# daniabib/ComfyUI_ProPainter_Nodes

Measured on NVIDIA H100. Metric: inpainted frames/sec at 640x360, 80-frame subvideo, higher is better.
Workload: dtype f16

## Files before the change

comfyui_propainter_nodes_b200/csrc/capi.cu:

```cuda
#include <math.h>
#include <string.h>

#include <thread>
#include <vector>

#include "../../include/propainter_b200.h"
#include "engine.cuh"

struct DeviceGuard {
  int prev = -1;
  bool changed = false, ok = true;
  explicit DeviceGuard(int dev) {
    if (cudaGetDevice(&prev) != cudaSuccess) prev = -1;
    if (prev != dev) {
      ok = cudaSetDevice(dev) == cudaSuccess;
      changed = ok;
    }
  }
  ~DeviceGuard() {
    if (changed && prev >= 0) cudaSetDevice(prev);
  }
};

#define PP_HANDLE(h)                                     \
  if ((h) == nullptr) {                                  \
    pp_set_error("null engine handle");                  \
    return PP_ERR_ARG;                                   \
  }                                                      \
  PPEngine& e = *reinterpret_cast<PPEngine*>(h);         \
  DeviceGuard _dev_guard(e.device);                      \
  if (!_dev_guard.ok) {                                  \
    pp_set_error("cudaSetDevice(%d) failed", e.device);  \
    return PP_ERR_CUDA;                                  \
  }

static inline cudaStream_t as_stream(void* s) { return reinterpret_cast<cudaStream_t>(s); }

struct ArenaGuard {
  PPArena& a;
  size_t m;
  bool keep = false;
  explicit ArenaGuard(PPArena& arena) : a(arena), m(arena.mark()) {}
  ~ArenaGuard() { if (!keep) a.release(m); }
};

template <class E>
static int op_instnorm(PPEngine& e, const void* x, const void* residual, void* out, int N, int HW, int C, int relu,
                       cudaStream_t st) {
  ArenaGuard guard(e.arena);
  float* sums;
  PP_TRY(pp_alloc(e, &sums, pp_k_instnorm_scratch_floats(N, HW, C), "instnorm sums"));
  PP_TRY(pp_k_instnorm_stats(static_cast<const E*>(x), N, HW, C, sums, st));
  PP_TRY(pp_k_instnorm_apply(static_cast<const E*>(x), sums, static_cast<const E*>(residual), static_cast<E*>(out), N,
                             HW, C, relu, st));
  PP_CUDA_CHECK(cudaStreamSynchronize(st));
  return PP_OK;
}

template <class E>
static int op_corr_pyramid(PPEngine& e, const void* fmap1, const void* fmap2, int pairs, int h8, int w8, void* l0,
                           void* l1, void* l2, void* l3, cudaStream_t st) {
  ArenaGuard guard(e.arena);
  const int P = h8 * w8, P_pad = pp_raft_corr_pad(P);
  E* fpack;
  PP_TRY(pp_alloc(e, &fpack, (size_t)pairs * P_pad * 256 * (sizeof(E) == 4 ? 3 : 1), "fmap packed"));
  PP_TRY(pp_k_pack_b_operand(static_cast<const E*>(fmap2), fpack, pairs, P, P_pad, 256, st));
  e.launches++;
  E* const corr[4] = {static_cast<E*>(l0), static_cast<E*>(l1), static_cast<E*>(l2), static_cast<E*>(l3)};
  PP_TRY(pp_raft_corr_volume<E>(e, static_cast<const E*>(fmap1), fpack, pairs, P, P_pad, corr[0], st));
  PP_TRY(pp_raft_corr_pool(e, corr, (long long)pairs * P, h8, w8, st));
  PP_CUDA_CHECK(cudaStreamSynchronize(st));
  return PP_OK;
}

template <class E>
static int flow_complete_dist(pp_handle h, const char* what, const float* flows_f, const float* flows_b,
                              const float* flow_masks, int T, int H, int W, float* out_f, float* out_b, int team_first,
                              int team_size, void* stream) {
  PP_HANDLE(h);
  PP_REQUIRE(flows_f && flows_b && flow_masks && out_f && out_b, "%s: null pointer", what);
  PP_REQUIRE(e.comm != nullptr || team_size <= 1, "%s: pp_comm_init was not called", what);
  PP_REQUIRE(team_first >= 0 && team_size >= 1 && team_first + team_size <= e.world,
             "%s: team [%d, %d) of %d ranks", what, team_first, team_first + team_size, e.world);
  ArenaGuard guard(e.arena);
  return pp_stage_flow_complete<E>(e, flows_f, flows_b, flow_masks, T, H, W, out_f, out_b, team_first, team_size,
                                   as_stream(stream));
}

extern "C" {

const char* pp_version(void) { return "propainter_b200 1 sm_90a"; }

int pp_create(int device, void* workspace, size_t workspace_bytes, pp_handle* out) {
  PP_REQUIRE(out != nullptr, "pp_create: out is null");
  PP_REQUIRE(workspace != nullptr && workspace_bytes >= (64u << 20), "pp_create: workspace must be >= 64 MiB");
  PP_REQUIRE((reinterpret_cast<uintptr_t>(workspace) & 255) == 0, "pp_create: workspace must be 256-byte aligned");
  PP_CUDA_CHECK(cudaSetDevice(device));
  cudaDeviceProp prop;
  PP_CUDA_CHECK(cudaGetDeviceProperties(&prop, device));
  PP_REQUIRE(prop.major == 9 && prop.minor == 0, "pp_create: this library is built for sm_90a (Hopper H100); device %d is sm_%d%d",
             device, prop.major, prop.minor);
  PPEngine* e = new PPEngine();
  e->device = device;
  e->arena.base = static_cast<uint8_t*>(workspace);
  e->arena.cap = workspace_bytes;
  if (cudaMalloc(&e->prog_counter, 256) != cudaSuccess || cudaMemset(e->prog_counter, 0, 256) != cudaSuccess) {
    delete e;
    pp_set_error("pp_create: cudaMalloc of the program barrier word failed");
    return PP_ERR_CUDA;
  }
  *out = reinterpret_cast<pp_handle>(e);
  return PP_OK;
}

int pp_set_workspace(pp_handle h, void* workspace, size_t workspace_bytes) {
  PP_HANDLE(h);
  PP_REQUIRE(!e.gen.active, "pp_set_workspace: a generator session is active (call pp_gen_end first)");
  PP_REQUIRE(e.arena.off == 0, "pp_set_workspace: the arena is in use");
  PP_REQUIRE(workspace != nullptr && workspace_bytes >= (64u << 20), "pp_set_workspace: workspace must be >= 64 MiB");
  PP_REQUIRE((reinterpret_cast<uintptr_t>(workspace) & 255) == 0, "pp_set_workspace: workspace must be 256-byte aligned");
  e.arena.base = static_cast<uint8_t*>(workspace);
  e.arena.cap = workspace_bytes;
  e.arena.peak = 0;
  return PP_OK;
}

int pp_destroy(pp_handle h) {
  if (h != nullptr) {
    PPEngine* e = reinterpret_cast<PPEngine*>(h);
    pp_comm_destroy_impl(*e);
    if (e->prog_counter != nullptr) cudaFree(e->prog_counter);
    delete e;
  }
  return PP_OK;
}

int pp_comm_unique_id(void* out128) {
  PP_REQUIRE(out128 != nullptr, "pp_comm_unique_id: null pointer");
  return pp_comm_unique_id_impl(out128);
}

int pp_comm_init(pp_handle h, const void* unique_id128, int rank, int world) {
  PP_HANDLE(h);
  PP_REQUIRE(unique_id128 != nullptr, "pp_comm_init: null id");
  return pp_comm_init_impl(e, unique_id128, rank, world);
}

int pp_comm_destroy(pp_handle h) {
  PP_HANDLE(h);
  return pp_comm_destroy_impl(e);
}

int pp_comm_all_gather_rows(pp_handle h, void* buf, const long long* rows_per_member, size_t row_bytes, int first_rank,
                            int n_members, void* stream) {
  PP_HANDLE(h);
  PP_REQUIRE(buf != nullptr && rows_per_member != nullptr && row_bytes > 0 && n_members >= 1,
             "pp_comm_all_gather_rows: bad argument");
  std::vector<long long> off(n_members, 0);
  for (int m = 1; m < n_members; ++m) off[m] = off[m - 1] + rows_per_member[m - 1];
  return pp_comm_all_gather_blocks_impl(e, buf, off.data(), rows_per_member, row_bytes, first_rank, n_members,
                                        as_stream(stream));
}

int pp_register_conv(pp_handle h, const char* name, const void* w, const float* bias, int cout_g, int cout_g_pad,
                     int bn, int cin_g, int kh, int kw, int groups) {
  PP_HANDLE(h);
  PP_REQUIRE(name != nullptr && w != nullptr, "pp_register_conv: null argument");
  PP_REQUIRE(bn % 16 == 0 && bn >= 16 && bn <= 256 && cout_g_pad % bn == 0 && cout_g <= cout_g_pad && cin_g % 8 == 0,
             "pp_register_conv(%s): invalid packing (cout_g=%d pad=%d bn=%d cin_g=%d)", name, cout_g, cout_g_pad, bn,
             cin_g);
  PPPackedConv c;
  c.w = static_cast<const __half*>(w); c.b = bias;
  c.cout_g = cout_g; c.cout_g_pad = cout_g_pad; c.bn = bn; c.cin_g = cin_g; c.kh = kh; c.kw = kw; c.groups = groups;
  e.convs[name] = c;
  return PP_OK;
}

int pp_set_conv_macs(pp_handle h, const char* name, double macs_per_pixel) {
  PP_HANDLE(h);
  PP_REQUIRE(name != nullptr, "pp_set_conv_macs: null name");
  auto it = e.convs.find(name);
  PP_REQUIRE(it != e.convs.end(), "pp_set_conv_macs: conv '%s' is not registered", name);
  it->second.macs_per_pixel = macs_per_pixel;
  return PP_OK;
}

int pp_register_tensor(pp_handle h, const char* name, const void* ptr, size_t bytes) {
  PP_HANDLE(h);
  PP_REQUIRE(name != nullptr && ptr != nullptr, "pp_register_tensor: null argument");
  PPTensor t;
  t.ptr = ptr; t.bytes = bytes;
  e.tensors[name] = t;
  return PP_OK;
}

int pp_raft_bidir(pp_handle h, const float* frames, int T, int H, int W, int iters, float* flows_f, float* flows_b,
                  void* stream) {
  PP_HANDLE(h);
  PP_REQUIRE(frames && flows_f && flows_b, "pp_raft_bidir: null pointer");
  ArenaGuard guard(e.arena);
  return pp_stage_raft<__half>(e, frames, T, H, W, iters, flows_f, flows_b, as_stream(stream));
}

int pp_raft_bidir_fp32(pp_handle h, const float* frames, int T, int H, int W, int iters, float* flows_f, float* flows_b,
                       void* stream) {
  PP_HANDLE(h);
  PP_REQUIRE(frames && flows_f && flows_b, "pp_raft_bidir_fp32: null pointer");
  ArenaGuard guard(e.arena);
  return pp_stage_raft<float>(e, frames, T, H, W, iters, flows_f, flows_b, as_stream(stream));
}

int pp_flow_complete(pp_handle h, const float* flows_f, const float* flows_b, const float* flow_masks, int T, int H,
                     int W, float* out_f, float* out_b, void* stream) {
  PP_HANDLE(h);
  PP_REQUIRE(flows_f && flows_b && flow_masks && out_f && out_b, "pp_flow_complete: null pointer");
  ArenaGuard guard(e.arena);
  return pp_stage_flow_complete<__half>(e, flows_f, flows_b, flow_masks, T, H, W, out_f, out_b, 0, 1,
                                        as_stream(stream));
}

int pp_flow_complete_fp32(pp_handle h, const float* flows_f, const float* flows_b, const float* flow_masks, int T, int H,
                          int W, float* out_f, float* out_b, void* stream) {
  PP_HANDLE(h);
  PP_REQUIRE(flows_f && flows_b && flow_masks && out_f && out_b, "pp_flow_complete_fp32: null pointer");
  ArenaGuard guard(e.arena);
  return pp_stage_flow_complete<float>(e, flows_f, flows_b, flow_masks, T, H, W, out_f, out_b, 0, 1, as_stream(stream));
}

int pp_flow_complete_dist(pp_handle h, const float* flows_f, const float* flows_b, const float* flow_masks, int T, int H,
                          int W, float* out_f, float* out_b, int team_first, int team_size, void* stream) {
  return flow_complete_dist<__half>(h, "pp_flow_complete_dist", flows_f, flows_b, flow_masks, T, H, W, out_f, out_b,
                                    team_first, team_size, stream);
}

int pp_flow_complete_dist_fp32(pp_handle h, const float* flows_f, const float* flows_b, const float* flow_masks, int T,
                               int H, int W, float* out_f, float* out_b, int team_first, int team_size, void* stream) {
  return flow_complete_dist<float>(h, "pp_flow_complete_dist_fp32", flows_f, flows_b, flow_masks, T, H, W, out_f,
                                   out_b, team_first, team_size, stream);
}

int pp_image_propagate(pp_handle h, const float* frames, const float* masks, const float* flows_f,
                       const float* flows_b, int T, int H, int W, float* updated_frames, float* updated_masks,
                       void* stream) {
  PP_HANDLE(h);
  PP_REQUIRE(frames && masks && flows_f && flows_b && updated_frames && updated_masks,
             "pp_image_propagate: null pointer");
  ArenaGuard guard(e.arena);
  return pp_stage_image_propagate<__half>(e, frames, masks, flows_f, flows_b, T, H, W, updated_frames, updated_masks,
                                          as_stream(stream));
}

int pp_image_propagate_fp32(pp_handle h, const float* frames, const float* masks, const float* flows_f,
                            const float* flows_b, int T, int H, int W, float* updated_frames, float* updated_masks,
                            void* stream) {
  PP_HANDLE(h);
  PP_REQUIRE(frames && masks && flows_f && flows_b && updated_frames && updated_masks,
             "pp_image_propagate_fp32: null pointer");
  ArenaGuard guard(e.arena);
  return pp_stage_image_propagate<float>(e, frames, masks, flows_f, flows_b, T, H, W, updated_frames, updated_masks,
                                         as_stream(stream));
}

int pp_gen_begin_subset(pp_handle h, const float* updated_frames, const float* masks_dilated,
                        const float* updated_masks, const float* flows_f, const float* flows_b, int T, int H, int W,
                        const unsigned char* frames_needed, void* stream) {
  PP_HANDLE(h);
  PP_REQUIRE(updated_frames && masks_dilated && updated_masks && flows_f && flows_b, "pp_gen_begin: null pointer");
  const int r = pp_stage_gen_begin(e, updated_frames, masks_dilated, updated_masks, flows_f, flows_b, T, H, W,
                                   frames_needed, as_stream(stream));
  if (r != PP_OK) pp_stage_gen_end(e);
  return r;
}

int pp_gen_begin(pp_handle h, const float* updated_frames, const float* masks_dilated, const float* updated_masks,
                 const float* flows_f, const float* flows_b, int T, int H, int W, void* stream) {
  return pp_gen_begin_subset(h, updated_frames, masks_dilated, updated_masks, flows_f, flows_b, T, H, W, nullptr, stream);
}

int pp_gen_window(pp_handle h, const int* frame_ids, int t, int l_t, void* pred_f16, void* stream) {
  PP_HANDLE(h);
  PP_REQUIRE(frame_ids && pred_f16, "pp_gen_window: null pointer");
  ArenaGuard guard(e.arena);
  return pp_stage_gen_window(e, frame_ids, t, l_t, static_cast<__half*>(pred_f16), as_stream(stream));
}

int pp_gen_run(pp_handle h, const int* frame_ids, const int* win_t, const int* win_lt, int n_windows, void* pred_f16,
               void* stream) {
  PP_HANDLE(h);
  PP_REQUIRE(frame_ids && win_t && win_lt && pred_f16, "pp_gen_run: null pointer");
  ArenaGuard guard(e.arena);
  return pp_stage_gen_run(e, frame_ids, win_t, win_lt, n_windows, static_cast<__half*>(pred_f16), as_stream(stream));
}

int pp_gen_end(pp_handle h) {
  PP_HANDLE(h);
  return pp_stage_gen_end(e);
}

int pp_composite(pp_handle h, const void* pred_f16, const float* masks_dilated, const uint8_t* orig, uint8_t* comp,
                 const int* frame_ids_dev, const int* first_visit_dev, int l_t, int H, int W, int half_math,
                 void* stream) {
  PP_HANDLE(h);
  PP_REQUIRE(pred_f16 && masks_dilated && orig && comp && frame_ids_dev && first_visit_dev, "pp_composite: null pointer");
  e.launches++;
  return pp_k_composite(static_cast<const __half*>(pred_f16), 4, masks_dilated, orig, comp, frame_ids_dev,
                        first_visit_dev, l_t, H, W, half_math, as_stream(stream));
}

int pp_preprocess(pp_handle h, const float* image, const float* mask, int mask_frames, int T, int H, int W,
                  int flow_mask_dilates, int mask_dilates, uint8_t* orig_u8, float* frames, float* flow_masks,
                  float* masks_dilated, void* stream) {
  PP_HANDLE(h);
  PP_REQUIRE(image && mask && orig_u8 && frames && flow_masks && masks_dilated, "pp_preprocess: null pointer");
  ArenaGuard guard(e.arena);
  uint8_t* scratch;
  PP_TRY(pp_alloc(e, &scratch, (size_t)mask_frames * H * W, "mask scratch"));
  PP_TRY(pp_k_quantize_frames(image, orig_u8, frames, T, H, W, as_stream(stream)));
  PP_TRY(pp_k_prepare_masks(mask, mask_frames, T, H, W, flow_mask_dilates, mask_dilates, scratch, flow_masks,
                            masks_dilated, as_stream(stream)));
  e.launches += 4;
  return PP_OK;
}

static int preprocess_from_u8(PPEngine& e, const uint8_t* u8_in, const uint8_t* m_in, int mask_frames, int T, int H, int W,
                              int out_h, int out_w, int flow_mask_dilates, int mask_dilates, uint8_t* orig_u8, float* frames,
                              float* flow_masks, float* masks_dilated, cudaStream_t st) {
  const bool resize = out_h != H || out_w != W;
  const uint8_t* m_use = m_in;
  if (resize) {
    const size_t mid_px = (size_t)T * H * out_w;
    uint8_t *tmp, *m_out;
    int* coef;
    const int mx = out_h > out_w ? out_h : out_w;
    const double sc = fmax(fmax((double)H / out_h, (double)W / out_w), 1.0);
    const size_t coef_ints = 2 * (size_t)mx * ((size_t)ceil(2.0 * sc) * 2 + 1 + 2) + 64;
    PP_TRY(pp_alloc(e, &tmp, mid_px * 3, "resize pass 1"));
    PP_TRY(pp_alloc(e, &m_out, (size_t)mask_frames * out_h * out_w, "mask resized"));
    PP_TRY(pp_alloc(e, &coef, coef_ints, "resize coefficients"));
    PP_TRY(pp_k_resize_bicubic_u8(u8_in, orig_u8, tmp, coef, coef_ints, T, H, W, 3, out_h, out_w, st));
    PP_TRY(pp_k_resize_bicubic_u8(m_in, m_out, tmp, coef, coef_ints, mask_frames, H, W, 1, out_h, out_w, st));
    m_use = m_out;
    e.launches += 4;
  } else {
    PP_CUDA_CHECK(cudaMemcpyAsync(orig_u8, u8_in, (size_t)T * H * W * 3, cudaMemcpyDeviceToDevice, st));
  }
  PP_TRY(pp_k_u8_to_frames(orig_u8, frames, T, out_h, out_w, st));
  PP_TRY(pp_k_dilate_masks_u8(m_use, mask_frames, T, out_h, out_w, flow_mask_dilates, mask_dilates, flow_masks,
                              masks_dilated, st));
  e.launches += 3;
  return PP_OK;
}

int pp_preprocess_resize(pp_handle h, const float* image, const float* mask, int mask_frames, int T, int H, int W,
                         int out_h, int out_w, int flow_mask_dilates, int mask_dilates, uint8_t* orig_u8, float* frames,
                         float* flow_masks, float* masks_dilated, void* stream) {
  PP_HANDLE(h);
  PP_REQUIRE(image && mask && orig_u8 && frames && flow_masks && masks_dilated, "pp_preprocess_resize: null pointer");
  PP_REQUIRE(out_h > 0 && out_w > 0 && H > 0 && W > 0, "pp_preprocess_resize: bad size");
  ArenaGuard guard(e.arena);
  cudaStream_t st = as_stream(stream);
  const size_t in_px = (size_t)T * H * W;
  uint8_t *u8_in, *m_in;
  PP_TRY(pp_alloc(e, &u8_in, in_px * 3, "resize input"));
  PP_TRY(pp_alloc(e, &m_in, (size_t)mask_frames * H * W, "mask input"));
  PP_TRY(pp_k_quantize_u8(image, u8_in, (long long)in_px * 3, st));
  PP_TRY(pp_k_quantize_u8(mask, m_in, (long long)mask_frames * H * W, st));
  e.launches += 2;
  return preprocess_from_u8(e, u8_in, m_in, mask_frames, T, H, W, out_h, out_w, flow_mask_dilates, mask_dilates, orig_u8,
                            frames, flow_masks, masks_dilated, st);
}

int pp_preprocess_u8(pp_handle h, const uint8_t* image_u8, const uint8_t* mask_u8, int mask_frames, int T, int H, int W,
                     int out_h, int out_w, int flow_mask_dilates, int mask_dilates, uint8_t* orig_u8, float* frames,
                     float* flow_masks, float* masks_dilated, void* stream) {
  PP_HANDLE(h);
  PP_REQUIRE(image_u8 && mask_u8 && orig_u8 && frames && flow_masks && masks_dilated, "pp_preprocess_u8: null pointer");
  PP_REQUIRE(out_h > 0 && out_w > 0 && H > 0 && W > 0, "pp_preprocess_u8: bad size");
  ArenaGuard guard(e.arena);
  return preprocess_from_u8(e, image_u8, mask_u8, mask_frames, T, H, W, out_h, out_w, flow_mask_dilates, mask_dilates,
                            orig_u8, frames, flow_masks, masks_dilated, as_stream(stream));
}

int pp_host_quantize_u8(const float* src, uint8_t* dst, long long n, int threads) {
  PP_REQUIRE(src != nullptr && dst != nullptr && n >= 0, "pp_host_quantize_u8: bad argument");
  if (threads < 1) threads = 1;
  if (threads > 64) threads = 64;
  auto work = [=](long long lo, long long hi) {
    for (long long i = lo; i < hi; ++i) {
      float v = src[i] * 255.0f;
      v = v < 0.0f ? 0.0f : (v > 255.0f ? 255.0f : v);
      dst[i] = (uint8_t)(int)v;
    }
  };
  if (threads == 1 || n < (1 << 16)) { work(0, n); return PP_OK; }
  std::vector<std::thread> pool;
  const long long per = (n + threads - 1) / threads;
  for (int t = 0; t < threads; ++t) {
    const long long lo = t * per, hi = lo + per < n ? lo + per : n;
    if (lo < hi) pool.emplace_back(work, lo, hi);
  }
  for (auto& th : pool) th.join();
  return PP_OK;
}

int pp_postprocess(pp_handle h, const uint8_t* comp_u8, float* image_out, long long n, void* stream) {
  PP_HANDLE(h);
  PP_REQUIRE(comp_u8 && image_out, "pp_postprocess: null pointer");
  e.launches++;
  return pp_k_u8_to_unit_float(comp_u8, image_out, n, as_stream(stream));
}

long long pp_launch_count(pp_handle h) { return h ? reinterpret_cast<PPEngine*>(h)->launches : 0; }
size_t pp_workspace_peak(pp_handle h) { return h ? reinterpret_cast<PPEngine*>(h)->arena.peak : 0; }

int pp_profile_enable(pp_handle h, int on) {
  PP_HANDLE(h);
  PP_CUDA_CHECK(cudaDeviceSynchronize());
  for (auto& r : e.prof) { cudaEventDestroy(r.a); cudaEventDestroy(r.b); }
  e.prof.clear();
  e.profile = on != 0;
  return PP_OK;
}

int pp_profile_dump(pp_handle h, char* buf, size_t cap) {
  PP_HANDLE(h);
  PP_REQUIRE(buf != nullptr && cap > 0, "pp_profile_dump: no buffer");
  PP_CUDA_CHECK(cudaDeviceSynchronize());
  struct Agg { long long n = 0; double ms = 0, rows = 0, flops = 0, bytes = 0; };
  std::map<std::string, Agg> agg;
  for (auto& r : e.prof) {
    float ms = 0.f;
    if (cudaEventElapsedTime(&ms, r.a, r.b) != cudaSuccess) ms = 0.f;
    Agg& a = agg[r.name];
    a.n++; a.ms += ms; a.rows += r.rows; a.flops += r.flops; a.bytes += r.bytes;
  }
  size_t off = 0;
  buf[0] = 0;
  for (auto& kv : agg) {
    char line[512];
    int n = snprintf(line, sizeof(line), "%s\t%lld\t%.6f\t%.0f\t%.0f\t%.0f\n", kv.first.c_str(), kv.second.n,
                     kv.second.ms, kv.second.rows, kv.second.flops, kv.second.bytes);
    if (off + n + 1 > cap) { pp_set_error("pp_profile_dump: buffer too small"); return PP_ERR_ARG; }
    memcpy(buf + off, line, n + 1);
    off += n;
  }
  return PP_OK;
}

int pp_op_conv(pp_handle h, const char* name, const void* x_f16, int N, int H, int W, int stride, int pad, int dil,
               int replicate, int act, float slope, const void* residual_f16, void* out_f16, void* stream) {
  PP_HANDLE(h);
  const PPPackedConv* w = nullptr;
  PP_TRY(pp_get_conv(e, name, &w));
  PPConvCall c(e, name, N, H, W);
  c.in(static_cast<const __half*>(x_f16), w->cin_g * w->groups, 0, w->cin_g, w->groups > 1 ? w->cin_g : 0)
      .geom(stride, stride, pad, pad, dil, dil, replicate)
      .out(static_cast<__half*>(out_f16), w->cout_g * w->groups, 0, w->groups > 1 ? w->cout_g : 0)
      .act(act, slope);
  if (residual_f16 != nullptr) c.residual(static_cast<const __half*>(residual_f16), w->cout_g * w->groups, 0);
  return c.run(as_stream(stream));
}

int pp_op_corr_lookup(pp_handle h, const void* l0, const void* l1, const void* l2, const void* l3,
                      const float* coords, void* out_f16, long long nq, int h8, int w8, void* stream) {
  PP_HANDLE(h);
  e.launches++;
  return pp_k_corr_lookup(static_cast<const __half*>(l0), static_cast<const __half*>(l1),
                          static_cast<const __half*>(l2), static_cast<const __half*>(l3), coords,
                          static_cast<__half*>(out_f16), 328, nq, h8, w8, as_stream(stream));
}

int pp_op_conv_tf32(pp_handle h, const char* name, const float* x0, int x0_C, int x0_co, int x0_ch, const float* x1,
                    int x1_C, int x1_co, int x1_ch, int N, int H, int W, int sh, int sw, int ph, int pw, int dh, int dw,
                    int replicate, int epi, int act, float slope, float scale, int act2, const float* aux0, int aux0_C, int aux0_co, float* aux1,
                    int aux1_C, int aux1_co, float* out, int out_C, int out_co, int out_fp32, void* stream) {
  PP_HANDLE(h);
  PP_REQUIRE(name && x0 && out, "pp_op_conv_tf32: null pointer");
  PP_REQUIRE(epi == PP_EPI_STD || (aux0 && aux1), "pp_op_conv_tf32: the GRU epilogues need aux0 and aux1");
  PPConvCall c(e, name, N, H, W);
  c.in(x0, x0_C, x0_co, x0_ch);
  if (x1 != nullptr) c.in(x1, x1_C, x1_co, x1_ch);
  c.geom(sh, sw, ph, pw, dh, dw, replicate);
  if (out_fp32) c.out_f32(out, out_C, out_co);
  else c.out(out, out_C, out_co);
  if (epi == PP_EPI_GRU_ZR) {
    c.gru_zr(aux0, aux0_C, aux0_co, aux1, aux1_C, aux1_co);
  } else if (epi == PP_EPI_GRU_H) {
    c.gru_h(aux0, aux0_C, aux0_co, aux1, aux1_C, aux1_co);
  } else {
    c.act(act, slope, scale, act2);
    if (aux0 != nullptr) c.residual(aux0, aux0_C, aux0_co);
  }
  return c.run(as_stream(stream));
}

int pp_op_dcn_sample_f32(pp_handle h, const float* x0, int C0, const float* x1, int C1, const float* offs, int N,
                         int H, int W, float max_mag, float* cols, void* stream) {
  PP_HANDLE(h);
  const auto al16 = [](const void* p) { return (reinterpret_cast<uintptr_t>(p) & 15) == 0; };
  PP_REQUIRE(al16(x0) && al16(x1) && al16(cols), "pp_op_dcn_sample_f32: x0, x1 and cols must be 16-byte aligned");
  e.launches++;
  return pp_k_dcn_sample(x0, C0, x1, C1, offs, 432, max_mag, cols, N, H, W, as_stream(stream));
}

int pp_op_upsample2x_f32(pp_handle h, const float* src, float* dst, int N, int H, int W, int C, void* stream) {
  PP_HANDLE(h);
  PP_REQUIRE(src && dst, "pp_op_upsample2x_f32: null pointer");
  PP_REQUIRE(((reinterpret_cast<uintptr_t>(src) | reinterpret_cast<uintptr_t>(dst)) & 15) == 0,
             "pp_op_upsample2x_f32: src and dst must be 16-byte aligned");
  e.launches++;
  return pp_k_upsample2x(src, dst, N, H, W, C, as_stream(stream));
}

int pp_op_instnorm(pp_handle h, const void* x, const void* residual, void* out, int N, int HW, int C, int relu, int fp32,
                   void* stream) {
  PP_HANDLE(h);
  PP_REQUIRE(x && out, "pp_op_instnorm: null pointer");
  return fp32 ? op_instnorm<float>(e, x, residual, out, N, HW, C, relu, as_stream(stream))
              : op_instnorm<__half>(e, x, residual, out, N, HW, C, relu, as_stream(stream));
}

int pp_op_corr_pyramid(pp_handle h, const void* fmap1, const void* fmap2, int pairs, int h8, int w8, int fp32, void* l0,
                       void* l1, void* l2, void* l3, void* stream) {
  PP_HANDLE(h);
  PP_REQUIRE(fmap1 && fmap2 && l0 && l1 && l2 && l3 && pairs >= 1, "pp_op_corr_pyramid: bad argument");
  return fp32 ? op_corr_pyramid<float>(e, fmap1, fmap2, pairs, h8, w8, l0, l1, l2, l3, as_stream(stream))
              : op_corr_pyramid<__half>(e, fmap1, fmap2, pairs, h8, w8, l0, l1, l2, l3, as_stream(stream));
}

int pp_op_corr_lookup_f32(pp_handle h, const float* l0, const float* l1, const float* l2, const float* l3,
                          const float* coords, float* out, long long nq, int h8, int w8, void* stream) {
  PP_HANDLE(h);
  e.launches++;
  return pp_k_corr_lookup(l0, l1, l2, l3, coords, out, 352, nq, h8, w8, as_stream(stream));
}

int pp_op_convex_upsample(pp_handle h, const float* coords1, const void* mask, float* out, int B, int h8, int w8, int fp32,
                          void* stream) {
  PP_HANDLE(h);
  e.launches++;
  if (fp32) return pp_k_convex_upsample(coords1, static_cast<const float*>(mask), out, B, h8, w8, as_stream(stream));
  return pp_k_convex_upsample(coords1, static_cast<const __half*>(mask), out, B, h8, w8, as_stream(stream));
}

int pp_op_imgprop_step(pp_handle h, const void* cur4_f16, const void* prop_in4_f16, void* prop_out4_f16,
                       const void* flow_prop_f16, const void* flow_check_f16, int H, int W, void* stream) {
  PP_HANDLE(h);
  e.launches++;
  return pp_k_imgprop_step(static_cast<const __half*>(cur4_f16), static_cast<const __half*>(prop_in4_f16),
                           static_cast<__half*>(prop_out4_f16), static_cast<const __half*>(flow_prop_f16),
                           static_cast<const __half*>(flow_check_f16), H, W, as_stream(stream));
}

int pp_op_imgprop_step_f32(pp_handle h, const float* cur4, const float* prop_in4, float* prop_out4,
                           const float* flow_prop, const float* flow_check, int H, int W, void* stream) {
  PP_HANDLE(h);
  PP_REQUIRE(cur4 && prop_in4 && prop_out4 && flow_prop && flow_check, "pp_op_imgprop_step_f32: null pointer");
  e.launches++;
  return pp_k_imgprop_step(cur4, prop_in4, prop_out4, flow_prop, flow_check, H, W, as_stream(stream));
}

int pp_op_attention(pp_handle h, const void* qkv_f16, const void* pkv_f16, void* out_f16, const int* win_flags_dev,
                    int t, int gh, int gw, int n_pool, int parity, void* stream) {
  PP_HANDLE(h);
  const int nh = pp_ceil_div(gh, 5) * 5, nw = pp_ceil_div(gw, 9) * 9;
  std::vector<int> ring;
  pp_build_ring_indices(nh, nw, ring);
  ArenaGuard guard(e.arena);
  int* ring_dev;
  PP_TRY(pp_alloc(e, &ring_dev, ring.size(), "ring indices"));
  PP_CUDA_CHECK(cudaMemcpyAsync(ring_dev, ring.data(), ring.size() * sizeof(int), cudaMemcpyHostToDevice,
                                as_stream(stream)));
  const __half* qkv = static_cast<const __half*>(qkv_f16);
  const __half* pkv = static_cast<const __half*>(pkv_f16);
  int meta_host[2] = {0, t};
  int* meta_dev;
  PP_TRY(pp_alloc(e, &meta_dev, 2, "attention meta"));
  PP_CUDA_CHECK(cudaMemcpyAsync(meta_dev, meta_host, sizeof(meta_host), cudaMemcpyHostToDevice, as_stream(stream)));
  const int key_stride = ((t + 1) / 2) * (193 + n_pool);
  int* key_tab;
  PP_TRY(pp_alloc(e, &key_tab, (size_t)(nh / 5) * (nw / 9) * key_stride, "attention key table"));
  int r = pp_k_attention(qkv, qkv + 512, qkv + 1024, 1536, pkv, pkv + 512, 1024, static_cast<__half*>(out_f16), 512,
                         win_flags_dev, ring_dev, meta_dev, meta_dev + 1, 1, t, gh, gw, nh, nw, n_pool, parity,
                         key_tab, key_stride, as_stream(stream));
  PP_CUDA_CHECK(cudaStreamSynchronize(as_stream(stream)));
  e.launches++;
  return r;
}

}
```

comfyui_propainter_nodes_b200/csrc/conv_epilogue.cuh:

```cuda
#pragma once
#include "conv_igemm.cuh"
#include "wgmma_ops.cuh"

namespace ppconv {

template <int ACT, bool ACC = false, int N>
__device__ __forceinline__ void act16_t(float (&v)[N], float slope) {
#pragma unroll
  for (int i = 0; i < N; ++i) {
    if (ACT == PP_ACT_RELU) v[i] = fmaxf(v[i], 0.f);
    else if (ACT == PP_ACT_LRELU) v[i] = v[i] > 0.f ? v[i] : v[i] * slope;
    else if (ACT == PP_ACT_SIGMOID) v[i] = ppx::sigmoidf_(v[i]);
    else if (ACT == PP_ACT_TANH) v[i] = ACC ? ppx::tanh_acc(v[i]) : tanhf(v[i]);
    else if (ACT == PP_ACT_GELU) v[i] = ppx::gelu_erf(v[i]);
  }
}
template <bool ACC = false, int N>
__device__ __forceinline__ void act16(float (&v)[N], int act, float slope) {
  switch (act) {
    case PP_ACT_RELU: act16_t<PP_ACT_RELU, ACC>(v, slope); break;
    case PP_ACT_LRELU: act16_t<PP_ACT_LRELU, ACC>(v, slope); break;
    case PP_ACT_SIGMOID: act16_t<PP_ACT_SIGMOID, ACC>(v, slope); break;
    case PP_ACT_TANH: act16_t<PP_ACT_TANH, ACC>(v, slope); break;
    case PP_ACT_GELU: act16_t<PP_ACT_GELU, ACC>(v, slope); break;
    default: break;
  }
}

__device__ __forceinline__ void load16(const __half* src, int nvalid, bool vec, float (&r)[16]) {
  if (vec && nvalid == 16) {
    const uint4 a = reinterpret_cast<const uint4*>(src)[0], b = reinterpret_cast<const uint4*>(src)[1];
    const __half2* ha = reinterpret_cast<const __half2*>(&a);
    const __half2* hb = reinterpret_cast<const __half2*>(&b);
#pragma unroll
    for (int i = 0; i < 4; ++i) {
      const float2 fa = __half22float2(ha[i]), fb = __half22float2(hb[i]);
      r[2 * i] = fa.x; r[2 * i + 1] = fa.y; r[8 + 2 * i] = fb.x; r[8 + 2 * i + 1] = fb.y;
    }
  } else {
#pragma unroll
    for (int i = 0; i < 16; ++i) r[i] = i < nvalid ? __half2float(src[i]) : 0.f;
  }
}
__device__ __forceinline__ void store16(__half* dst, int nvalid, bool vec, const float (&v)[16]) {
  if (vec && nvalid == 16) {
    __align__(16) __half2 h[8];
#pragma unroll
    for (int i = 0; i < 8; ++i) h[i] = __floats2half2_rn(v[2 * i], v[2 * i + 1]);
    reinterpret_cast<uint4*>(dst)[0] = reinterpret_cast<uint4*>(h)[0];
    reinterpret_cast<uint4*>(dst)[1] = reinterpret_cast<uint4*>(h)[1];
  } else {
#pragma unroll
    for (int i = 0; i < 16; ++i)
      if (i < nvalid) dst[i] = __float2half_rn(v[i]);
  }
}

__device__ __forceinline__ void conv_epilogue16(const PPConvParams& p, const uint32_t (&raw)[16], long long mrow, int g,
                                                int ng0, int epi, bool vec) {
    const int nvalid = min(16, p.Cout_g - ng0);
    float v[16];
#pragma unroll
    for (int i = 0; i < 16; ++i) v[i] = __uint_as_float(raw[i]);
    if (p.bias != nullptr) {
      const float* bp = p.bias + g * p.Cout_g + ng0;
      if (vec && nvalid == 16) {
#pragma unroll
        for (int i = 0; i < 4; ++i) {
          const float4 b4 = __ldg(reinterpret_cast<const float4*>(bp) + i);
          v[4 * i] += b4.x; v[4 * i + 1] += b4.y; v[4 * i + 2] += b4.z; v[4 * i + 3] += b4.w;
        }
      } else {
#pragma unroll
        for (int i = 0; i < 16; ++i)
          if (i < nvalid) v[i] += __ldg(bp + i);
      }
    }
    if (epi == PP_EPI_STD) {
      act16(v, p.act1, p.slope);
      if (p.scale != 1.f) {
#pragma unroll
        for (int i = 0; i < 16; ++i) v[i] *= p.scale;
      }
      if (p.aux0 != nullptr) {
        float r[16];
        load16(p.aux0 + mrow * p.aux0_cstride + p.aux0_coff + ng0, nvalid, vec, r);
#pragma unroll
        for (int i = 0; i < 16; ++i) v[i] += r[i];
      }
      act16(v, p.act2, p.slope);
      const long long o = mrow * p.out_cstride + p.out_coff + (long long)g * p.out_gstep + ng0;
      if (p.out_fp32) {
        float* dst = reinterpret_cast<float*>(p.out) + o;
        if (vec && nvalid == 16) {
#pragma unroll
          for (int i = 0; i < 4; ++i)
            reinterpret_cast<float4*>(dst)[i] = make_float4(v[4 * i], v[4 * i + 1], v[4 * i + 2], v[4 * i + 3]);
        } else {
#pragma unroll
          for (int i = 0; i < 16; ++i)
            if (i < nvalid) dst[i] = v[i];
        }
      } else {
        store16(reinterpret_cast<__half*>(p.out) + o, nvalid, vec, v);
      }
    } else if (epi == PP_EPI_GRU_ZR) {
      const int half_c = p.Cout_g >> 1;
      act16_t<PP_ACT_SIGMOID>(v, 0.f);
      if (ng0 < half_c) {
        store16(reinterpret_cast<__half*>(p.out) + mrow * p.out_cstride + p.out_coff + ng0, nvalid, vec, v);
      } else {
        const int c = ng0 - half_c;
        float h[16];
        load16(p.aux0 + mrow * p.aux0_cstride + p.aux0_coff + c, nvalid, vec, h);
#pragma unroll
        for (int i = 0; i < 16; ++i) v[i] *= h[i];
        store16(p.out2 + mrow * p.out2_cstride + p.out2_coff + c, nvalid, vec, v);
      }
    } else {
      float h[16], z[16];
      load16(p.aux0 + mrow * p.aux0_cstride + p.aux0_coff + ng0, nvalid, vec, h);
      load16(p.aux1 + mrow * p.aux1_cstride + p.aux1_coff + ng0, nvalid, vec, z);
      act16_t<PP_ACT_TANH>(v, 0.f);
#pragma unroll
      for (int i = 0; i < 16; ++i) v[i] = (1.f - z[i]) * h[i] + z[i] * v[i];
      store16(reinterpret_cast<__half*>(p.out) + mrow * p.out_cstride + p.out_coff + ng0, nvalid, vec, v);
    }
}

__device__ __forceinline__ void load16_split(const float* src, int lo, int nvalid, bool vec, float (&r)[16]) {
  if (vec && nvalid == 16) {
#pragma unroll
    for (int i = 0; i < 4; ++i) {
      const float4 h = reinterpret_cast<const float4*>(src)[i], l = reinterpret_cast<const float4*>(src + lo)[i];
      r[4 * i] = h.x + l.x; r[4 * i + 1] = h.y + l.y; r[4 * i + 2] = h.z + l.z; r[4 * i + 3] = h.w + l.w;
    }
  } else {
#pragma unroll
    for (int i = 0; i < 16; ++i) r[i] = i < nvalid ? src[i] + src[lo + i] : 0.f;
  }
}
__device__ __forceinline__ void store16_split(float* dst, int lo, int nvalid, bool vec, const float (&v)[16]) {
  float h[16], l[16];
#pragma unroll
  for (int i = 0; i < 16; ++i) { h[i] = ppx::tf32_rna(v[i]); l[i] = v[i] - h[i]; }
  if (vec && nvalid == 16) {
#pragma unroll
    for (int i = 0; i < 4; ++i) {
      reinterpret_cast<float4*>(dst)[i] = make_float4(h[4 * i], h[4 * i + 1], h[4 * i + 2], h[4 * i + 3]);
      reinterpret_cast<float4*>(dst + lo)[i] = make_float4(l[4 * i], l[4 * i + 1], l[4 * i + 2], l[4 * i + 3]);
    }
  } else {
#pragma unroll
    for (int i = 0; i < 16; ++i)
      if (i < nvalid) { dst[i] = h[i]; dst[lo + i] = l[i]; }
  }
}

__device__ __forceinline__ void conv_epilogue16_split(const PPConvParams& p, const float (&acc)[16], long long mrow, int g,
                                                      int ng0, bool vec) {
  const int nvalid = min(16, p.Cout_g - ng0);
  float v[16];
#pragma unroll
  for (int i = 0; i < 16; ++i) v[i] = acc[i];
  if (p.bias != nullptr) {
    const float* bp = p.bias + g * p.Cout_g + ng0;
#pragma unroll
    for (int i = 0; i < 16; ++i)
      if (i < nvalid) v[i] += __ldg(bp + i);
  }
  const float* aux0 = reinterpret_cast<const float*>(p.aux0);
  const float* aux1 = reinterpret_cast<const float*>(p.aux1);
  float* out = reinterpret_cast<float*>(p.out);
  if (p.epi == PP_EPI_STD) {
    act16<true>(v, p.act1, p.slope);
    if (p.scale != 1.f) {
#pragma unroll
      for (int i = 0; i < 16; ++i) v[i] *= p.scale;
    }
    if (aux0 != nullptr) {
      float r[16];
      load16_split(aux0 + mrow * p.aux0_cstride + p.aux0_coff + ng0, p.aux0_lo, nvalid, vec, r);
#pragma unroll
      for (int i = 0; i < 16; ++i) v[i] += r[i];
    }
    act16<true>(v, p.act2, p.slope);
    float* dst = out + mrow * p.out_cstride + p.out_coff + (long long)g * p.out_gstep + ng0;
    if (p.out_fp32) {
      if (vec && nvalid == 16) {
#pragma unroll
        for (int i = 0; i < 4; ++i)
          reinterpret_cast<float4*>(dst)[i] = make_float4(v[4 * i], v[4 * i + 1], v[4 * i + 2], v[4 * i + 3]);
      } else {
#pragma unroll
        for (int i = 0; i < 16; ++i)
          if (i < nvalid) dst[i] = v[i];
      }
    } else {
      store16_split(dst, p.out_lo, nvalid, vec, v);
    }
  } else if (p.epi == PP_EPI_GRU_ZR) {
    const int half_c = p.Cout_g >> 1;
    act16_t<PP_ACT_SIGMOID, true>(v, 0.f);
    if (ng0 < half_c) {
      store16_split(out + mrow * p.out_cstride + p.out_coff + ng0, p.out_lo, nvalid, vec, v);
    } else {
      const int c = ng0 - half_c;
      float h[16];
      load16_split(aux0 + mrow * p.aux0_cstride + p.aux0_coff + c, p.aux0_lo, nvalid, vec, h);
#pragma unroll
      for (int i = 0; i < 16; ++i) v[i] *= h[i];
      store16_split(reinterpret_cast<float*>(p.out2) + mrow * p.out2_cstride + p.out2_coff + c, p.out2_lo, nvalid, vec, v);
    }
  } else {
    float h[16], z[16];
    load16_split(aux0 + mrow * p.aux0_cstride + p.aux0_coff + ng0, p.aux0_lo, nvalid, vec, h);
    load16_split(aux1 + mrow * p.aux1_cstride + p.aux1_coff + ng0, p.aux1_lo, nvalid, vec, z);
    act16_t<PP_ACT_TANH, true>(v, 0.f);
#pragma unroll
    for (int i = 0; i < 16; ++i) v[i] = (1.f - z[i]) * h[i] + z[i] * v[i];
    store16_split(out + mrow * p.out_cstride + p.out_coff + ng0, p.out_lo, nvalid, vec, v);
  }
}

constexpr int STG_LD = 40;
constexpr int STG_BYTES = 64 * STG_LD * 4;

template <int N, class Emit>
__device__ __forceinline__ void drain_acc(const float (&acc)[N / 2], float* stg, int t128, int bar_id, Emit&& emit) {
  const int wrow = 16 * (t128 >> 5) + ((t128 & 31) >> 2), wcol = 2 * (t128 & 3);
#pragma unroll 1
  for (int c0 = 0; c0 < N; c0 += 32) {
#pragma unroll
    for (int cc = 0; cc < N; cc += 32) {
      if (cc == c0) {
#pragma unroll
        for (int j = 0; j < 4; ++j) {
          if (cc + 8 * j < N) {
            const int i = (cc / 8 + j) * 4;
            *reinterpret_cast<float2*>(stg + wrow * STG_LD + 8 * j + wcol) = make_float2(acc[i], acc[i + 1]);
            *reinterpret_cast<float2*>(stg + (wrow + 8) * STG_LD + 8 * j + wcol) = make_float2(acc[i + 2], acc[i + 3]);
          }
        }
      }
    }
    ppx::named_bar(bar_id, 128);
    const int c = c0 + 16 * (t128 & 1);
    if (c < N) emit(stg + (t128 >> 1) * STG_LD + 16 * (t128 & 1), t128 >> 1, c);
    ppx::named_bar(bar_id, 128);
  }
}

template <bool SPLIT = false, int EPI = -1>
__device__ __forceinline__ void epilogue_from_stage(const PPConvParams& p, const float* src, long long mrow, int g, int ng0) {
  if constexpr (SPLIT) {
    float acc[16];
#pragma unroll
    for (int i = 0; i < 16; i += 4) {
      const float4 v = *reinterpret_cast<const float4*>(src + i);
      acc[i] = v.x; acc[i + 1] = v.y; acc[i + 2] = v.z; acc[i + 3] = v.w;
    }
    conv_epilogue16_split(p, acc, mrow, g, ng0, p.vec_ok != 0);
  } else {
    uint32_t raw[16];
#pragma unroll
    for (int i = 0; i < 16; i += 4) {
      const float4 v = *reinterpret_cast<const float4*>(src + i);
      raw[i] = __float_as_uint(v.x); raw[i + 1] = __float_as_uint(v.y);
      raw[i + 2] = __float_as_uint(v.z); raw[i + 3] = __float_as_uint(v.w);
    }
    conv_epilogue16(p, raw, mrow, g, ng0, EPI >= 0 ? EPI : p.epi, p.vec_ok != 0);
  }
}

template <int V>
struct IntC { static constexpr int value = V; };
template <int MAX_N, class F>
__device__ __forceinline__ void with_tile_width(int bn, F&& f) {
  switch (bn) {
    case 16: f(IntC<16>{}); break;
    case 32: f(IntC<32>{}); break;
    case 48: f(IntC<48>{}); break;
    case 64: f(IntC<64>{}); break;
    case 80: f(IntC<80>{}); break;
    case 96: f(IntC<96>{}); break;
    case 112: f(IntC<112>{}); break;
    case 128: f(IntC<128>{}); break;
    default:
      if constexpr (MAX_N > 128) {
        switch (bn) {
          case 144: f(IntC<144>{}); break;
          case 160: f(IntC<160>{}); break;
          case 176: f(IntC<176>{}); break;
          case 192: f(IntC<192>{}); break;
          case 208: f(IntC<208>{}); break;
          case 224: f(IntC<224>{}); break;
          case 240: f(IntC<240>{}); break;
          case 256: f(IntC<256>{}); break;
          default: __trap();
        }
      } else {
        __trap();
      }
  }
}

}
```

comfyui_propainter_nodes_b200/csrc/conv_gemm.cu:

```cuda
#include <string.h>

#include "conv_epilogue.cuh"
#include "conv_igemm.cuh"

namespace {

constexpr int NUM_THREADS = 384;
constexpr int NUM_CONSUMERS = 256;
constexpr int WARP_PRODUCER = 8;
constexpr int STAGE_BYTES = 48 * 1024;
constexpr int STAGES = 3;
constexpr int OUT_BYTES = 64 * 1024;
constexpr int BIAS_BYTES = 2 * 256 * 4;
constexpr int SMEM_BYTES = 1024 + STAGES * STAGE_BYTES + OUT_BYTES + 1024 + BIAS_BYTES;

struct GemmParams {
  PPConvParams c;
  CUtensorMap tmap_a[PP_MAX_SEGS];
  CUtensorMap tmap_out;
  CUtensorMap tmap_res;
  int m_tiles, n_tiles, chunks;
  int debug;
};

struct Smem {
  uint8_t* stages;
  uint8_t* out;
  uint64_t *full, *empty, *res;
  float* bias;
};
__device__ __forceinline__ Smem gemm_smem() {
  uint8_t* base = ppx::dyn_smem_1024();
  Smem m;
  m.stages = base;
  m.out = base + STAGES * STAGE_BYTES;
  m.full = reinterpret_cast<uint64_t*>(m.out + OUT_BYTES);
  m.empty = m.full + STAGES;
  m.res = m.empty + STAGES;
  m.bias = reinterpret_cast<float*>(m.out + OUT_BYTES + 1024);
  return m;
}

template <int ACT1>
__device__ __forceinline__ void gemm_epi4(float (&v)[4], bool has_bias, const float2& bias, float scale, bool has_res,
                                          const float (&res)[4], int act2, float slope) {
  if (has_bias) {
    v[0] += bias.x; v[1] += bias.y; v[2] += bias.x; v[3] += bias.y;
  }
  ppconv::act16_t<ACT1>(v, slope);
  if (scale != 1.f) {
#pragma unroll
    for (int i = 0; i < 4; ++i) v[i] *= scale;
  }
  if (has_res) {
#pragma unroll
    for (int i = 0; i < 4; ++i) v[i] += res[i];
  }
  if (act2 != PP_ACT_NONE) ppconv::act16(v, act2, slope);
}

template <int MB, int BN, int ACT1>
__device__ __forceinline__ void gemm_epilogue(const PPConvParams& p, const float (&acc)[MB][BN / 2], uint8_t* so,
                                              const float* bs, bool has_res, int t128) {
  constexpr int PANEL = 128 * MB * 128;
  const bool has_bias = p.bias != nullptr;
  const float scale = p.scale, slope = p.slope;
  const int act2 = p.act2;
  const int fr = 16 * (t128 >> 5) + ((t128 & 31) >> 2), fc = 2 * (t128 & 3);
#pragma unroll
  for (int b = 0; b < MB; ++b) {
    const int r = 64 * b + fr;
#pragma unroll
    for (int j = 0; j < BN / 8; ++j) {
      const int col = 8 * j + fc;
      const int off = (col >> 6) * PANEL + r * 128 + (((((col & 63) >> 3) ^ (r & 7))) << 4) + (col & 7) * 2;
      __half2* lo = reinterpret_cast<__half2*>(so + off);
      __half2* hi = reinterpret_cast<__half2*>(so + off + 8 * 128);
      const float2 bias = *reinterpret_cast<const float2*>(bs + col);
      float v[4] = {acc[b][4 * j], acc[b][4 * j + 1], acc[b][4 * j + 2], acc[b][4 * j + 3]};
      float res[4] = {0.f, 0.f, 0.f, 0.f};
      if (has_res) {
        const float2 r0 = __half22float2(*lo), r1 = __half22float2(*hi);
        res[0] = r0.x; res[1] = r0.y; res[2] = r1.x; res[3] = r1.y;
      }
      gemm_epi4<ACT1>(v, has_bias, bias, scale, has_res, res, act2, slope);
      *lo = __floats2half2_rn(v[0], v[1]);
      *hi = __floats2half2_rn(v[2], v[3]);
    }
  }
}

template <int MB, int BN>
__device__ __forceinline__ void gemm_tile(const GemmParams& h, const Smem& m, int tile, int& s, uint32_t& ph, uint32_t& rph,
                                          int wg, int t128) {
  using namespace ppx;
  const PPConvParams& p = h.c;
  constexpr int A_BYTES = 128 * MB * 128;
  constexpr int WG_ROWS = 64 * MB;
  constexpr int PANEL = 128 * MB * 128;
  const int n0 = (tile % h.n_tiles) * BN;
  const int m0 = (tile / h.n_tiles) * (128 * MB);
  float acc[MB][BN / 2];
  int prev = -1;
  for (int c = 0; c < h.chunks; ++c) {
    mbar_wait(&m.full[s], ph);
    const uint32_t a = smem_u32(m.stages + s * STAGE_BYTES);
    uint64_t adesc[MB];
#pragma unroll
    for (int b = 0; b < MB; ++b) adesc[b] = gmma_desc_sw128_kmajor(a + (wg * MB + b) * 64 * 128);
    const uint64_t bdesc = gmma_desc_sw128_kmajor(a + A_BYTES);
    wgmma_fence();
#pragma unroll
    for (int k = 0; k < 4; ++k)
#pragma unroll
      for (int b = 0; b < MB; ++b) wgmma_f16<BN>(acc[b], adesc[b] + 2 * k, bdesc + 2 * k, (c | k) != 0 ? 1u : 0u);
    wgmma_commit();
    wgmma_wait<1>();
    if (prev >= 0) mbar_arrive(&m.empty[prev]);
    prev = s;
    if (++s == STAGES) { s = 0; ph ^= 1; }
  }
  wgmma_wait<0>();
#pragma unroll
  for (int b = 0; b < MB; ++b) wgmma_fence_acc(acc[b]);
  mbar_arrive(&m.empty[prev]);
  if (h.debug & 1) return;

  const int bar_id = 2 + wg, row0 = m0 + wg * WG_ROWS;
  const int npanel = (min(BN, p.Cout_g - n0) + 63) / 64;
  uint8_t* so = m.out + wg * WG_ROWS * 128;
  const bool issuer = t128 == 0;
  float* bs = m.bias + wg * 256;
  {
    const int c0 = 2 * t128, n = n0 + c0;
    float2 bv = make_float2(0.f, 0.f);
    if (p.bias != nullptr && c0 < BN) {
      if (n < p.Cout_g) bv.x = __ldg(p.bias + n);
      if (n + 1 < p.Cout_g) bv.y = __ldg(p.bias + n + 1);
    }
    if (c0 < BN) *reinterpret_cast<float2*>(bs + c0) = bv;
  }
  if (issuer) tma_store_wait_read<0>();
  named_bar(bar_id, 128);
  const bool has_res = p.aux0 != nullptr;
  if (has_res) {
    if (issuer) {
      mbar_arrive_expect_tx(&m.res[wg], (uint32_t)(npanel * WG_ROWS * 128));
      for (int pnl = 0; pnl < npanel; ++pnl) tma_load_2d(smem_u32(so + pnl * PANEL), &h.tmap_res, n0 + pnl * 64, row0, &m.res[wg]);
    }
    mbar_wait(&m.res[wg], rph);
    rph ^= 1;
  }
  switch (p.act1) {
    case PP_ACT_RELU: gemm_epilogue<MB, BN, PP_ACT_RELU>(p, acc, so, bs, has_res, t128); break;
    case PP_ACT_LRELU: gemm_epilogue<MB, BN, PP_ACT_LRELU>(p, acc, so, bs, has_res, t128); break;
    case PP_ACT_SIGMOID: gemm_epilogue<MB, BN, PP_ACT_SIGMOID>(p, acc, so, bs, has_res, t128); break;
    case PP_ACT_TANH: gemm_epilogue<MB, BN, PP_ACT_TANH>(p, acc, so, bs, has_res, t128); break;
    case PP_ACT_GELU: gemm_epilogue<MB, BN, PP_ACT_GELU>(p, acc, so, bs, has_res, t128); break;
    default: gemm_epilogue<MB, BN, PP_ACT_NONE>(p, acc, so, bs, has_res, t128); break;
  }
  fence_proxy_async();
  named_bar(bar_id, 128);
  if (issuer) {
    for (int pnl = 0; pnl < npanel; ++pnl) tma_store_2d(&h.tmap_out, smem_u32(so + pnl * PANEL), n0 + pnl * 64, row0);
    tma_store_commit();
  }
}

template <int MB>
__global__ void __launch_bounds__(NUM_THREADS, 1) conv_gemm_kernel(const __grid_constant__ GemmParams h) {
  using namespace ppx;
  constexpr int BN = 256 / MB;
  constexpr int A_BYTES = 128 * MB * 128;
  const Smem m = gemm_smem();
  const PPConvParams& p = h.c;
  const int tid = threadIdx.x, warp = tid >> 5;
  const int total_tiles = h.m_tiles * h.n_tiles;
  if (tid == 0) {
    for (int s = 0; s < STAGES; ++s) { mbar_init(&m.full[s], 1); mbar_init(&m.empty[s], NUM_CONSUMERS); }
    mbar_init(&m.res[0], 1);
    mbar_init(&m.res[1], 1);
    mbar_fence_init();
  }
  __syncthreads();
  asm volatile("griddepcontrol.wait;" ::: "memory");
  asm volatile("griddepcontrol.launch_dependents;" ::: "memory");

  if (warp < 8) setmaxnreg_inc<232>();
  else setmaxnreg_dec<40>();
  if (warp < 8) {
    const int wg = tid >> 7, t128 = tid & 127;
    int s = 0;
    uint32_t ph = 0, rph = 0;
    for (int tile = blockIdx.x; tile < total_tiles; tile += gridDim.x) gemm_tile<MB, BN>(h, m, tile, s, ph, rph, wg, t128);
    if (t128 == 0) tma_store_wait<0>();
  } else if (warp == WARP_PRODUCER) {
    if (elect_one()) {
      int s = 0;
      uint32_t ph = 0;
      for (int tile = blockIdx.x; tile < total_tiles; tile += gridDim.x) {
        const int n0 = (tile % h.n_tiles) * BN;
        const int m0 = (tile / h.n_tiles) * (128 * MB);
        const uint32_t b_bytes = (uint32_t)(min(BN, p.Cout_g_pad - n0) * 128);
        for (int c = 0; c < h.chunks; ++c) {
          const int ci = c * 64;
          const int q = pp_seg_of(p, ci);
          mbar_wait(&m.empty[s], ph ^ 1);
          mbar_arrive_expect_tx(&m.full[s], (uint32_t)A_BYTES + b_bytes);
          const uint32_t dst = smem_u32(m.stages + s * STAGE_BYTES);
          tma_load_4d(dst, &h.tmap_a[q], ci - p.seg[q].cbegin, m0, 0, 0, &m.full[s]);
          bulk_g2s(dst + A_BYTES, p.wpacked + ((long long)c * p.Cout_g_pad + n0) * 64, b_bytes, &m.full[s]);
          if (++s == STAGES) { s = 0; ph ^= 1; }
        }
      }
    }
  }
}

int gemm_mb(const PPConvParams& p) { return p.Cout_g_pad <= 128 && p.M_total >= 256 ? 2 : 1; }

long long gemm_tiles(const PPConvParams& p, int mb) {
  return pp_ceil_div64(p.M_total, 128 * mb) * pp_ceil_div(p.Cout_g_pad, 256 / mb);
}

bool aligned16(const void* ptr, int cstride, int coff) {
  return (reinterpret_cast<uintptr_t>(ptr) & 15) == 0 && cstride % 8 == 0 && coff % 8 == 0;
}

}

int pp_conv_gemm_eligible(const PPConvParams& p) {
  if (p.kh != 1 || p.kw != 1 || p.sh != 1 || p.sw != 1 || p.ph != 0 || p.pw != 0 || p.pad_replicate) return 0;
  if (p.groups != 1 || p.split || p.epi != PP_EPI_STD || p.out_fp32 || p.M_total < 128) return 0;
  if (!pp_conv_segs_chunked(p, true)) return 0;
  if (!aligned16(p.out, p.out_cstride, p.out_coff)) return 0;
  if (p.aux0 != nullptr && !aligned16(p.aux0, p.aux0_cstride, p.aux0_coff)) return 0;
  if (p.bias != nullptr && (reinterpret_cast<uintptr_t>(p.bias) & 7) != 0) return 0;
  int num_sms = 0;
  if (pp_num_sms(&num_sms) != PP_OK || gemm_tiles(p, gemm_mb(p)) < num_sms) return 0;
  return pp_tmap_supported() ? 1 : 0;
}

int pp_launch_conv_gemm(const PPConvParams& pin, cudaStream_t stream) {
  static bool attr_set = false;
  if (!attr_set) {
    PP_CUDA_CHECK(cudaFuncSetAttribute(conv_gemm_kernel<1>, cudaFuncAttributeMaxDynamicSharedMemorySize, SMEM_BYTES));
    PP_CUDA_CHECK(cudaFuncSetAttribute(conv_gemm_kernel<2>, cudaFuncAttributeMaxDynamicSharedMemorySize, SMEM_BYTES));
    attr_set = true;
  }
  GemmParams h;
  memset(&h, 0, sizeof(h));
  h.c = pin;
  const PPConvParams& p = h.c;
  const int mb = gemm_mb(p);
  h.m_tiles = (int)pp_ceil_div64(p.M_total, 128 * mb);
  h.n_tiles = pp_ceil_div(p.Cout_g_pad, 256 / mb);
  h.chunks = pp_ceil_div(p.Cin, 64);
  PP_REQUIRE((long long)h.m_tiles * h.n_tiles < (1LL << 31), "conv_gemm: too many tiles");
  h.debug = pp_conv_noepi();
  PP_TRY(pp_conv_input_tmaps(p, 128 * mb, 1, true, h.tmap_a));
  PP_TRY(pp_tmap_2d_f16(&h.tmap_out, static_cast<const __half*>(p.out) + p.out_coff, p.Cout_g, p.M_total, p.out_cstride, 64 * mb));
  if (p.aux0 != nullptr)
    PP_TRY(pp_tmap_2d_f16(&h.tmap_res, p.aux0 + p.aux0_coff, p.Cout_g, p.M_total, p.aux0_cstride, 64 * mb));
  int num_sms = 0;
  PP_TRY(pp_num_sms(&num_sms));
  return pp_conv_launch(mb == 2 ? conv_gemm_kernel<2> : conv_gemm_kernel<1>, h, min(h.m_tiles * h.n_tiles, num_sms),
                        NUM_THREADS, SMEM_BYTES, stream);
}
```

comfyui_propainter_nodes_b200/csrc/conv_halo.cu:

```cuda
#include <cuda.h>
#include <stdlib.h>
#include <string.h>

#include <memory>

#include "conv_epilogue.cuh"
#include "conv_igemm.cuh"
#include "dcn_sample.cuh"

namespace {

constexpr int NUM_THREADS = 384;
constexpr int NUM_EPI_THREADS = 256;
constexpr int WARP_A = 8, WARP_B = 9;
constexpr int MAX_SA = 4, MAX_SB = 8;
constexpr int SMEM_BUDGET = 186 * 1024;

struct HaloParams {
  PPConvParams c;
  CUtensorMap tmap[PP_MAX_SEGS];
  int MT;
  int BW, BH;
  int tiles_x, tiles_y, n_tiles;
  int a_stage_bytes, b_stage_bytes, SA, SB;
  int tps;
  int chunks;
  int flat;
  int n_img;
  int sub_bytes;
  int debug;
};

struct TileCoord {
  int n_idx, tx, ty, img, g;
};
__device__ __forceinline__ TileCoord decode_tile(const HaloParams& h, int tile) {
  TileCoord t;
  t.n_idx = tile % h.n_tiles;
  int r = tile / h.n_tiles;
  t.tx = r % h.tiles_x; r /= h.tiles_x;
  t.ty = r % h.tiles_y; r /= h.tiles_y;
  t.img = r % h.n_img;
  t.g = r / h.n_img;
  return t;
}

__host__ __device__ inline int halo_total_tiles(const HaloParams& h) {
  return h.n_tiles * h.tiles_x * h.tiles_y * h.n_img * h.c.groups;
}

struct Ring {
  int s;
  uint32_t ph;
};

struct HaloSmem {
  uint8_t* a;
  uint8_t* b;
  int SA, SB, a_stage_bytes, b_stage_bytes;
  uint64_t *a_full, *a_empty, *b_full, *b_empty;
  uint64_t* spare;
  float* acc_stg;
  int bytes;
};

__host__ __device__ inline HaloSmem halo_smem(uint8_t* base, int SA, int a_stage_bytes, int SB, int b_stage_bytes) {
  const int b_off = SA * a_stage_bytes, bar_off = b_off + SB * b_stage_bytes, acc_off = bar_off + 1024;
  HaloSmem m;
  m.SA = SA; m.SB = SB; m.a_stage_bytes = a_stage_bytes; m.b_stage_bytes = b_stage_bytes;
  m.a = base;
  m.b = base + b_off;
  m.a_full = reinterpret_cast<uint64_t*>(base + bar_off);
  m.a_empty = m.a_full + MAX_SA;
  m.b_full = m.a_empty + MAX_SA;
  m.b_empty = m.b_full + MAX_SB;
  m.spare = m.b_empty + MAX_SB;
  m.acc_stg = reinterpret_cast<float*>(base + acc_off);
  m.bytes = 1024 + acc_off + 2 * ppconv::STG_BYTES;
  return m;
}

__host__ __device__ constexpr int halo_max_tps(int bn) { return 128 / bn > 1 ? 128 / bn : 1; }

template <int BN, int MB, bool TF32>
__device__ __forceinline__ void halo_tap(float (&acc)[MB][BN / 2], uint64_t (&adesc)[MB], uint64_t& bdesc, uint32_t& accum,
                                         int& kx, int kw, uint32_t step_x, uint32_t step_row, uint32_t tap16) {
#pragma unroll
  for (int k = 0; k < 4; ++k)
#pragma unroll
    for (int b = 0; b < MB; ++b) {
      if constexpr (TF32) ppx::wgmma_tf32<BN>(acc[b], adesc[b] + 2 * k, bdesc + 2 * k, (accum | k) != 0 ? 1u : 0u);
      else ppx::wgmma_f16<BN>(acc[b], adesc[b] + 2 * k, bdesc + 2 * k, (accum | k) != 0 ? 1u : 0u);
    }
  accum = 1u;
  bdesc += tap16;
  const uint32_t step = ++kx == kw ? step_row : step_x;
  if (kx == kw) kx = 0;
#pragma unroll
  for (int b = 0; b < MB; ++b) adesc[b] += step;
}

template <int BN, int MB, int NT, bool TF32>
__device__ __forceinline__ void halo_tap_group(int tn, float (&acc)[MB][BN / 2], uint64_t (&adesc)[MB], uint64_t bdesc,
                                               uint32_t& accum, int& kx, int kw, uint32_t step_x, uint32_t step_row,
                                               uint32_t tap16) {
  using namespace ppx;
  if constexpr (NT > 1) {
    if (tn < NT) {
      halo_tap_group<BN, MB, NT - 1, TF32>(tn, acc, adesc, bdesc, accum, kx, kw, step_x, step_row, tap16);
      return;
    }
  }
  wgmma_fence();
#pragma unroll
  for (int tt = 0; tt < NT; ++tt) halo_tap<BN, MB, TF32>(acc, adesc, bdesc, accum, kx, kw, step_x, step_row, tap16);
  wgmma_commit();
}

template <int BN, int MB, int NT, bool TF32 = false, bool PROG = false>
__device__ __forceinline__ void halo_tile(const HaloParams& h, int tile, const HaloSmem& m, Ring& ra, Ring& rb, float* stg,
                                          int wg, int t128) {
  using namespace ppx;
  const PPConvParams& p = h.c;
  const int taps = p.kh * p.kw;
  const TileCoord t = decode_tile(h, tile);
  const int n0 = t.n_idx * p.BN;
  const int bnt = min(p.BN, p.Cout_g_pad - n0);
  const uint32_t sbo = h.flat ? 1024u : (uint32_t)h.BW * 128;
  const uint32_t step_x = (uint32_t)p.dw * 8;
  const uint32_t step_row = (uint32_t)(p.dh * h.BW - (p.kw - 1) * p.dw) * 8;
  const uint32_t tap16 = (uint32_t)p.BN * 8;
  const int kw = p.kw;
  uint32_t aoff[MB];
#pragma unroll
  for (int b = 0; b < MB; ++b) aoff[b] = MB == 2 ? wg * h.sub_bytes + b * 8 * sbo : wg * 8 * sbo;
  float acc[MB][BN / 2];
  uint32_t accum = 0;
  int pend_a = -1, pend_b = -1;
  for (int c = 0; c < h.chunks; ++c) {
    mbar_wait(&m.a_full[ra.s], ra.ph);
    uint64_t adesc[MB];
#pragma unroll
    for (int b = 0; b < MB; ++b) adesc[b] = gmma_desc_sw128_kmajor(smem_u32(m.a + ra.s * m.a_stage_bytes) + aoff[b], sbo);
    int kx = 0;
    for (int tap0 = 0; tap0 < taps; tap0 += h.tps) {
      mbar_wait(&m.b_full[rb.s], rb.ph);
      const uint64_t bdesc = gmma_desc_sw128_kmajor(smem_u32(m.b + rb.s * m.b_stage_bytes));
      halo_tap_group<BN, MB, NT, TF32>(min(h.tps, taps - tap0), acc, adesc, bdesc, accum, kx, kw, step_x, step_row, tap16);
      wgmma_wait<1>();
      if (pend_b >= 0) mbar_arrive(&m.b_empty[pend_b]);
      if (pend_a >= 0) mbar_arrive(&m.a_empty[pend_a]);
      pend_b = rb.s;
      pend_a = tap0 + h.tps >= taps ? ra.s : -1;
      if (++rb.s == m.SB) { rb.s = 0; rb.ph ^= 1; }
    }
    if (++ra.s == m.SA) { ra.s = 0; ra.ph ^= 1; }
  }
  wgmma_wait<0>();
#pragma unroll
  for (int b = 0; b < MB; ++b) wgmma_fence_acc(acc[b]);
  if (pend_b >= 0) mbar_arrive(&m.b_empty[pend_b]);
  if (pend_a >= 0) mbar_arrive(&m.a_empty[pend_a]);

  const bool skip = (h.debug & 1) != 0;
#pragma unroll
  for (int b = 0; b < MB; ++b) {
    const int sub = MB == 2 ? wg : 0, rbase = MB == 2 ? 64 * b : 64 * wg;
    ppconv::drain_acc<BN>(acc[b], stg, t128, 4 + wg, [&](const float* src, int r64, int cc) {
      const int r = rbase + r64;
      bool mvalid;
      long long mrow;
      if (h.flat) {
        mrow = ((long long)t.tx * h.MT + sub) * 128 + r;
        mvalid = mrow < p.M_total;
      } else {
        const int oy = t.ty * 16 + (r >> 3), ox = t.tx * (8 * h.MT) + 8 * sub + (r & 7);
        mvalid = oy < p.OH && ox < p.OW;
        mrow = ((long long)t.img * p.OH + oy) * p.OW + ox;
      }
      if (!mvalid || skip || cc >= bnt || n0 + cc >= p.Cout_g) return;
      ppconv::epilogue_from_stage<TF32, PROG ? PP_EPI_STD : -1>(p, src, mrow, t.g, n0 + cc);
    });
  }
}

template <class F>
__device__ __forceinline__ void with_tile_shape(int mt, int bn, F&& f) {
  if (mt == 2) ppconv::with_tile_width<128>(bn, [&](auto n) { f(n, ppconv::IntC<2>{}); });
  else ppconv::with_tile_width<256>(bn, [&](auto n) { f(n, ppconv::IntC<1>{}); });
}

__device__ __forceinline__ void halo_smem_init_barriers(const HaloSmem& m) {
  using namespace ppx;
  for (int s = 0; s < m.SA; ++s) { mbar_init(&m.a_full[s], 1); mbar_init(&m.a_empty[s], NUM_EPI_THREADS); }
  for (int s = 0; s < m.SB; ++s) { mbar_init(&m.b_full[s], 1); mbar_init(&m.b_empty[s], NUM_EPI_THREADS); }
  mbar_fence_init();
}

__device__ __forceinline__ void halo_produce_patches(const HaloParams& h, const HaloSmem& m, Ring& r) {
  using namespace ppx;
  const PPConvParams& p = h.c;
  const int total_tiles = halo_total_tiles(h);
  const uint32_t bytes = (uint32_t)(h.BW * h.BH * 128);
  for (int tile = blockIdx.x; tile < total_tiles; tile += gridDim.x) {
    const TileCoord t = decode_tile(h, tile);
    const int x0 = h.flat ? t.tx * (128 * h.MT) : t.tx * (8 * h.MT) - p.pw, y0 = h.flat ? 0 : t.ty * 16 - p.ph;
    for (int c = 0; c < h.chunks; ++c) {
      const int ci = c * 64;
      const int q = pp_seg_of(p, ci);
      const int ch0 = t.g * p.seg[q].gstep + (ci - p.seg[q].cbegin);
      mbar_wait(&m.a_empty[r.s], r.ph ^ 1);
      mbar_arrive_expect_tx(&m.a_full[r.s], bytes);
      tma_load_4d(smem_u32(m.a + r.s * m.a_stage_bytes), &h.tmap[q], ch0, x0, y0, t.img, &m.a_full[r.s]);
      if (++r.s == m.SA) { r.s = 0; r.ph ^= 1; }
    }
  }
}

__device__ __forceinline__ void halo_produce_weights(const HaloParams& h, const HaloSmem& m, Ring& r) {
  using namespace ppx;
  const PPConvParams& p = h.c;
  const int total_tiles = halo_total_tiles(h);
  const int taps = p.kh * p.kw;
  for (int tile = blockIdx.x; tile < total_tiles; tile += gridDim.x) {
    const TileCoord t = decode_tile(h, tile);
    const int n0 = t.n_idx * p.BN;
    const uint32_t bytes = (uint32_t)(min(p.BN, p.Cout_g_pad - n0) * 128);
    const __half* wbase = p.wpacked + ((long long)t.g * p.num_kc * p.Cout_g_pad + n0) * 64;
    for (int c = 0; c < h.chunks; ++c) {
      for (int tap0 = 0; tap0 < taps; tap0 += h.tps) {
        const int tn = min(h.tps, taps - tap0);
        mbar_wait(&m.b_empty[r.s], r.ph ^ 1);
        mbar_arrive_expect_tx(&m.b_full[r.s], bytes * (uint32_t)tn);
        for (int t = 0; t < tn; ++t) {
          const int kc = (tap0 + t) * h.chunks + c;
          bulk_g2s(smem_u32(m.b + r.s * m.b_stage_bytes + t * p.BN * 128), wbase + (long long)kc * p.Cout_g_pad * 64, bytes,
                   &m.b_full[r.s]);
        }
        if (++r.s == m.SB) { r.s = 0; r.ph ^= 1; }
      }
    }
  }
}

template <bool TF32>
__device__ __forceinline__ void halo_body(const HaloParams& h) {
  using namespace ppx;
  const HaloSmem m = halo_smem(dyn_smem_1024(), h.SA, h.a_stage_bytes, h.SB, h.b_stage_bytes);
  const int tid = threadIdx.x, warp = tid >> 5;
  if (tid == 0) halo_smem_init_barriers(m);
  __syncthreads();
  asm volatile("griddepcontrol.wait;" ::: "memory");
  asm volatile("griddepcontrol.launch_dependents;" ::: "memory");

  if (warp < 8) setmaxnreg_inc<232>();
  else setmaxnreg_dec<40>();
  if (warp < 8) {
    const int wg = tid >> 7, t128 = tid & 127;
    float* stg = m.acc_stg + wg * (ppconv::STG_BYTES / 4);
    Ring ra = {0, 0}, rb = {0, 0};
    const int total_tiles = halo_total_tiles(h);
    with_tile_shape(h.MT, h.c.BN, [&](auto bn, auto mb) {
      constexpr int BN = decltype(bn)::value;
      for (int tile = blockIdx.x; tile < total_tiles; tile += gridDim.x)
        halo_tile<BN, decltype(mb)::value, halo_max_tps(BN), TF32>(h, tile, m, ra, rb, stg, wg, t128);
    });
  } else if (warp == WARP_A) {
    if (elect_one()) {
      Ring r = {0, 0};
      halo_produce_patches(h, m, r);
    }
  } else if (warp == WARP_B) {
    if (elect_one()) {
      Ring r = {0, 0};
      halo_produce_weights(h, m, r);
    }
  }
}

__global__ void __launch_bounds__(NUM_THREADS, 1) conv_halo_kernel(const __grid_constant__ HaloParams h) {
  halo_body<false>(h);
}

__global__ void __launch_bounds__(NUM_THREADS, 1) conv_halo_tf32_kernel(const __grid_constant__ HaloParams h) {
  halo_body<true>(h);
}

constexpr int PROG_MAX_LAYERS = 10;
enum { PROG_CONV = 0, PROG_DCN = 1 };

constexpr int PROG_WIDTHS[] = {32, 64, 224};

template <class F>
__device__ __forceinline__ void with_prog_width(int bn, F&& f) {
  static_assert(sizeof(PROG_WIDTHS) == 3 * sizeof(int), "with_prog_width: one case per PROG_WIDTHS entry");
  switch (bn) {
    case PROG_WIDTHS[0]: f(ppconv::IntC<PROG_WIDTHS[0]>{}); break;
    case PROG_WIDTHS[1]: f(ppconv::IntC<PROG_WIDTHS[1]>{}); break;
    case PROG_WIDTHS[2]: f(ppconv::IntC<PROG_WIDTHS[2]>{}); break;
    default: __trap();
  }
}

struct ProgParams {
  int n_layers;
  int SA, SB, a_stage_bytes, b_stage_bytes;
  unsigned int* counter;
  unsigned int base;
  unsigned long long* ts;
  int kind[PROG_MAX_LAYERS];
  PPDcnArgs dcn[PROG_MAX_LAYERS];
  HaloParams layer[PROG_MAX_LAYERS];
};

__device__ __forceinline__ void prog_wait(const unsigned int* counter, unsigned int target) {
  unsigned int v, spins = 0;
  uint64_t t0 = 0;
  for (;;) {
    asm volatile("ld.acquire.gpu.global.u32 %0, [%1];" : "=r"(v) : "l"(counter) : "memory");
    if ((int)(v - target) >= 0) return;
    __nanosleep(64);
    if ((++spins & 0xFFFu) == 0) {
      uint64_t now;
      asm volatile("mov.u64 %0, %%globaltimer;" : "=l"(now));
      if (t0 == 0) t0 = now;
      else if (now - t0 > 2000000000ull) __trap();
    }
  }
}

__global__ void __launch_bounds__(NUM_THREADS, 1) conv_prog_kernel(const __grid_constant__ ProgParams P) {
  using namespace ppx;
  const HaloSmem m = halo_smem(dyn_smem_1024(), P.SA, P.a_stage_bytes, P.SB, P.b_stage_bytes);
  uint64_t* layer_go = m.spare;

  const int tid = threadIdx.x, warp = tid >> 5;
  const unsigned int G = gridDim.x;
  if (tid == 0) {
    mbar_init(layer_go, 1);
    halo_smem_init_barriers(m);
  }
  __syncthreads();
  asm volatile("griddepcontrol.wait;" ::: "memory");
  asm volatile("griddepcontrol.launch_dependents;" ::: "memory");

  if (warp < 8) setmaxnreg_inc<232>();
  else setmaxnreg_dec<40>();
  if (warp < 8) {
    const int wg = tid >> 7, t128 = tid & 127;
    float* stg = m.acc_stg + wg * (ppconv::STG_BYTES / 4);
    Ring ra = {0, 0}, rb = {0, 0};
    for (int li = 0; li < P.n_layers; ++li) {
      mbar_wait(layer_go, (uint32_t)li & 1u);
      if (P.ts != nullptr && blockIdx.x == 0 && tid == 0) {
        unsigned long long now;
        asm volatile("mov.u64 %0, %%globaltimer;" : "=l"(now));
        P.ts[2 * li] = now;
      }
      if (P.kind[li] == PROG_DCN) {
        const PPDcnArgs& a = P.dcn[li];
        const unsigned per_img = (unsigned)(a.H * a.W * 144);
        const unsigned total = per_img * (unsigned)a.N;
        const unsigned stride = G * NUM_EPI_THREADS;
        for (unsigned idx = blockIdx.x * NUM_EPI_THREADS + tid; idx < total; idx += 4 * stride) {
#pragma unroll
          for (int u = 0; u < 4; ++u) {
            const unsigned i2 = idx + u * stride;
            if (i2 < total) {
              const unsigned n = i2 / per_img;
              if (a.C == 128) dcn_sample_item<8, true>(a, i2 - n * per_img, (int)n);
              else dcn_sample_item<16, true>(a, i2 - n * per_img, (int)n);
            }
          }
        }
      } else {
        const HaloParams& h = P.layer[li];
        const int total_tiles = halo_total_tiles(h);
        with_prog_width(h.c.BN, [&](auto bn) {
          constexpr int BN = decltype(bn)::value;
          for (int tile = blockIdx.x; tile < total_tiles; tile += G)
            halo_tile<BN, 1, halo_max_tps(BN), false, true>(h, tile, m, ra, rb, stg, wg, t128);
        });
      }
      fence_proxy_async_global();
      asm volatile("bar.sync 1, %0;" ::"n"(NUM_EPI_THREADS) : "memory");
      if (tid == 0) {
        __threadfence();
        atomicAdd(P.counter, 1u);
        if (P.ts != nullptr && blockIdx.x == 0) {
          unsigned long long now;
          asm volatile("mov.u64 %0, %%globaltimer;" : "=l"(now));
          P.ts[2 * li + 1] = now;
        }
      }
    }
  } else if (warp == WARP_A) {
    if (elect_one()) {
      Ring r = {0, 0};
      for (int li = 0; li < P.n_layers; ++li) {
        if (li > 0) {
          prog_wait(P.counter, P.base + (unsigned int)li * G);
          fence_proxy_async_global();
        }
        mbar_arrive(layer_go);
        if (P.kind[li] == PROG_CONV) halo_produce_patches(P.layer[li], m, r);
      }
    }
  } else if (warp == WARP_B) {
    if (elect_one()) {
      Ring r = {0, 0};
      for (int li = 0; li < P.n_layers; ++li)
        if (P.kind[li] == PROG_CONV) halo_produce_weights(P.layer[li], m, r);
    }
  }
}

}

int pp_conv_halo_eligible(const PPConvParams& p) {
  if (p.sh != 1 || p.sw != 1 || p.pad_replicate) return 0;
  const bool flat = p.kh * p.kw == 1;
  if (flat) {
    if (p.ph != 0 || p.pw != 0 || p.groups != 1) return 0;
  } else if (p.Cin % 64 != 0) {
    return 0;
  }
  if (!pp_conv_segs_chunked(p, flat)) return 0;
  if ((p.kw - 1) * p.dw + 16 > 256 || (p.kh - 1) * p.dh + 16 > 256) return 0;
  if ((long long)p.N * p.OH * p.OW < 128) return 0;
  return pp_tmap_supported() ? 1 : 0;
}

namespace {

int halo_set_smem_limit() {
  static bool done = false;
  if (!done) {
    PP_CUDA_CHECK(cudaFuncSetAttribute(conv_halo_kernel, cudaFuncAttributeMaxDynamicSharedMemorySize, 224 * 1024));
    PP_CUDA_CHECK(cudaFuncSetAttribute(conv_halo_tf32_kernel, cudaFuncAttributeMaxDynamicSharedMemorySize, 224 * 1024));
    PP_CUDA_CHECK(cudaFuncSetAttribute(conv_prog_kernel, cudaFuncAttributeMaxDynamicSharedMemorySize, 224 * 1024));
    done = true;
  }
  return PP_OK;
}

bool halo_stages(int budget, int a_bytes, int b_bytes, int& sa, int& sb) {
  for (sa = 3; sa >= 2; --sa) {
    sb = (budget - sa * a_bytes) / b_bytes;
    if (sb >= 3) {
      if (sb > MAX_SB) sb = MAX_SB;
      return true;
    }
  }
  return false;
}

int halo_configure(const PPConvParams& pin, HaloParams& h, bool one_wave) {
  h.c = pin;
  PPConvParams& p = h.c;
  int num_sms = 0;
  PP_TRY(pp_num_sms(&num_sms));
  const bool flat = p.kh * p.kw == 1;
  const int n_tiles0 = pp_ceil_div(p.Cout_g_pad, 128);
  int bn = pp_ceil_div(pp_ceil_div(p.Cout_g_pad, n_tiles0), 16) * 16;
  const int tiles_y = flat ? 1 : pp_ceil_div(p.OH, 16);
  auto tiles_x = [&](int mt) { return flat ? (int)pp_ceil_div64(p.M_total, 128 * mt) : pp_ceil_div(p.OW, 8 * mt); };
  const int n_img = flat ? 1 : p.N;
  auto count = [&](int mt, int bn_) {
    return (long long)pp_ceil_div(p.Cout_g_pad, bn_) * tiles_x(mt) * tiles_y * n_img * p.groups;
  };
  int mt = count(2, bn) < num_sms ? 1 : 2;
  while (count(mt, bn) < num_sms && bn >= 64 && bn % 32 == 0) bn /= 2;
  if (one_wave) {
    mt = 1;
    long long best_cols = -1, best_waves = 0;
    for (const int b : PROG_WIDTHS) {
      const long long waves = (count(1, b) + num_sms - 1) / num_sms;
      if (best_cols < 0 || waves * b < best_cols || (waves * b == best_cols && waves < best_waves)) {
        best_cols = waves * b;
        best_waves = waves;
        bn = b;
      }
    }
  }
  p.BN = bn;
  h.MT = mt;
  h.flat = flat ? 1 : 0;
  h.n_img = n_img;
  h.BW = flat ? 128 * mt : 8 * mt + (p.kw - 1) * p.dw;
  h.BH = flat ? 1 : 16 + (p.kh - 1) * p.dh;
  h.sub_bytes = flat ? 128 * 128 : 8 * 128;
  h.tiles_x = tiles_x(mt);
  h.tiles_y = tiles_y;
  h.n_tiles = pp_ceil_div(p.Cout_g_pad, bn);
  h.chunks = pp_ceil_div(p.Cin, 64);
  h.a_stage_bytes = pp_ceil_div(h.BW * h.BH * 128, 1024) * 1024;
  h.tps = min(halo_max_tps(bn), p.kh * p.kw);
  h.b_stage_bytes = h.tps * bn * 128;
  int sa = 0, sb = 0;
  PP_REQUIRE(halo_stages(SMEM_BUDGET, h.a_stage_bytes, h.b_stage_bytes, sa, sb),
             "conv_halo: patch %dx%d does not fit shared memory", h.BW, h.BH);
  if (sa == 3 && sb == MAX_SB && (SMEM_BUDGET - 4 * h.a_stage_bytes) / h.b_stage_bytes >= MAX_SB) sa = 4;
  h.SA = sa; h.SB = sb;
  h.debug = pp_conv_noepi();
  const long long total_tiles = count(mt, bn);
  PP_REQUIRE(total_tiles < (1LL << 31), "conv_halo: too many tiles");
  return pp_conv_input_tmaps(p, h.BW, h.BH, flat, h.tmap);
}

}

int pp_launch_conv_halo(const PPConvParams& pin, cudaStream_t stream) {
  HaloParams h;
  PP_TRY(halo_configure(pin, h, false));
  PP_TRY(halo_set_smem_limit());
  int num_sms = 0;
  PP_TRY(pp_num_sms(&num_sms));
  const int smem = halo_smem(nullptr, h.SA, h.a_stage_bytes, h.SB, h.b_stage_bytes).bytes;
  return pp_conv_launch(h.c.split ? conv_halo_tf32_kernel : conv_halo_kernel, h, min(halo_total_tiles(h), num_sms),
                        NUM_THREADS, smem, stream);
}

namespace {
thread_local PPProgRecorder* g_recorder = nullptr;
}

struct PPProgRecorder {
  ProgParams prog;
  double flops = 0.0;
  int n_conv = 0;
};

bool pp_prog_recording() { return g_recorder != nullptr; }

int pp_prog_begin() {
  PP_REQUIRE(g_recorder == nullptr, "conv program: already recording");
  g_recorder = new PPProgRecorder();
  memset(&g_recorder->prog, 0, sizeof(ProgParams));
  return PP_OK;
}

void pp_prog_abort() {
  delete g_recorder;
  g_recorder = nullptr;
}

int pp_prog_record_conv(const PPConvParams& p) {
  PPProgRecorder* r = g_recorder;
  PP_REQUIRE(r != nullptr, "conv program: not recording");
  PP_REQUIRE(r->prog.n_layers < PROG_MAX_LAYERS, "conv program: more than %d layers", PROG_MAX_LAYERS);
  PP_REQUIRE(pp_conv_halo_eligible(p), "conv program: layer is not a stride-1 TMA halo-kernel convolution");
  PP_REQUIRE(!p.split, "conv program: split-tf32 layers are not supported");
  PP_REQUIRE(p.epi == PP_EPI_STD, "conv program: only the plain epilogue (bias, activations, residual) is compiled in");
  const int li = r->prog.n_layers;
  PP_TRY(halo_configure(p, r->prog.layer[li], true));
  const HaloParams& h = r->prog.layer[li];
  PP_REQUIRE(h.MT == 1 && (h.c.BN == PROG_WIDTHS[0] || h.c.BN == PROG_WIDTHS[1] || h.c.BN == PROG_WIDTHS[2]),
             "conv program: layer tile %d x %d columns is not instantiated", h.MT, h.c.BN);
  r->prog.kind[li] = PROG_CONV;
  r->prog.n_layers++;
  r->n_conv++;
  return PP_OK;
}

int pp_prog_record_dcn(const PPDcnArgs& a) {
  PPProgRecorder* r = g_recorder;
  PP_REQUIRE(r != nullptr, "conv program: not recording");
  PP_REQUIRE(r->prog.n_layers < PROG_MAX_LAYERS, "conv program: more than %d layers", PROG_MAX_LAYERS);
  const int li = r->prog.n_layers;
  r->prog.kind[li] = PROG_DCN;
  r->prog.dcn[li] = a;
  r->prog.n_layers++;
  return PP_OK;
}

int pp_prog_end(unsigned int* counter, unsigned int* arrivals, cudaStream_t stream) {
  PPProgRecorder* r = g_recorder;
  PP_REQUIRE(r != nullptr, "conv program: not recording");
  g_recorder = nullptr;
  std::unique_ptr<PPProgRecorder> guard(r);
  ProgParams& P = r->prog;
  if (P.n_layers == 0) return PP_OK;
  PP_TRY(halo_set_smem_limit());
  int num_sms = 0;
  PP_TRY(pp_num_sms(&num_sms));
  int a_max = 1024, b_max = 2048;
  for (int i = 0; i < P.n_layers; ++i)
    if (P.kind[i] == PROG_CONV) {
      if (P.layer[i].a_stage_bytes > a_max) a_max = P.layer[i].a_stage_bytes;
      if (P.layer[i].b_stage_bytes > b_max) b_max = P.layer[i].b_stage_bytes;
    }
  int sa = 0, sb = 0;
  PP_REQUIRE(halo_stages(SMEM_BUDGET, a_max, b_max, sa, sb), "conv program: stages do not fit shared memory (A %d B, B %d B)",
             a_max, b_max);
  P.SA = sa; P.SB = sb; P.a_stage_bytes = a_max; P.b_stage_bytes = b_max;
  P.counter = counter;
  P.base = *arrivals;
  static int ts_mode = -1, ts_printed = 0;
  static unsigned long long* ts_dev = nullptr;
  if (ts_mode < 0) {
    const char* e = getenv("PP_PROG_TS");
    ts_mode = (e != nullptr && atoi(e) != 0) ? atoi(e) : 0;
    if (ts_mode) PP_CUDA_CHECK(cudaMalloc(&ts_dev, 2 * PROG_MAX_LAYERS * sizeof(unsigned long long)));
  }
  P.ts = (ts_mode && ts_printed < ts_mode) ? ts_dev : nullptr;
  const int grid = num_sms;
  *arrivals += (unsigned int)(P.n_layers * grid);
  PP_TRY(pp_conv_launch(conv_prog_kernel, P, grid, NUM_THREADS, halo_smem(nullptr, sa, a_max, sb, b_max).bytes, stream));
  if (P.ts != nullptr) {
    unsigned long long h[2 * PROG_MAX_LAYERS];
    PP_CUDA_CHECK(cudaStreamSynchronize(stream));
    PP_CUDA_CHECK(cudaMemcpy(h, ts_dev, sizeof(h), cudaMemcpyDeviceToHost));
    ++ts_printed;
    fprintf(stderr, "[prog %d] %d layers:", ts_printed, P.n_layers);
    for (int i = 0; i < P.n_layers; ++i) {
      const HaloParams& L = P.layer[i];
      if (P.kind[i] == PROG_CONV)
        fprintf(stderr, " | conv K=%d N=%d bn=%d mt=%d tiles=%d: %.1f us (gap %.1f)", L.c.K_total, L.c.Cout_g, L.c.BN, L.MT,
                halo_total_tiles(L), (h[2 * i + 1] - h[2 * i]) / 1e3, i ? (h[2 * i] - h[2 * i - 1]) / 1e3 : 0.0);
      else
        fprintf(stderr, " | dcn: %.1f us (gap %.1f)", (h[2 * i + 1] - h[2 * i]) / 1e3, i ? (h[2 * i] - h[2 * i - 1]) / 1e3 : 0.0);
    }
    fprintf(stderr, " | total %.1f us\n", (h[2 * P.n_layers - 1] - h[0]) / 1e3);
  }
  return PP_OK;
}
```

comfyui_propainter_nodes_b200/csrc/conv_igemm.cu:

```cuda
#include <stdlib.h>

#include "conv_igemm.cuh"
#include "conv_epilogue.cuh"

namespace {

constexpr int BM = 128;
constexpr int BK = 64;
constexpr int A_STAGE_BYTES = BM * BK * 2;
constexpr int NUM_CONSUMERS = 256;
constexpr int NUM_PRODUCERS = 128;
constexpr int NUM_THREADS = 384;
constexpr int MAX_STAGES = 8;
constexpr int SMEM_BUDGET = 192 * 1024;

template <int BN, bool TF32>
__device__ __forceinline__ void igemm_consume(const PPConvParams& p, uint8_t* smem, int stage_bytes, uint64_t* full_bar,
                                              uint64_t* empty_bar, float* stg, int wg, int t128) {
  using namespace ppx;
  const int S = p.stages;
  const int num_kc = p.num_kc;
  const int m_tiles = (p.M_total + BM - 1) / BM;
  const int n_tiles = p.Cout_g_pad / p.BN;
  const int total_tiles = m_tiles * n_tiles * p.groups;
  float acc[BN / 2];
  int s = 0;
  uint32_t phase = 0;
  for (int tile = blockIdx.x; tile < total_tiles; tile += gridDim.x) {
    const int n_idx = tile % n_tiles;
    const int rest = tile / n_tiles;
    const int m0 = (rest % m_tiles) * BM;
    const int g = rest / m_tiles;
    const int n0 = n_idx * p.BN;
    int prev = -1;
    for (int kc = 0; kc < num_kc; ++kc) {
      mbar_wait(&full_bar[s], phase);
      fence_proxy_async();
      wgmma_fence();
      const uint32_t a_addr = smem_u32(smem + s * stage_bytes);
      const uint64_t adesc = gmma_desc_sw128_kmajor(a_addr + wg * (A_STAGE_BYTES / 2));
      const uint64_t bdesc = gmma_desc_sw128_kmajor(a_addr + A_STAGE_BYTES);
#pragma unroll
      for (int k = 0; k < BK / 16; ++k) {
        if constexpr (TF32) wgmma_tf32<BN>(acc, adesc + 2 * k, bdesc + 2 * k, (kc | k) != 0 ? 1u : 0u);
        else wgmma_f16<BN>(acc, adesc + 2 * k, bdesc + 2 * k, (kc | k) != 0 ? 1u : 0u);
      }
      wgmma_commit();
      wgmma_wait<1>();
      if (prev >= 0) mbar_arrive(&empty_bar[prev]);
      prev = s;
      if (++s == S) { s = 0; phase ^= 1; }
    }
    wgmma_wait<0>();
    wgmma_fence_acc(acc);
    mbar_arrive(&empty_bar[prev]);
    ppconv::drain_acc<BN>(acc, stg, t128, 4 + wg, [&](const float* src, int r, int c) {
      const int m = m0 + wg * 64 + r;
      if (m < p.M_total && n0 + c < p.Cout_g)
        ppconv::epilogue_from_stage<TF32>(p, src, m, g, n0 + c);
    });
  }
}

template <bool TF32>
__device__ __forceinline__ void igemm_body(const PPConvParams& p) {
  using namespace ppx;
  uint8_t* smem = dyn_smem_1024();

  const int S = p.stages;
  const int b_stage_bytes = p.BN * 128;
  const int stage_bytes = A_STAGE_BYTES + b_stage_bytes;
  float* stg = reinterpret_cast<float*>(smem + S * stage_bytes);
  uint64_t* full_bar = reinterpret_cast<uint64_t*>(smem + S * stage_bytes + 2 * ppconv::STG_BYTES);
  uint64_t* empty_bar = full_bar + MAX_STAGES;

  const int tid = threadIdx.x;
  const int num_kc = p.num_kc;
  const int m_tiles = (p.M_total + BM - 1) / BM;
  const int n_tiles = p.Cout_g_pad / p.BN;
  const int total_tiles = m_tiles * n_tiles * p.groups;

  if (tid == 0) {
    for (int s = 0; s < S; ++s) {
      mbar_init(&full_bar[s], NUM_PRODUCERS + 1);
      mbar_init(&empty_bar[s], NUM_CONSUMERS);
    }
    mbar_fence_init();
  }
  __syncthreads();
  asm volatile("griddepcontrol.wait;" ::: "memory");
  asm volatile("griddepcontrol.launch_dependents;" ::: "memory");

  if (tid < NUM_CONSUMERS) {
    setmaxnreg_inc<216>();
    const int wg = tid >> 7;
    ppconv::with_tile_width<256>(p.BN, [&](auto bn) {
      igemm_consume<decltype(bn)::value, TF32>(p, smem, stage_bytes, full_bar, empty_bar, stg + wg * (ppconv::STG_BYTES / 4), wg,
                                         tid & 127);
    });
  } else {
    setmaxnreg_dec<64>();
    const int ptid = tid - NUM_CONSUMERS;
    const int j = ptid & 7;
    const int rb = ptid >> 3;
    const uint32_t a_off = rb * 128 + ((j ^ (rb & 7)) << 4);
    int s = 0;
    uint32_t phase = 0;
    for (int tile = blockIdx.x; tile < total_tiles; tile += gridDim.x) {
      const int n0 = (tile % n_tiles) * p.BN;
      const int rest = tile / n_tiles;
      const int m0 = (rest % m_tiles) * BM;
      const int g = rest / m_tiles;
      const __half* wsrc = p.wpacked + ((long long)g * num_kc * p.Cout_g_pad + n0) * BK;
      int rpix[8], riy[8], rix[8];
      uint32_t rvalid = 0;
#pragma unroll
      for (int i = 0; i < 8; ++i) {
        const int m = m0 + rb + 16 * i;
        if (m < p.M_total) {
          const int ox = m % p.OW;
          const int t = m / p.OW;
          const int oy = t % p.OH;
          const int img = t / p.OH;
          rpix[i] = img * p.H * p.W;
          riy[i] = oy * p.sh - p.ph;
          rix[i] = ox * p.sw - p.pw;
          rvalid |= 1u << i;
        } else {
          rpix[i] = 0; riy[i] = 0; rix[i] = 0;
        }
      }
      int k = j * 8;
      int tap0 = k / p.Cin;
      int ci = k - tap0 * p.Cin;
      int ky = tap0 / p.kw;
      int kx = tap0 - ky * p.kw;
      for (int kc = 0; kc < num_kc; ++kc) {
        mbar_wait(&empty_bar[s], phase ^ 1);
        if (ptid == 0) {
          mbar_arrive_expect_tx(&full_bar[s], (uint32_t)b_stage_bytes);
          bulk_g2s(smem_u32(smem + s * stage_bytes + A_STAGE_BYTES), wsrc + (long long)kc * p.Cout_g_pad * BK,
                   (uint32_t)b_stage_bytes, &full_bar[s]);
        }
        const bool kvalid = k < p.K_total;
        const int q = pp_seg_of(p, ci);
        const __half* sbase = p.seg[q].ptr + p.seg[q].coff + g * p.seg[q].gstep + (ci - p.seg[q].cbegin);
        const long long cs = p.seg[q].cstride;
        const int dy = ky * p.dh, dx = kx * p.dw;
        const uint32_t a_dst = smem_u32(smem + s * stage_bytes) + a_off;
#pragma unroll
        for (int i = 0; i < 8; ++i) {
          int iy = riy[i] + dy, ix = rix[i] + dx;
          bool v = kvalid && ((rvalid >> i) & 1u);
          if (p.pad_replicate) {
            iy = min(max(iy, 0), p.H - 1);
            ix = min(max(ix, 0), p.W - 1);
          } else {
            v = v && ((unsigned)iy < (unsigned)p.H) && ((unsigned)ix < (unsigned)p.W);
          }
          const __half* src = v ? sbase + (long long)(rpix[i] + iy * p.W + ix) * cs : p.seg[0].ptr;
          cp_async16(a_dst + i * (16 * 128), src, v ? 16u : 0u);
        }
        k += BK;
        ci += BK;
        while (ci >= p.Cin) {
          ci -= p.Cin;
          if (++kx == p.kw) { kx = 0; ++ky; }
        }
        cp_async_arrive_noinc(&full_bar[s]);
        if (++s == S) { s = 0; phase ^= 1; }
      }
    }
  }
}

__global__ void __launch_bounds__(NUM_THREADS, 1) conv_igemm_kernel(const __grid_constant__ PPConvParams p) {
  igemm_body<false>(p);
}

__global__ void __launch_bounds__(NUM_THREADS, 1) conv_igemm_tf32_kernel(const __grid_constant__ PPConvParams p) {
  igemm_body<true>(p);
}

}

namespace {
thread_local char g_last_kind = '?';
}
char pp_last_conv_kind() { return g_last_kind; }

int pp_launch_conv(const PPConvParams& pin, cudaStream_t stream) {
  PPConvParams p = pin;
  PP_REQUIRE(p.BN >= 16 && p.BN <= 256 && p.BN % 16 == 0, "conv: BN=%d must be a multiple of 16 in [16,256]", p.BN);
  PP_REQUIRE(p.Cout_g_pad % p.BN == 0, "conv: Cout_g_pad=%d not a multiple of BN=%d", p.Cout_g_pad, p.BN);
  PP_REQUIRE(p.Cin % 8 == 0, "conv: Cin=%d must be a multiple of 8", p.Cin);
  PP_REQUIRE(p.nseg >= 1 && p.nseg <= PP_MAX_SEGS, "conv: nseg=%d", p.nseg);
  PP_REQUIRE(p.seg[p.nseg - 1].cend == p.Cin && p.seg[0].cbegin == 0, "conv: segments do not cover Cin=%d", p.Cin);
  for (int i = 0; i < p.nseg; ++i) {
    PP_REQUIRE(p.seg[i].cstride % 8 == 0 && p.seg[i].coff % 8 == 0 && p.seg[i].gstep % 8 == 0 &&
                   p.seg[i].cbegin % 8 == 0 && p.seg[i].cend % 8 == 0,
               "conv: segment %d is not 16-byte aligned (cstride=%d coff=%d)", i, p.seg[i].cstride, p.seg[i].coff);
    PP_REQUIRE((reinterpret_cast<uintptr_t>(p.seg[i].ptr) & 15) == 0, "conv: segment %d pointer misaligned", i);
  }
  PP_REQUIRE((reinterpret_cast<uintptr_t>(p.wpacked) & 15) == 0, "conv: weight pointer misaligned");
  p.K_total = p.kh * p.kw * p.Cin;
  p.num_kc = pp_ceil_div(p.K_total, BK);
  p.M_total = p.N * p.OH * p.OW;
  if (p.M_total <= 0) return PP_OK;
  if (p.split) {
    auto al = [](const void* ptr, long long cs, long long co, long long gs, long long lo) {
      return ptr == nullptr || ((reinterpret_cast<uintptr_t>(ptr) & 15) == 0 && cs % 4 == 0 && co % 4 == 0 && gs % 4 == 0 &&
                                lo % 4 == 0);
    };
    bool ok = al(p.out, p.out_cstride, p.out_coff, p.out_gstep, p.out_fp32 ? 0 : p.out_lo) &&
              al(p.aux0, p.aux0_cstride, p.aux0_coff, 0, p.aux0_lo) && al(p.aux1, p.aux1_cstride, p.aux1_coff, 0, p.aux1_lo) &&
              al(p.out2, p.out2_cstride, p.out2_coff, 0, p.out2_lo);
    if (p.epi == PP_EPI_GRU_ZR) ok = ok && ((p.Cout_g >> 1) % 16 == 0);
    p.vec_ok = ok ? 1 : 0;
  } else {
    const int esz = p.out_fp32 ? 4 : 2, per16 = 16 / esz;
    auto al = [](const void* ptr, long long cs, long long co, long long gs, int per) {
      return ptr == nullptr || ((reinterpret_cast<uintptr_t>(ptr) & 15) == 0 && cs % per == 0 && co % per == 0 && gs % per == 0);
    };
    bool ok = al(p.out, p.out_cstride, p.out_coff, p.out_gstep, per16) && al(p.aux0, p.aux0_cstride, p.aux0_coff, 0, 8) &&
              al(p.aux1, p.aux1_cstride, p.aux1_coff, 0, 8) && al(p.out2, p.out2_cstride, p.out2_coff, 0, 8);
    if (p.bias != nullptr) ok = ok && (reinterpret_cast<uintptr_t>(p.bias) & 15) == 0 && (p.groups == 1 || p.Cout_g % 4 == 0);
    if (p.epi == PP_EPI_GRU_ZR) ok = ok && ((p.Cout_g >> 1) % 16 == 0);
    p.vec_ok = ok ? 1 : 0;
  }
  if (pp_prog_recording()) {
    PP_REQUIRE(!p.split, "conv program: split-tf32 layers are not supported");
    g_last_kind = 'p';
    return pp_prog_record_conv(p);
  }
  if (pp_conv_gemm_eligible(p)) { g_last_kind = 'g'; return pp_launch_conv_gemm(p, stream); }
  if (pp_conv_halo_eligible(p)) { g_last_kind = 'h'; return pp_launch_conv_halo(p, stream); }
  g_last_kind = 'i';
  for (int i = 0; i < p.nseg; ++i)
    PP_REQUIRE(p.seg[i].cvalid == 0, "conv: zero-extended input channels (cvalid=%d of %d) need the TMA halo kernel "
               "(stride 1, zero padding, Cin %% 64 == 0)", p.seg[i].cvalid, p.seg[i].cend - p.seg[i].cbegin);
  const int stage_bytes = A_STAGE_BYTES + p.BN * 128;
  int stages = SMEM_BUDGET / stage_bytes;
  if (stages > MAX_STAGES) stages = MAX_STAGES;
  p.stages = stages;
  const size_t smem = (size_t)stages * stage_bytes + 2 * ppconv::STG_BYTES + 1024 + 256;
  static bool smem_limit_set = false;
  if (!smem_limit_set) {
    PP_CUDA_CHECK(cudaFuncSetAttribute(conv_igemm_kernel, cudaFuncAttributeMaxDynamicSharedMemorySize, 220 * 1024));
    PP_CUDA_CHECK(cudaFuncSetAttribute(conv_igemm_tf32_kernel, cudaFuncAttributeMaxDynamicSharedMemorySize, 220 * 1024));
    smem_limit_set = true;
  }
  int num_sms = 0;
  PP_TRY(pp_num_sms(&num_sms));
  const long long total_tiles = (long long)pp_ceil_div(p.M_total, BM) * (p.Cout_g_pad / p.BN) * p.groups;
  PP_REQUIRE(total_tiles < (1LL << 31), "conv: too many tiles");
  const int grid = (int)(total_tiles < num_sms ? total_tiles : num_sms);
  return pp_conv_launch(p.split ? conv_igemm_tf32_kernel : conv_igemm_kernel, p, grid, NUM_THREADS, smem, stream);
}

int pp_num_sms(int* n) {
  static int num_sms = 0;
  if (num_sms == 0) {
    int dev = 0, v = 0;
    PP_CUDA_CHECK(cudaGetDevice(&dev));
    PP_CUDA_CHECK(cudaDeviceGetAttribute(&v, cudaDevAttrMultiProcessorCount, dev));
    num_sms = v;
  }
  *n = num_sms;
  return PP_OK;
}

int pp_conv_noepi() {
  const char* e = getenv("PP_CONV_NOEPI");
  return (e != nullptr && atoi(e) != 0) ? 1 : 0;
}

namespace {

typedef CUresult (*EncodeTiledFn)(CUtensorMap*, CUtensorMapDataType, cuuint32_t, void*, const cuuint64_t*, const cuuint64_t*,
                                  const cuuint32_t*, const cuuint32_t*, CUtensorMapInterleave, CUtensorMapSwizzle,
                                  CUtensorMapL2promotion, CUtensorMapFloatOOBfill);

EncodeTiledFn encode_fn() {
  static EncodeTiledFn fn = nullptr;
  static bool tried = false;
  if (!tried) {
    tried = true;
    cudaDriverEntryPointQueryResult qr;
    void* ptr = nullptr;
    if (cudaGetDriverEntryPoint("cuTensorMapEncodeTiled", &ptr, cudaEnableDefault, &qr) == cudaSuccess &&
        qr == cudaDriverEntryPointSuccess)
      fn = reinterpret_cast<EncodeTiledFn>(ptr);
  }
  return fn;
}

}

bool pp_tmap_supported() { return encode_fn() != nullptr; }

int pp_conv_input_tmaps(const PPConvParams& p, int bw, int bh, bool flat, CUtensorMap* maps) {
  EncodeTiledFn enc = encode_fn();
  PP_REQUIRE(enc != nullptr, "conv: cuTensorMapEncodeTiled is not available");
  for (int i = 0; i < p.nseg; ++i) {
    const PPConvSeg& s = p.seg[i];
    const cuuint64_t cacc = (cuuint64_t)(p.groups - 1) * s.gstep + (s.cvalid > 0 ? s.cvalid : s.cend - s.cbegin);
    cuuint64_t dims[4] = {cacc, (cuuint64_t)p.W, (cuuint64_t)p.H, (cuuint64_t)p.N};
    cuuint64_t strides[3] = {(cuuint64_t)s.cstride * 2, (cuuint64_t)p.W * s.cstride * 2, (cuuint64_t)p.H * p.W * s.cstride * 2};
    cuuint32_t box[4] = {64, (cuuint32_t)bw, (cuuint32_t)bh, 1};
    if (flat) {
      dims[1] = (cuuint64_t)p.M_total; dims[2] = 1; dims[3] = 1;
      strides[1] = strides[2] = (cuuint64_t)p.M_total * s.cstride * 2;
    }
    cuuint32_t es[4] = {1, 1, 1, 1};
    const CUresult r = enc(&maps[i], CU_TENSOR_MAP_DATA_TYPE_FLOAT16, 4, const_cast<__half*>(s.ptr + s.coff), dims, strides, box,
                           es, CU_TENSOR_MAP_INTERLEAVE_NONE, CU_TENSOR_MAP_SWIZZLE_128B,
                           CU_TENSOR_MAP_L2_PROMOTION_L2_128B, CU_TENSOR_MAP_FLOAT_OOB_FILL_NONE);
    PP_REQUIRE(r == CUDA_SUCCESS, "conv: cuTensorMapEncodeTiled failed (%d) for segment %d (cstride=%d W=%d H=%d N=%d)",
               (int)r, i, s.cstride, p.W, p.H, p.N);
  }
  return PP_OK;
}

int pp_tmap_2d_f16(CUtensorMap* map, const __half* base, int cols, long long rows, int ld, int box_rows) {
  EncodeTiledFn enc = encode_fn();
  PP_REQUIRE(enc != nullptr, "conv: cuTensorMapEncodeTiled is not available");
  cuuint64_t dims[2] = {(cuuint64_t)cols, (cuuint64_t)rows};
  cuuint64_t strides[1] = {(cuuint64_t)ld * 2};
  cuuint32_t box[2] = {64, (cuuint32_t)box_rows};
  cuuint32_t es[2] = {1, 1};
  const CUresult r = enc(map, CU_TENSOR_MAP_DATA_TYPE_FLOAT16, 2, const_cast<__half*>(base), dims, strides, box, es,
                         CU_TENSOR_MAP_INTERLEAVE_NONE, CU_TENSOR_MAP_SWIZZLE_128B, CU_TENSOR_MAP_L2_PROMOTION_L2_128B,
                         CU_TENSOR_MAP_FLOAT_OOB_FILL_NONE);
  PP_REQUIRE(r == CUDA_SUCCESS, "conv: cuTensorMapEncodeTiled (2-D, %d x %lld, ld %d) failed (%d)", cols, rows, ld, (int)r);
  return PP_OK;
}
```

comfyui_propainter_nodes_b200/csrc/conv_igemm.cuh:

```cuda
#pragma once
#include <cuda.h>

#include "pp_common.cuh"

enum PPAct : int { PP_ACT_NONE = 0, PP_ACT_RELU = 1, PP_ACT_LRELU = 2, PP_ACT_SIGMOID = 3, PP_ACT_TANH = 4,
                   PP_ACT_GELU = 5 };

enum PPEpi : int {
  PP_EPI_STD = 0,
  PP_EPI_GRU_ZR = 1,
  PP_EPI_GRU_H = 2,
};

struct PPConvSeg {
  const __half* ptr;
  int cstride;
  int coff;
  int gstep;
  int cbegin;
  int cend;
  int cvalid;
};

constexpr int PP_MAX_SEGS = 6;

struct PPConvParams {
  PPConvSeg seg[PP_MAX_SEGS];
  int nseg;
  int N, H, W, OH, OW;
  int Cin;
  int kh, kw, sh, sw, ph, pw, dh, dw;
  int pad_replicate;
  int K_total;
  int num_kc;
  int M_total;
  const __half* wpacked;
  const float* bias;
  int Cout_g, Cout_g_pad, BN, groups;
  int stages;
  int vec_ok;
  int epi, act1, act2;
  float slope, scale;
  void* out; int out_cstride, out_coff, out_gstep, out_fp32;
  const __half* aux0; int aux0_cstride, aux0_coff;
  const __half* aux1; int aux1_cstride, aux1_coff;
  __half* out2; int out2_cstride, out2_coff;
  int split;
  int out_lo, aux0_lo, aux1_lo, out2_lo;
};

int pp_launch_conv(const PPConvParams& p, cudaStream_t stream);
char pp_last_conv_kind();
int pp_conv_halo_eligible(const PPConvParams& p);
int pp_launch_conv_halo(const PPConvParams& p, cudaStream_t stream);
int pp_conv_gemm_eligible(const PPConvParams& p);
int pp_launch_conv_gemm(const PPConvParams& p, cudaStream_t stream);

int pp_num_sms(int* n);
bool pp_tmap_supported();
int pp_conv_input_tmaps(const PPConvParams& p, int bw, int bh, bool flat, CUtensorMap* maps);
int pp_tmap_2d_f16(CUtensorMap* map, const __half* base, int cols, long long rows, int ld, int box_rows);
int pp_conv_noepi();

inline bool pp_conv_segs_chunked(const PPConvParams& p, bool flat) {
  for (int i = 0; i < p.nseg; ++i) {
    if (p.seg[i].cbegin % 64 != 0) return false;
    if (p.seg[i].cend % 64 != 0 && !(flat && i == p.nseg - 1)) return false;
  }
  return true;
}

__device__ __forceinline__ int pp_seg_of(const PPConvParams& p, int ci) {
  int q = 0;
#pragma unroll
  for (int t = 1; t < PP_MAX_SEGS; ++t)
    if (t < p.nseg && ci >= p.seg[t].cbegin) q = t;
  return q;
}

template <class Params>
int pp_conv_launch(void (*kernel)(Params), const Params& params, int grid, int threads, size_t smem_bytes,
                   cudaStream_t stream) {
  cudaLaunchConfig_t cfg = {};
  cfg.gridDim = dim3(grid);
  cfg.blockDim = dim3(threads);
  cfg.dynamicSmemBytes = smem_bytes;
  cfg.stream = stream;
  cudaLaunchAttribute attr[1];
  attr[0].id = cudaLaunchAttributeProgrammaticStreamSerialization;
  attr[0].val.programmaticStreamSerializationAllowed = 1;
  cfg.attrs = attr;
  cfg.numAttrs = 1;
  PP_CUDA_CHECK(cudaLaunchKernelEx(&cfg, kernel, params));
  PP_CUDA_CHECK(cudaGetLastError());
  return PP_OK;
}

struct PPDcnArgs;
struct PPProgRecorder;
bool pp_prog_recording();
int pp_prog_begin();
void pp_prog_abort();
int pp_prog_record_conv(const PPConvParams& p);
int pp_prog_record_dcn(const PPDcnArgs& a);
int pp_prog_end(unsigned int* counter, unsigned int* arrivals, cudaStream_t stream);
```

comfyui_propainter_nodes_b200/csrc/pp_common.cuh:

```cuda
#pragma once
#include <cuda_runtime.h>
#include <cuda_fp16.h>
#include <stdint.h>
#include <stdio.h>

#define PP_OK 0
#define PP_ERR_CUDA 1
#define PP_ERR_ARG 2
#define PP_ERR_STATE 3

void pp_set_error(const char* fmt, ...);

#define PP_CUDA_CHECK(expr)                                                                   \
  do {                                                                                        \
    cudaError_t _e = (expr);                                                                  \
    if (_e != cudaSuccess) {                                                                  \
      pp_set_error("%s:%d CUDA error %s: %s", __FILE__, __LINE__, #expr, cudaGetErrorString(_e)); \
      return PP_ERR_CUDA;                                                                     \
    }                                                                                         \
  } while (0)

#define PP_REQUIRE(cond, ...)        \
  do {                               \
    if (!(cond)) {                   \
      pp_set_error(__VA_ARGS__);     \
      return PP_ERR_ARG;             \
    }                                \
  } while (0)

#define PP_TRY(expr)                 \
  do {                               \
    int _r = (expr);                 \
    if (_r != PP_OK) return _r;      \
  } while (0)

static inline int pp_ceil_div(int a, int b) { return (a + b - 1) / b; }
static inline long long pp_ceil_div64(long long a, long long b) { return (a + b - 1) / b; }

#ifdef __CUDACC__

namespace ppx {

__device__ __forceinline__ uint32_t smem_u32(const void* p) {
  return static_cast<uint32_t>(__cvta_generic_to_shared(p));
}

__device__ __forceinline__ void mbar_init(uint64_t* bar, uint32_t count) {
  asm volatile("mbarrier.init.shared::cta.b64 [%0], %1;" ::"r"(smem_u32(bar)), "r"(count));
}
__device__ __forceinline__ void mbar_fence_init() {
  asm volatile("fence.mbarrier_init.release.cluster;" ::: "memory");
}
__device__ __forceinline__ void mbar_arrive(uint64_t* bar) {
  asm volatile("mbarrier.arrive.shared::cta.b64 _, [%0];" ::"r"(smem_u32(bar)) : "memory");
}
__device__ __forceinline__ void mbar_arrive_expect_tx(uint64_t* bar, uint32_t bytes) {
  asm volatile("mbarrier.arrive.expect_tx.shared::cta.b64 _, [%0], %1;" ::"r"(smem_u32(bar)), "r"(bytes)
               : "memory");
}
__device__ __forceinline__ void mbar_wait(uint64_t* bar, uint32_t parity) {
  const uint32_t addr = smem_u32(bar);
  asm volatile(
      "{\n"
      ".reg .pred p;\n"
      ".reg .u32 n;\n"
      "mov.u32 n, 0;\n"
      "WAIT_LOOP:\n"
      "mbarrier.try_wait.parity.shared::cta.b64 p, [%0], %1;\n"
      "@p bra WAIT_DONE;\n"
      "add.u32 n, n, 1;\n"
      "setp.lt.u32 p, n, 0x4000000;\n"
      "@p bra WAIT_LOOP;\n"
      "trap;\n"
      "WAIT_DONE:\n"
      "}\n" ::"r"(addr),
      "r"(parity)
      : "memory");
}

__device__ __forceinline__ void grid_barrier(unsigned int* counter, unsigned int target) {
  __syncthreads();
  if (threadIdx.x == 0) {
    __threadfence();
    atomicAdd(counter, 1u);
    unsigned int v, spins = 0;
    uint64_t t0 = 0;
    for (;;) {
      asm volatile("ld.acquire.gpu.global.u32 %0, [%1];" : "=r"(v) : "l"(counter) : "memory");
      if (v >= target) break;
      if ((++spins & 0xFFFu) == 0) {
        uint64_t now;
        asm volatile("mov.u64 %0, %%globaltimer;" : "=l"(now));
        if (t0 == 0) t0 = now;
        else if (now - t0 > 2000000000ull) __trap();
      }
    }
  }
  __syncthreads();
}

__device__ __forceinline__ void cp_async16(uint32_t dst_smem, const void* src, uint32_t src_bytes) {
  asm volatile("cp.async.cg.shared.global [%0], [%1], 16, %2;" ::"r"(dst_smem), "l"(src), "r"(src_bytes)
               : "memory");
}
__device__ __forceinline__ void cp_async_arrive_noinc(uint64_t* bar) {
  asm volatile("cp.async.mbarrier.arrive.noinc.shared::cta.b64 [%0];" ::"r"(smem_u32(bar)) : "memory");
}
__device__ __forceinline__ void cp_async_commit() { asm volatile("cp.async.commit_group;" ::: "memory"); }
template <int N>
__device__ __forceinline__ void cp_async_wait() {
  asm volatile("cp.async.wait_group %0;" ::"n"(N) : "memory");
}
__device__ __forceinline__ void fence_proxy_async() { asm volatile("fence.proxy.async.shared::cta;" ::: "memory"); }
__device__ __forceinline__ void fence_proxy_async_global() { asm volatile("fence.proxy.async.global;" ::: "memory"); }

__device__ __forceinline__ void bulk_g2s(uint32_t dst_smem, const void* src, uint32_t bytes, uint64_t* bar) {
  asm volatile(
      "cp.async.bulk.shared::cluster.global.mbarrier::complete_tx::bytes [%0], [%1], %2, [%3];" ::"r"(dst_smem),
      "l"(src), "r"(bytes), "r"(smem_u32(bar))
      : "memory");
}

__device__ __forceinline__ void tma_load_2d(uint32_t dst, const void* tmap, int c0, int c1, uint64_t* bar) {
  asm volatile(
      "cp.async.bulk.tensor.2d.shared::cluster.global.mbarrier::complete_tx::bytes [%0], [%1, {%3, %4}], [%2];" ::"r"(dst),
      "l"(tmap), "r"(smem_u32(bar)), "r"(c0), "r"(c1)
      : "memory");
}
__device__ __forceinline__ void tma_load_4d(uint32_t dst, const void* tmap, int c0, int c1, int c2, int c3, uint64_t* bar) {
  asm volatile(
      "cp.async.bulk.tensor.4d.shared::cluster.global.mbarrier::complete_tx::bytes [%0], [%1, {%3, %4, %5, %6}], [%2];" ::"r"(dst),
      "l"(tmap), "r"(smem_u32(bar)), "r"(c0), "r"(c1), "r"(c2), "r"(c3)
      : "memory");
}
__device__ __forceinline__ void tma_store_2d(const void* tmap, uint32_t src, int c0, int c1) {
  asm volatile("cp.async.bulk.tensor.2d.global.shared::cta.bulk_group [%0, {%2, %3}], [%1];" ::"l"(tmap), "r"(src), "r"(c0), "r"(c1)
               : "memory");
}
__device__ __forceinline__ void tma_store_commit() { asm volatile("cp.async.bulk.commit_group;" ::: "memory"); }
template <int N>
__device__ __forceinline__ void tma_store_wait_read() {
  asm volatile("cp.async.bulk.wait_group.read %0;" ::"n"(N) : "memory");
}
template <int N>
__device__ __forceinline__ void tma_store_wait() {
  asm volatile("cp.async.bulk.wait_group %0;" ::"n"(N) : "memory");
}

__device__ __forceinline__ uint8_t* dyn_smem_1024() {
  extern __shared__ uint8_t smem_raw[];
  const uint32_t raw_addr = smem_u32(smem_raw);
  return smem_raw + (((raw_addr + 1023u) & ~1023u) - raw_addr);
}

__device__ __forceinline__ void wgmma_fence() { asm volatile("wgmma.fence.sync.aligned;" ::: "memory"); }
__device__ __forceinline__ void wgmma_commit() { asm volatile("wgmma.commit_group.sync.aligned;" ::: "memory"); }
template <int N>
__device__ __forceinline__ void wgmma_wait() {
  asm volatile("wgmma.wait_group.sync.aligned %0;" ::"n"(N) : "memory");
}
template <int N>
__device__ __forceinline__ void wgmma_fence_acc(float (&d)[N]) {
#pragma unroll
  for (int i = 0; i < N; ++i) asm volatile("" : "+f"(d[i])::"memory");
}

__device__ __forceinline__ uint64_t gmma_desc_sw128(uint32_t smem_addr, uint32_t lbo, uint32_t sbo) {
  uint64_t d = 0;
  d |= (uint64_t)((smem_addr & 0x3FFFF) >> 4);
  d |= (uint64_t)((lbo >> 4) & 0x3FFF) << 16;
  d |= (uint64_t)((sbo >> 4) & 0x3FFF) << 32;
  d |= (uint64_t)1 << 62;
  return d;
}
__device__ __forceinline__ uint64_t gmma_desc_sw128_kmajor(uint32_t smem_addr, uint32_t sbo = 1024) {
  return gmma_desc_sw128(smem_addr, 16, sbo);
}
__device__ __forceinline__ uint64_t gmma_desc_sw128_mnmajor(uint32_t smem_addr, uint32_t panel_bytes) {
  return gmma_desc_sw128(smem_addr, panel_bytes, 1024);
}

template <int N>
__device__ __forceinline__ void setmaxnreg_inc() { asm volatile("setmaxnreg.inc.sync.aligned.u32 %0;" ::"n"(N)); }
template <int N>
__device__ __forceinline__ void setmaxnreg_dec() { asm volatile("setmaxnreg.dec.sync.aligned.u32 %0;" ::"n"(N)); }

__device__ __forceinline__ void named_bar(int id, int n) { asm volatile("bar.sync %0, %1;" ::"r"(id), "r"(n) : "memory"); }

__device__ __forceinline__ bool elect_one() {
  uint32_t pred;
  asm volatile(
      "{\n"
      ".reg .pred p;\n"
      "elect.sync _|p, 0xffffffff;\n"
      "selp.u32 %0, 1, 0, p;\n"
      "}\n"
      : "=r"(pred));
  return pred != 0;
}

__device__ __forceinline__ float tf32_rna(float x) {
  uint32_t r;
  asm("cvt.rna.tf32.f32 %0, %1;" : "=r"(r) : "f"(x));
  return __uint_as_float(r);
}

__device__ __forceinline__ float sigmoidf_(float x) { return 1.f / (1.f + __expf(-x)); }
__device__ __forceinline__ float gelu_erf(float x) { return 0.5f * x * (1.f + erff(x * 0.70710678118654752f)); }

__device__ __forceinline__ float rcp_acc(float d) {
  const float r = __fdividef(1.f, d);
  return fmaf(fmaf(-d, r, 1.f), r, r);
}
__device__ __forceinline__ float exp_acc(float x) {
  const float t = x * 1.44269502f;
  const float r = fmaf(x, 1.44269502f, -t) + x * 1.92596303e-8f;
  return exp2f(t) * fmaf(r, 0.693147181f, 1.f);
}
__device__ __forceinline__ float tanh_acc(float x) {
  const float a = fabsf(x);
  const float e = expm1f(2.f * a), d = e + 2.f;
  float q = e * rcp_acc(d);
  q = fmaf(fmaf(-q, d, e), rcp_acc(d), q);
  return copysignf(a > 9.f ? 1.f : q, x);
}

}

#endif
```

comfyui_propainter_nodes_b200/engine.py:

```python
from __future__ import annotations

import ctypes
import math
import os
from typing import Dict, Tuple

import torch

from . import weights as Wspec

_LIB = None
_PKG_DIR = os.path.dirname(os.path.abspath(__file__))
LIB_PATH = os.environ.get("PP_LIB_PATH") or os.path.join(_PKG_DIR, "libpropainter_b200.so")

MAX_BN = 256
ACT_NONE, ACT_RELU, ACT_LRELU, ACT_SIGMOID, ACT_TANH, ACT_GELU = range(6)

_VP, _I, _F, _LL, _SZ, _CP = (ctypes.c_void_p, ctypes.c_int, ctypes.c_float, ctypes.c_longlong, ctypes.c_size_t,
                              ctypes.c_char_p)
_SIGNATURES = {
    "pp_last_error": (_CP, []),
    "pp_version": (_CP, []),
    "pp_create": (_I, [_I, _VP, _SZ, ctypes.POINTER(_VP)]),
    "pp_destroy": (_I, [_VP]),
    "pp_set_workspace": (_I, [_VP, _VP, _SZ]),
    "pp_comm_unique_id": (_I, [_VP]),
    "pp_comm_init": (_I, [_VP, _VP, _I, _I]),
    "pp_comm_destroy": (_I, [_VP]),
    "pp_comm_all_gather_rows": (_I, [_VP, _VP, ctypes.POINTER(_LL), _SZ, _I, _I, _VP]),
    "pp_register_conv": (_I, [_VP, _CP, _VP, _VP, _I, _I, _I, _I, _I, _I, _I]),
    "pp_register_tensor": (_I, [_VP, _CP, _VP, _SZ]),
    "pp_set_conv_macs": (_I, [_VP, _CP, ctypes.c_double]),
    "pp_raft_bidir": (_I, [_VP, _VP, _I, _I, _I, _I, _VP, _VP, _VP]),
    "pp_raft_bidir_fp32": (_I, [_VP, _VP, _I, _I, _I, _I, _VP, _VP, _VP]),
    "pp_flow_complete": (_I, [_VP, _VP, _VP, _VP, _I, _I, _I, _VP, _VP, _VP]),
    "pp_flow_complete_dist": (_I, [_VP, _VP, _VP, _VP, _I, _I, _I, _VP, _VP, _I, _I, _VP]),
    "pp_flow_complete_fp32": (_I, [_VP, _VP, _VP, _VP, _I, _I, _I, _VP, _VP, _VP]),
    "pp_flow_complete_dist_fp32": (_I, [_VP, _VP, _VP, _VP, _I, _I, _I, _VP, _VP, _I, _I, _VP]),
    "pp_image_propagate": (_I, [_VP, _VP, _VP, _VP, _VP, _I, _I, _I, _VP, _VP, _VP]),
    "pp_image_propagate_fp32": (_I, [_VP, _VP, _VP, _VP, _VP, _I, _I, _I, _VP, _VP, _VP]),
    "pp_gen_begin": (_I, [_VP, _VP, _VP, _VP, _VP, _VP, _I, _I, _I, _VP]),
    "pp_gen_begin_subset": (_I, [_VP, _VP, _VP, _VP, _VP, _VP, _I, _I, _I, ctypes.c_char_p, _VP]),
    "pp_gen_window": (_I, [_VP, ctypes.POINTER(_I), _I, _I, _VP, _VP]),
    "pp_gen_run": (_I, [_VP, ctypes.POINTER(_I), ctypes.POINTER(_I), ctypes.POINTER(_I), _I, _VP, _VP]),
    "pp_gen_end": (_I, [_VP]),
    "pp_composite": (_I, [_VP, _VP, _VP, _VP, _VP, _VP, _VP, _I, _I, _I, _I, _VP]),
    "pp_preprocess": (_I, [_VP, _VP, _VP, _I, _I, _I, _I, _I, _I, _VP, _VP, _VP, _VP, _VP]),
    "pp_preprocess_resize": (_I, [_VP, _VP, _VP, _I, _I, _I, _I, _I, _I, _I, _I, _VP, _VP, _VP, _VP, _VP]),
    "pp_preprocess_u8": (_I, [_VP, _VP, _VP, _I, _I, _I, _I, _I, _I, _I, _I, _VP, _VP, _VP, _VP, _VP]),
    "pp_host_quantize_u8": (_I, [_VP, _VP, _LL, _I]),
    "pp_postprocess": (_I, [_VP, _VP, _VP, _LL, _VP]),
    "pp_launch_count": (_LL, [_VP]),
    "pp_workspace_peak": (_SZ, [_VP]),
    "pp_profile_enable": (_I, [_VP, _I]),
    "pp_profile_dump": (_I, [_VP, ctypes.c_char_p, _SZ]),
    "pp_op_conv": (_I, [_VP, _CP, _VP, _I, _I, _I, _I, _I, _I, _I, _I, _F, _VP, _VP, _VP]),
    "pp_op_corr_lookup": (_I, [_VP, _VP, _VP, _VP, _VP, _VP, _VP, _LL, _I, _I, _VP]),
    "pp_op_conv_tf32": (_I, [_VP, _CP, _VP, _I, _I, _I, _VP, _I, _I, _I, _I, _I, _I, _I, _I, _I, _I, _I, _I, _I, _I, _I,
                             _F, _F, _I, _VP, _I, _I, _VP, _I, _I, _VP, _I, _I, _I, _VP]),
    "pp_op_dcn_sample_f32": (_I, [_VP, _VP, _I, _VP, _I, _VP, _I, _I, _I, _F, _VP, _VP]),
    "pp_op_upsample2x_f32": (_I, [_VP, _VP, _VP, _I, _I, _I, _I, _VP]),
    "pp_op_instnorm": (_I, [_VP, _VP, _VP, _VP, _I, _I, _I, _I, _I, _VP]),
    "pp_op_corr_pyramid": (_I, [_VP, _VP, _VP, _I, _I, _I, _I, _VP, _VP, _VP, _VP, _VP]),
    "pp_op_corr_lookup_f32": (_I, [_VP, _VP, _VP, _VP, _VP, _VP, _VP, _LL, _I, _I, _VP]),
    "pp_op_convex_upsample": (_I, [_VP, _VP, _VP, _VP, _I, _I, _I, _I, _VP]),
    "pp_op_imgprop_step": (_I, [_VP, _VP, _VP, _VP, _VP, _VP, _I, _I, _VP]),
    "pp_op_imgprop_step_f32": (_I, [_VP, _VP, _VP, _VP, _VP, _VP, _I, _I, _VP]),
    "pp_op_attention": (_I, [_VP, _VP, _VP, _VP, _VP, _I, _I, _I, _I, _I, _VP]),
}


def load_library() -> ctypes.CDLL:
    global _LIB
    if _LIB is None:
        if not os.path.exists(LIB_PATH):
            raise RuntimeError(
                f"{LIB_PATH} is missing: build it with `make -C {os.path.join(_PKG_DIR, 'csrc')}` "
                "(there is no CPU or PyTorch fallback for the ProPainter hot path)")
        lib = ctypes.CDLL(LIB_PATH)
        for name, (res, args) in _SIGNATURES.items():
            fn = getattr(lib, name)
            fn.restype = res
            fn.argtypes = args
        _LIB = lib
    return _LIB


def exported_symbols():
    return sorted(_SIGNATURES)




def choose_bn(cout: int) -> Tuple[int, int]:
    best = None
    t0 = (cout + MAX_BN - 1) // MAX_BN
    for n_tiles in (t0, t0 + 1):
        bn = ((cout + n_tiles - 1) // n_tiles + 15) // 16 * 16
        if bn > MAX_BN:
            continue
        cand = (bn * n_tiles, n_tiles, bn)
        if best is None or cand < best:
            best = cand
    return best[2], best[0]


def pack_conv_weight(w: torch.Tensor, groups: int = 1, cin_map=None):
    w = w.detach().float().cpu()
    cout, cin_ref, kh, kw = w.shape
    if cin_map is None:
        cin_map = list(range(cin_ref)) + [-1] * ((-cin_ref) % 8)
    assert len(cin_map) % 8 == 0
    cin_k = len(cin_map)
    idx = torch.tensor([max(i, 0) for i in cin_map], dtype=torch.long)
    keep = torch.tensor([1.0 if i >= 0 else 0.0 for i in cin_map])
    wk = w[:, idx] * keep.view(1, -1, 1, 1)
    wk = wk.permute(0, 2, 3, 1).reshape(cout, kh * kw * cin_k)
    cout_g = cout // groups
    bn, cout_g_pad = choose_bn(cout_g)
    K = wk.shape[1]
    K_pad = (K + 63) // 64 * 64
    buf = torch.zeros(groups, cout_g_pad, K_pad)
    buf[:, :cout_g, :K] = wk.view(groups, cout_g, K)
    num_kc = K_pad // 64
    buf = buf.view(groups, cout_g_pad, num_kc, 8, 8).permute(0, 2, 1, 3, 4).contiguous()
    rows = torch.arange(cout_g_pad)
    pos = torch.arange(8).view(1, 8) ^ (rows.view(-1, 1) & 7)
    buf = torch.gather(buf, 3, pos.view(1, 1, cout_g_pad, 8, 1).expand(groups, num_kc, cout_g_pad, 8, 8))
    meta = dict(cout_g=cout_g, cout_g_pad=cout_g_pad, bn=bn, cin_g=cin_k, kh=kh, kw=kw, groups=groups)
    return buf.to(torch.float16).contiguous(), meta


def split_tf32(x: torch.Tensor):
    x = x.detach().float().contiguous()
    hi = ((x.view(torch.int32) + 0x1000) & ~0x1FFF).view(torch.float32)
    return hi, x - hi


def pack_conv_weight_tf32(w, cin_map=None):
    w = w.detach().float().cpu()
    cout, cin_ref, kh, kw = w.shape
    if cin_map is None:
        cin_map = list(range(cin_ref)) + [-1] * ((-cin_ref) % 4)
    assert len(cin_map) % 4 == 0
    cin_k = len(cin_map)
    idx = torch.tensor([max(i, 0) for i in cin_map], dtype=torch.long)
    keep = torch.tensor([1.0 if i >= 0 else 0.0 for i in cin_map])
    hi, lo = split_tf32(w[:, idx] * keep.view(1, -1, 1, 1))
    wk = torch.cat([hi, hi, lo], 1).permute(0, 2, 3, 1).reshape(cout, kh * kw * 3 * cin_k)
    bn, cout_pad = choose_bn(cout)
    K = wk.shape[1]
    K_pad = (K + 31) // 32 * 32
    buf = torch.zeros(cout_pad, K_pad)
    buf[:cout, :K] = wk
    num_kc = K_pad // 32
    buf = buf.view(cout_pad, num_kc, 8, 4).permute(1, 0, 2, 3).contiguous()
    rows = torch.arange(cout_pad)
    pos = torch.arange(8).view(1, 8) ^ (rows.view(-1, 1) & 7)
    buf = torch.gather(buf, 2, pos.view(1, cout_pad, 8, 1).expand(num_kc, cout_pad, 8, 4))
    meta = dict(cout_g=cout, cout_g_pad=cout_pad, bn=bn, cin_g=2 * 3 * cin_k, kh=kh, kw=kw, groups=1)
    return buf.contiguous(), meta


def _fold_bn(w, b, sd, p, eps=1e-5):
    scale = sd[p + ".weight"] / torch.sqrt(sd[p + ".running_var"] + eps)
    return w * scale.view(-1, 1, 1, 1), (b - sd[p + ".running_mean"]) * scale + sd[p + ".bias"]


def _pad_map(n_real: int, total: int):
    return list(range(n_real)) + [-1] * (total - n_real)


def build_layers(raft_sd, rfc_sd, gen_sd):
    convs: Dict[str, tuple] = {}
    tens: Dict[str, torch.Tensor] = {}

    def add(name, w, b, groups=1, cin_map=None, macs=None):
        convs[name] = (w.float(), None if b is None else b.float(), groups, cin_map,
                       float(w.shape[0] * w.shape[1] * w.shape[2] * w.shape[3]) if macs is None else float(macs))

    r = {(k[7:] if k.startswith("module.") else k): v.float() for k, v in raft_sd.items()}
    Wspec.check_state_dict(r, Wspec.raft_spec())
    for net, bn in (("fnet", False), ("cnet", True)):
        def cv(dst, src, norm=None, cin_map=None):
            w, b = r[f"{net}.{src}.weight"], r[f"{net}.{src}.bias"]
            if bn and norm is not None:
                w, b = _fold_bn(w, b, r, f"{net}.{norm}")
            add(f"raft.{net}.{dst}", w, b, 1, cin_map)
        cv("conv1", "conv1", "norm1", _pad_map(3, 8))
        for li in (1, 2, 3):
            for bi in (0, 1):
                q = f"layer{li}.{bi}."
                cv(q + "conv1", q + "conv1", q + "norm1")
                cv(q + "conv2", q + "conv2", q + "norm2")
                if li > 1 and bi == 0:
                    cv(q + "downsample", q + "downsample.0", q + "norm3")
        cv("conv2", "conv2")
    u = "update_block."
    add("raft.update.convc1", r[u + "encoder.convc1.weight"], r[u + "encoder.convc1.bias"], 1, _pad_map(324, 328))
    add("raft.update.convc2", r[u + "encoder.convc2.weight"], r[u + "encoder.convc2.bias"])
    wf1 = r[u + "encoder.convf1.weight"]
    wf1 = torch.cat([wf1.permute(0, 2, 3, 1).reshape(128, 98), torch.zeros(128, 30)], 1).view(128, 128, 1, 1)
    add("raft.update.convf1", wf1, r[u + "encoder.convf1.bias"], 1, None, macs=128 * 98)
    add("raft.update.convf2", r[u + "encoder.convf2.weight"], r[u + "encoder.convf2.bias"])
    add("raft.update.conv", r[u + "encoder.conv.weight"], r[u + "encoder.conv.bias"])
    for s in ("1", "2"):
        add("raft.update.gru.zr" + s, torch.cat([r[u + f"gru.convz{s}.weight"], r[u + f"gru.convr{s}.weight"]], 0),
            torch.cat([r[u + f"gru.convz{s}.bias"], r[u + f"gru.convr{s}.bias"]], 0))
        add("raft.update.gru.q" + s, r[u + f"gru.convq{s}.weight"], r[u + f"gru.convq{s}.bias"])
    add("raft.update.fh1", r[u + "flow_head.conv1.weight"], r[u + "flow_head.conv1.bias"])
    add("raft.update.fh2", r[u + "flow_head.conv2.weight"], r[u + "flow_head.conv2.bias"])
    add("raft.update.mask0", r[u + "mask.0.weight"], r[u + "mask.0.bias"])
    add("raft.update.mask2", r[u + "mask.2.weight"], r[u + "mask.2.bias"])

    f = {k: v.float() for k, v in rfc_sd.items()}
    Wspec.check_state_dict(f, Wspec.rfc_spec())
    add("rfc.downsample", f["downsample.0.weight"][:, :, 0], f["downsample.0.bias"], 1, _pad_map(3, 8))
    for enc in ("encoder1", "encoder2"):
        for i in (0, 2):
            add(f"rfc.{enc}.{i}.conv1", f[f"{enc}.{i}.conv1.0.weight"][:, :, 0], f[f"{enc}.{i}.conv1.0.bias"])
            add(f"rfc.{enc}.{i}.conv2", f[f"{enc}.{i}.conv2.0.weight"][:, :, :, :, 0], f[f"{enc}.{i}.conv2.0.bias"])
    for j, i in enumerate((0, 2, 4)):
        add(f"rfc.mid.{j}", f[f"mid_dilation.{i}.weight"][:, :, 0], f[f"mid_dilation.{i}.bias"])

    def add_align(dst, sd, src):
        for j, i in enumerate((0, 2, 4, 6)):
            w = sd[f"{src}.conv_offset.{i}.weight"]
            cm = None if w.shape[1] % 8 == 0 else _pad_map(w.shape[1], (w.shape[1] + 7) // 8 * 8)
            add(f"{dst}.offset.{j}", w, sd[f"{src}.conv_offset.{i}.bias"], 1, cm)
        w = sd[src + ".weight"]
        add(f"{dst}.dcn", w.permute(0, 2, 3, 1).reshape(w.shape[0], -1, 1, 1), sd[src + ".bias"])

    fp = "feat_prop_module."
    for d in ("backward_", "forward_"):
        add_align(f"rfc.fp.{d}", f, fp + "deform_align." + d)
        add(f"rfc.fp.{d}.backbone.0", f[fp + f"backbone.{d}.0.weight"], f[fp + f"backbone.{d}.0.bias"])
        add(f"rfc.fp.{d}.backbone.1", f[fp + f"backbone.{d}.2.weight"], f[fp + f"backbone.{d}.2.bias"])
    add("rfc.fp.fusion", f[fp + "fusion.weight"], f[fp + "fusion.bias"])
    for dst, src in (("decoder2.0", "decoder2.0"), ("decoder2.deconv", "decoder2.2.conv"), ("decoder1.0", "decoder1.0"),
                     ("decoder1.deconv", "decoder1.2.conv"), ("upsample.0", "upsample.0"),
                     ("upsample.deconv", "upsample.2.conv")):
        add("rfc." + dst, f[src + ".weight"], f[src + ".bias"])

    g = {k: v.float() if v.is_floating_point() else v for k, v in gen_sd.items()}
    Wspec.check_state_dict(g, Wspec.generator_spec())
    enc_groups = {0: 1, 2: 1, 4: 1, 6: 1, 8: 1, 10: 2, 12: 4, 14: 8, 16: 1}
    for i, gr in enc_groups.items():
        w = g[f"encoder.layers.{i}.weight"]
        if i == 14:
            cout, cg = w.shape[0], w.shape[1]
            nx, npv = 256 // gr, 384 // gr
            assert cg == nx + npv and cout % gr == 0
            dense = torch.zeros(cout, 640, w.shape[2], w.shape[3])
            for k in range(gr):
                rows = slice(k * (cout // gr), (k + 1) * (cout // gr))
                dense[rows, k * nx:(k + 1) * nx] = w[rows, :nx]
                dense[rows, 256 + k * npv:256 + (k + 1) * npv] = w[rows, nx:]
            add("gen.encoder.14", dense, g["encoder.layers.14.bias"], 1, None, macs=w.numel())
            continue
        add(f"gen.encoder.{i}", w, g[f"encoder.layers.{i}.bias"], gr, _pad_map(5, 8) if i == 0 else None)
    for dst, src in (("0", "0.conv"), ("2", "2"), ("4", "4.conv"), ("6", "6")):
        add("gen.decoder." + dst, g[f"decoder.{src}.weight"], g[f"decoder.{src}.bias"])
    add("gen.ss", g["ss.embedding.weight"].view(512, 128, 7, 7), g["ss.embedding.bias"])
    perm = (torch.arange(49).view(49, 1) + 49 * torch.arange(128).view(1, 128)).reshape(-1)
    add("gen.sc.embedding", g["sc.embedding.weight"][perm].view(6272, 512, 1, 1), g["sc.embedding.bias"][perm])
    add("gen.sc.bias_conv", g["sc.bias_conv.weight"], g["sc.bias_conv.bias"])
    for d in ("backward_1", "forward_1"):
        add_align(f"gen.fp.{d}", g, fp + "deform_align." + d)
        add(f"gen.fp.{d}.backbone.0", g[fp + f"backbone.{d}.0.weight"], g[fp + f"backbone.{d}.0.bias"], 1,
            _pad_map(258, 264))
        add(f"gen.fp.{d}.backbone.1", g[fp + f"backbone.{d}.2.weight"], g[fp + f"backbone.{d}.2.bias"])
    add("gen.fp.fuse.0", g[fp + "fuse.0.weight"], g[fp + "fuse.0.bias"], 1, _pad_map(258, 264))
    add("gen.fp.fuse.1", g[fp + "fuse.2.weight"], g[fp + "fuse.2.bias"])
    perm40 = (torch.arange(49).view(49, 1) + 49 * torch.arange(40).view(1, 40)).reshape(-1)
    for b in range(Wspec.N_TRANSFORMER_BLOCKS):
        t = f"transformers.transformer.{b}."
        a = t + "attention."
        o = f"gen.tf.{b}."
        qkv_w = torch.cat([g[a + "query.weight"], g[a + "key.weight"], g[a + "value.weight"]], 0)
        qkv_b = torch.cat([g[a + "query.bias"], g[a + "key.bias"], g[a + "value.bias"]], 0)
        add(o + "qkv", qkv_w.view(1536, 512, 1, 1), qkv_b)
        add(o + "kv", qkv_w[512:].reshape(1024, 512, 1, 1), qkv_b[512:])
        add(o + "proj", g[a + "proj.weight"].view(512, 512, 1, 1), g[a + "proj.bias"])
        add(o + "fc1", g[t + "mlp.fc1.0.weight"][perm40].view(1960, 512, 1, 1), g[t + "mlp.fc1.0.bias"][perm40])
        add(o + "fc2", g[t + "mlp.fc2.1.weight"].view(512, 40, 7, 7), g[t + "mlp.fc2.1.bias"])
        for n in ("norm1", "norm2"):
            tens[o + n + ".weight"] = g[t + n + ".weight"].float()
            tens[o + n + ".bias"] = g[t + n + ".bias"].float()
        tens[o + "pool.weight"] = g[a + "pool_layer.weight"].reshape(512, 16).float().t().contiguous()
        tens[o + "pool.bias"] = g[a + "pool_layer.bias"].float()
        expect = torch.from_numpy(Wspec.rolled_valid_indices())
        if not torch.equal(g[a + "valid_ind_rolled"].cpu().long(), expect):
            raise ValueError("checkpoint's valid_ind_rolled differs from the 5x9 window ring this engine implements")
    return convs, tens




def _ptr(t):
    return None if t is None else ctypes.c_void_p(t.data_ptr())


class Engine:

    MIN_WORKSPACE = 256 << 20

    def __init__(self, device: torch.device | str | int = "cuda:0", workspace_gb: float | None = None):
        self.lib = load_library()
        self.device = torch.device(device)
        if self.device.type != "cuda" or not torch.cuda.is_available():
            raise RuntimeError("the ProPainter CUDA engine needs a CUDA device (no CPU fallback)")
        if self.device.index is None:
            self.device = torch.device("cuda", torch.cuda.current_device())
        self._keep = []
        self._total_mem = torch.cuda.get_device_properties(self.device).total_memory
        self.fixed_workspace = workspace_gb is not None
        nbytes = self.MIN_WORKSPACE if workspace_gb is None else int(min(workspace_gb * (1 << 30), self._total_mem * 0.8))
        self.workspace = torch.empty(nbytes, dtype=torch.uint8, device=self.device)
        h = ctypes.c_void_p()
        self._check(self.lib.pp_create(self.device.index, _ptr(self.workspace), nbytes, ctypes.byref(h)))
        self.h = h
        self.conv_meta: Dict[str, dict] = {}

    @staticmethod
    def clip_workspace_bytes(T: int, H: int, W: int) -> int:
        return int(1400 * min(T, 100) * H * W + (2 << 30))

    def set_workspace_bytes(self, nbytes: int) -> None:
        nbytes = max(int(nbytes), self.MIN_WORKSPACE)
        torch.cuda.current_stream(self.device).synchronize()
        self.workspace = None
        torch.cuda.empty_cache()
        ws = torch.empty(nbytes, dtype=torch.uint8, device=self.device)
        self._check(self.lib.pp_set_workspace(self.h, _ptr(ws), nbytes))
        self.workspace = ws

    def reserve_for_clip(self, T: int, H: int, W: int) -> int:
        if self.fixed_workspace:
            return self.workspace.numel()
        free, _ = torch.cuda.mem_get_info(self.device)
        have = self.workspace.numel()
        want = min(self.clip_workspace_bytes(T, H, W), int(self._total_mem * 0.8), int((free + have) * 0.9))
        if want > have:
            self.set_workspace_bytes(want)
        return self.workspace.numel()

    def release_workspace(self) -> None:
        if not self.fixed_workspace and self.workspace.numel() > self.MIN_WORKSPACE:
            self.set_workspace_bytes(self.MIN_WORKSPACE)

    def _check(self, rc: int):
        if rc != 0:
            raise RuntimeError("propainter_b200: " + self.lib.pp_last_error().decode())

    def _stream(self):
        return ctypes.c_void_p(torch.cuda.current_stream(self.device).cuda_stream)

    def close(self):
        if getattr(self, "h", None):
            self.lib.pp_destroy(self.h)
            self.h = None
        self.workspace = None
        self._keep = []

    def __del__(self):
        try:
            self.close()
        except Exception:
            pass

    def _register_packed(self, name, packed, meta, w, b, macs):
        packed = packed.to(self.device)
        bias = None if b is None else b.detach().float().contiguous().to(self.device)
        self._keep += [packed, bias]
        self.conv_meta[name] = meta
        self._check(self.lib.pp_register_conv(self.h, name.encode(), _ptr(packed), _ptr(bias), meta["cout_g"],
                                              meta["cout_g_pad"], meta["bn"], meta["cin_g"], meta["kh"], meta["kw"],
                                              meta["groups"]))
        self._check(self.lib.pp_set_conv_macs(self.h, name.encode(), float(w.numel() if macs is None else macs)))

    def register_conv(self, name, w, b, groups=1, cin_map=None, macs=None):
        self._register_packed(name, *pack_conv_weight(w, groups, cin_map), w, b, macs)

    def register_conv_tf32(self, name, w, b, cin_map=None, macs=None):
        self._register_packed(name + ".tf32", *pack_conv_weight_tf32(w, cin_map), w, b, macs)

    def register_tensor(self, name, t):
        t = t.detach().float().contiguous().to(self.device)
        self._keep.append(t)
        self._check(self.lib.pp_register_tensor(self.h, name.encode(), _ptr(t), t.numel() * 4))

    PAD64_CONVS = ("rfc.encoder1.0.conv1", "rfc.encoder1.0.conv2", "rfc.upsample.0", "rfc.upsample.deconv") + tuple(
        f"raft.{net}.layer2.{blk}" for net in ("fnet", "cnet") for blk in ("0.conv2", "1.conv1", "1.conv2")) + (
        "gen.fp.backward_1.offset.0", "gen.fp.forward_1.offset.0", "gen.fp.backward_1.backbone.0",
        "gen.fp.forward_1.backbone.0", "gen.fp.fuse.0")

    TF32_CIN_MAPS = {"raft.fnet.conv1": (3, 4), "raft.cnet.conv1": (3, 4), "raft.update.convc1": (324, 352),
                     "rfc.downsample": (3, 4)}

    def load_weights(self, raft_sd, rfc_sd, gen_sd):
        convs, tens = build_layers(raft_sd, rfc_sd, gen_sd)
        for name, (w, b, groups, cin_map, macs) in convs.items():
            if name.startswith(("raft.", "rfc.")):
                tm = self.TF32_CIN_MAPS.get(name)
                self.register_conv_tf32(name, w, b, None if tm is None else _pad_map(*tm), macs)
            if name in self.PAD64_CONVS:
                cin_map = list(cin_map) if cin_map is not None else list(range(w.shape[1]))
                cin_map += [-1] * ((-len(cin_map)) % 64)
            self.register_conv(name, w, b, groups, cin_map, macs)
        for name, t in tens.items():
            self.register_tensor(name, t)
        return self

    def _f32(self, t):
        return t.to(device=self.device, dtype=torch.float32).contiguous()

    def raft_bidir(self, frames: torch.Tensor, iters: int, out=None, fp32: bool = False):
        frames = self._f32(frames)
        T, _, H, W = frames.shape
        if out is not None:
            ff, fb = out
            assert ff.is_contiguous() and fb.is_contiguous() and ff.dtype == torch.float32 and ff.shape == (T - 1, 2, H, W)
        else:
            ff = torch.empty(T - 1, 2, H, W, device=self.device, dtype=torch.float32)
            fb = torch.empty_like(ff)
        fn = self.lib.pp_raft_bidir_fp32 if fp32 else self.lib.pp_raft_bidir
        self._check(fn(self.h, _ptr(frames), T, H, W, int(iters), _ptr(ff), _ptr(fb), self._stream()))
        return ff, fb

    def flow_complete(self, flows_f, flows_b, flow_masks, fp32: bool = False):
        flows_f, flows_b, flow_masks = self._f32(flows_f), self._f32(flows_b), self._f32(flow_masks)
        T, _, H, W = flow_masks.shape
        assert flows_f.shape[0] == T - 1
        of, ob = torch.empty_like(flows_f), torch.empty_like(flows_b)
        fn = self.lib.pp_flow_complete_fp32 if fp32 else self.lib.pp_flow_complete
        self._check(fn(self.h, _ptr(flows_f), _ptr(flows_b), _ptr(flow_masks), T, H, W, _ptr(of), _ptr(ob),
                       self._stream()))
        return of, ob

    def flow_complete_dist(self, flows_f, flows_b, flow_masks, team_first: int, team_size: int, out=None,
                           fp32: bool = False):
        flows_f, flows_b, flow_masks = self._f32(flows_f), self._f32(flows_b), self._f32(flow_masks)
        T, _, H, W = flow_masks.shape
        assert flows_f.shape[0] == T - 1
        of, ob = out if out is not None else (torch.empty_like(flows_f), torch.empty_like(flows_b))
        assert of.is_contiguous() and ob.is_contiguous() and of.dtype == torch.float32
        fn = self.lib.pp_flow_complete_dist_fp32 if fp32 else self.lib.pp_flow_complete_dist
        self._check(fn(self.h, _ptr(flows_f), _ptr(flows_b), _ptr(flow_masks), T, H, W, _ptr(of), _ptr(ob),
                       int(team_first), int(team_size), self._stream()))
        return of, ob

    def image_propagate(self, frames, masks, flows_f, flows_b, fp32: bool = False):
        frames, masks, flows_f, flows_b = map(self._f32, (frames, masks, flows_f, flows_b))
        T, _, H, W = frames.shape
        uf, um = torch.empty_like(frames), torch.empty_like(masks)
        fn = self.lib.pp_image_propagate_fp32 if fp32 else self.lib.pp_image_propagate
        self._check(fn(self.h, _ptr(frames), _ptr(masks), _ptr(flows_f), _ptr(flows_b), T, H, W, _ptr(uf), _ptr(um),
                       self._stream()))
        return uf, um

    def gen_begin(self, updated_frames, masks_dilated, updated_masks, flows_f, flows_b, frames_needed=None):
        a = [self._f32(x) for x in (updated_frames, masks_dilated, updated_masks, flows_f, flows_b)]
        T, _, H, W = a[0].shape
        self._gen_shape = (T, H, W)
        self._gen_inputs = a
        self._gen_needed = None if frames_needed is None else set(int(i) for i in frames_needed)
        if frames_needed is None:
            self._check(self.lib.pp_gen_begin(self.h, *[_ptr(x) for x in a], T, H, W, self._stream()))
        else:
            need = bytes(1 if i in self._gen_needed else 0 for i in range(T))
            self._check(self.lib.pp_gen_begin_subset(self.h, *[_ptr(x) for x in a], T, H, W, need, self._stream()))

    def gen_window(self, frame_ids, l_t: int) -> torch.Tensor:
        T, H, W = self._gen_shape
        ids = (ctypes.c_int * len(frame_ids))(*[int(i) for i in frame_ids])
        pred = torch.empty(l_t, H, W, 4, device=self.device, dtype=torch.float16)
        self._check(self.lib.pp_gen_window(self.h, ids, len(frame_ids), int(l_t), _ptr(pred), self._stream()))
        return pred

    @staticmethod
    def gen_slot_bytes(H: int, W: int) -> int:
        p4 = (H // 4) * (W // 4)
        gh, gw = (H // 4 + 6 - 7) // 3 + 1, (W // 4 + 6 - 7) // 3 + 1
        rows_pad = -(-gh // 5) * 5 * (-(-gw // 9) * 9)
        xfmr = p4 * (256 + 80) + gh * gw * 2 * (512 * 3 + 1960) + rows_pad * 2 * (512 + 1536)
        featprop = p4 * 2 * (128 * 4) + p4 * 2 * (264 + 432 + 1152 + 128 * 3) // 8
        return int(1.25 * (xfmr + featprop))

    def gen_batches(self, windows, budget_bytes: int, shape=None):
        T, H, W = shape if shape is not None else self._gen_shape
        per_slot = self.gen_slot_bytes(H, W)
        out, cur, used = [], [], 0
        for w in windows:
            need = (len(w[0]) + len(w[1])) * per_slot
            if cur and used + need > budget_bytes:
                out.append(cur)
                cur, used = [], 0
            cur.append(w)
            used += need
        if cur:
            out.append(cur)
        return out

    def gen_run(self, windows) -> torch.Tensor:
        T, H, W = self._gen_shape
        enc_bytes = T * (H // 4) * (W // 4) * (256 + 32) + (64 << 20)
        decoder_reserve = 24 * H * W * 2 * 200
        budget = max(self.workspace.numel() - enc_bytes - decoder_reserve, self.gen_slot_bytes(H, W))
        out = [self._gen_run_or_split(b) for b in self.gen_batches(list(windows), budget)]
        return out[0] if len(out) == 1 else torch.cat(out, 0)

    def _gen_run_or_split(self, windows) -> torch.Tensor:
        try:
            return self._gen_run_once(windows)
        except RuntimeError as ex:
            if "workspace" not in str(ex) or len(windows) == 1:
                raise
        half = len(windows) // 2
        return torch.cat([self._gen_run_or_split(windows[:half]), self._gen_run_or_split(windows[half:])], 0)

    gen_run_calls = 0

    def _gen_run_once(self, windows) -> torch.Tensor:
        self.gen_run_calls += 1
        T, H, W = self._gen_shape
        flat, wt, wl = [], [], []
        if getattr(self, "_gen_needed", None) is not None:
            missing = {int(i) for nb, refs in windows for i in list(nb) + list(refs)} - self._gen_needed
            if missing:
                raise ValueError(f"gen_run: frames {sorted(missing)} were not encoded by gen_begin(frames_needed=...)")
        for nb, refs in windows:
            flat += [int(i) for i in nb] + [int(i) for i in refs]
            wt.append(len(nb) + len(refs))
            wl.append(len(nb))
        arr = lambda v: (ctypes.c_int * len(v))(*v)
        pred = torch.empty(sum(wl), H, W, 4, device=self.device, dtype=torch.float16)
        self._check(self.lib.pp_gen_run(self.h, arr(flat), arr(wt), arr(wl), len(windows), _ptr(pred), self._stream()))
        return pred

    def gen_end(self):
        self._check(self.lib.pp_gen_end(self.h))
        self._gen_inputs = None

    def composite(self, pred, masks_dilated, orig_u8, comp_u8, frame_ids_dev, first_visit_dev, half_math=False):
        l_t, H, W, _ = pred.shape
        self._check(self.lib.pp_composite(self.h, _ptr(pred), _ptr(masks_dilated), _ptr(orig_u8), _ptr(comp_u8),
                                          _ptr(frame_ids_dev), _ptr(first_visit_dev), l_t, H, W, int(bool(half_math)),
                                          self._stream()))

    def preprocess(self, image, mask, flow_mask_dilates: int, mask_dilates: int, process_size=None):
        T, H, W, _ = image.shape
        ow, oh = (W, H) if process_size is None else (int(process_size[0]), int(process_size[1]))
        if image.device.type == "cpu" and mask.device.type == "cpu" and image.dtype == torch.float32 and mask.dtype == torch.float32:
            return self._preprocess_host(image.contiguous(), mask.contiguous(), flow_mask_dilates, mask_dilates, ow, oh)
        img = image.to(self.device, torch.float32, non_blocking=True).contiguous()
        msk = mask.to(self.device, torch.float32, non_blocking=True).contiguous()
        orig = torch.empty(T, oh, ow, 3, device=self.device, dtype=torch.uint8)
        frames = torch.empty(T, 3, oh, ow, device=self.device, dtype=torch.float32)
        fm = torch.empty(T, 1, oh, ow, device=self.device, dtype=torch.float32)
        md = torch.empty_like(fm)
        if (ow, oh) == (W, H):
            self._check(self.lib.pp_preprocess(self.h, _ptr(img), _ptr(msk), msk.shape[0], T, H, W, int(flow_mask_dilates),
                                               int(mask_dilates), _ptr(orig), _ptr(frames), _ptr(fm), _ptr(md),
                                               self._stream()))
        else:
            self._check(self.lib.pp_preprocess_resize(self.h, _ptr(img), _ptr(msk), msk.shape[0], T, H, W, oh, ow,
                                                      int(flow_mask_dilates), int(mask_dilates), _ptr(orig), _ptr(frames),
                                                      _ptr(fm), _ptr(md), self._stream()))
        return frames.unsqueeze(0), fm.unsqueeze(0), md.unsqueeze(0), orig

    def _preprocess_host(self, image, mask, flow_mask_dilates, mask_dilates, ow, oh):
        T, H, W, _ = image.shape
        threads = min(os.cpu_count() or 1, int(os.environ.get("PP_HOST_THREADS", 16)))
        try:
            img8 = torch.empty(image.shape, dtype=torch.uint8, pin_memory=True)
            msk8 = torch.empty(mask.shape, dtype=torch.uint8, pin_memory=True)
        except RuntimeError:
            img8 = torch.empty(image.shape, dtype=torch.uint8)
            msk8 = torch.empty(mask.shape, dtype=torch.uint8)
        self._check(self.lib.pp_host_quantize_u8(_ptr(image), _ptr(img8), image.numel(), threads))
        img8d = img8.to(self.device, non_blocking=True)
        self._check(self.lib.pp_host_quantize_u8(_ptr(mask), _ptr(msk8), mask.numel(), threads))
        msk8d = msk8.to(self.device, non_blocking=True)
        orig = torch.empty(T, oh, ow, 3, device=self.device, dtype=torch.uint8)
        frames = torch.empty(T, 3, oh, ow, device=self.device, dtype=torch.float32)
        fm = torch.empty(T, 1, oh, ow, device=self.device, dtype=torch.float32)
        md = torch.empty_like(fm)
        self._check(self.lib.pp_preprocess_u8(self.h, _ptr(img8d), _ptr(msk8d), mask.shape[0], T, H, W, oh, ow,
                                              int(flow_mask_dilates), int(mask_dilates), _ptr(orig), _ptr(frames), _ptr(fm),
                                              _ptr(md), self._stream()))
        self._keep_staging = (img8, msk8)
        return frames.unsqueeze(0), fm.unsqueeze(0), md.unsqueeze(0), orig

    def postprocess(self, comp_u8: torch.Tensor) -> torch.Tensor:
        out = torch.empty(comp_u8.shape, device=self.device, dtype=torch.float32)
        self._check(self.lib.pp_postprocess(self.h, _ptr(comp_u8), _ptr(out), comp_u8.numel(), self._stream()))
        return out

    rank, world = 0, 1

    def comm_unique_id(self) -> bytes:
        buf = ctypes.create_string_buffer(128)
        self._check(self.lib.pp_comm_unique_id(buf))
        return buf.raw

    def comm_init(self, unique_id: bytes, rank: int, world: int):
        assert len(unique_id) == 128
        self._check(self.lib.pp_comm_init(self.h, ctypes.create_string_buffer(unique_id, 128), int(rank), int(world)))
        self.rank, self.world = int(rank), int(world)

    def comm_destroy(self):
        self._check(self.lib.pp_comm_destroy(self.h))
        self.rank, self.world = 0, 1

    def comm_all_gather_rows(self, buf: torch.Tensor, rows, first_rank: int = 0):
        assert buf.is_contiguous() and buf.shape[0] == sum(rows)
        row_bytes = buf[0].numel() * buf.element_size() if buf.shape[0] else 0
        if len(rows) <= 1 or row_bytes == 0:
            return buf
        arr = (ctypes.c_longlong * len(rows))(*[int(r) for r in rows])
        self._check(self.lib.pp_comm_all_gather_rows(self.h, _ptr(buf), arr, row_bytes, int(first_rank), len(rows),
                                                     self._stream()))
        return buf

    @property
    def launch_count(self) -> int:
        return int(self.lib.pp_launch_count(self.h))

    @property
    def workspace_peak(self) -> int:
        return int(self.lib.pp_workspace_peak(self.h))

    def profile_enable(self, on: bool):
        self._check(self.lib.pp_profile_enable(self.h, int(on)))

    def profile_dump(self):
        buf = ctypes.create_string_buffer(1 << 20)
        self._check(self.lib.pp_profile_dump(self.h, buf, len(buf)))
        out = {}
        for line in buf.value.decode().splitlines():
            name, n, ms, rows, flops, nbytes = line.split("\t")
            out[name] = dict(count=int(n), ms=float(ms), rows=float(rows), flops=float(flops), bytes=float(nbytes))
        return out

    def op_conv(self, name, x_nhwc, stride=1, pad=0, dil=1, replicate=False, act=ACT_NONE, slope=0.0, residual=None):
        m = self.conv_meta[name]
        N, H, W, _ = x_nhwc.shape
        kh, kw = m["kh"], m["kw"]
        OH = (H + 2 * pad - dil * (kh - 1) - 1) // stride + 1
        OW = (W + 2 * pad - dil * (kw - 1) - 1) // stride + 1
        out = torch.empty(N, OH, OW, m["cout_g"] * m["groups"], device=self.device, dtype=torch.float16)
        self._check(self.lib.pp_op_conv(self.h, name.encode(), _ptr(x_nhwc), N, H, W, stride, pad, dil, int(replicate),
                                        act, float(slope), _ptr(residual), _ptr(out), self._stream()))
        return out

    def op_corr_lookup(self, levels, coords, h8, w8):
        nq = coords.shape[0]
        out = torch.empty(nq, 328, device=self.device, dtype=torch.float16)
        self._check(self.lib.pp_op_corr_lookup(self.h, *[_ptr(l) for l in levels], _ptr(coords), _ptr(out), nq, h8, w8,
                                               self._stream()))
        return out

    EPI_STD, EPI_GRU_ZR, EPI_GRU_H = range(3)

    def op_conv_tf32(self, name, inputs, out, out_co=0, stride=(1, 1), pad=(0, 0), act=ACT_NONE, slope=0.0, scale=1.0,
                     act2=ACT_NONE, residual=None, gru_zr=None, gru_h=None, out_fp32=False, dilation=(1, 1),
                     replicate=False):
        N, H, W = inputs[0][0].shape[:3]
        (x0, c0, n0), (x1, c1, n1) = inputs[0], (inputs[1] if len(inputs) > 1 else (None, 0, 0))
        C = lambda t: 0 if t is None else t.shape[-1] // 2
        epi, a0, a0_co, a1, a1_co = self.EPI_STD, None, 0, None, 0
        if residual is not None:
            a0, a0_co = residual
        if gru_zr is not None:
            epi, (a0, a0_co, a1, a1_co) = self.EPI_GRU_ZR, gru_zr
        if gru_h is not None:
            epi, (a0, a0_co, a1, a1_co) = self.EPI_GRU_H, gru_h
        self._check(self.lib.pp_op_conv_tf32(
            self.h, (name + ".tf32").encode(), _ptr(x0), C(x0), c0, n0, _ptr(x1), C(x1), c1, n1, N, H, W, stride[0],
            stride[1], pad[0], pad[1], dilation[0], dilation[1], int(replicate), epi, act, float(slope), float(scale), act2, _ptr(a0), C(a0), a0_co, _ptr(a1), C(a1),
            a1_co, _ptr(out), out.shape[-1] if out_fp32 else C(out), out_co, int(out_fp32), self._stream()))
        return out

    def op_dcn_sample_f32(self, x0, x1, offs, max_mag=5.0):
        N, H, W = x0.shape[:3]
        cols = torch.empty(N, H, W, 2 * 2304, device=self.device, dtype=torch.float32)
        C1 = 0 if x1 is None else x1.shape[-1] // 2
        self._check(self.lib.pp_op_dcn_sample_f32(self.h, _ptr(x0), x0.shape[-1] // 2, _ptr(x1), C1, _ptr(offs), N, H,
                                                  W, float(max_mag), _ptr(cols), self._stream()))
        return cols

    def op_upsample2x_f32(self, x):
        N, H, W, C2 = x.shape
        out = torch.empty(N, 2 * H, 2 * W, C2, device=self.device, dtype=torch.float32)
        self._check(self.lib.pp_op_upsample2x_f32(self.h, _ptr(x), _ptr(out), N, H, W, C2 // 2, self._stream()))
        return out

    def op_instnorm(self, x, C, relu=False, residual=None, out=None, fp32=True):
        out = torch.empty_like(x) if out is None else out
        N, HW = x.shape[:2]
        self._check(self.lib.pp_op_instnorm(self.h, _ptr(x), _ptr(residual), _ptr(out), N, HW, C, int(relu), int(fp32),
                                            self._stream()))
        return out

    def op_corr_pyramid(self, fmap1, fmap2, h8, w8, fp32=True):
        pairs = fmap1.shape[0]
        dt = torch.float32 if fp32 else torch.float16
        lv = [torch.empty(pairs * h8 * w8, (h8 >> l) * (w8 >> l), device=self.device, dtype=dt) for l in range(4)]
        self._check(self.lib.pp_op_corr_pyramid(self.h, _ptr(fmap1), _ptr(fmap2), pairs, h8, w8, int(fp32),
                                                *[_ptr(t) for t in lv], self._stream()))
        return lv

    def op_corr_lookup_f32(self, levels, coords, h8, w8):
        nq = coords.shape[0]
        out = torch.empty(nq, 704, device=self.device, dtype=torch.float32)
        self._check(self.lib.pp_op_corr_lookup_f32(self.h, *[_ptr(l) for l in levels], _ptr(coords), _ptr(out), nq, h8,
                                                   w8, self._stream()))
        return out

    def op_convex_upsample(self, coords1, mask, B, h8, w8, fp32=True):
        out = torch.empty(B, 2, 8 * h8, 8 * w8, device=self.device, dtype=torch.float32)
        self._check(self.lib.pp_op_convex_upsample(self.h, _ptr(coords1), _ptr(mask), _ptr(out), B, h8, w8, int(fp32),
                                                   self._stream()))
        return out

    def op_imgprop_step(self, cur4, prop4, flow_prop, flow_check):
        H, W, _ = cur4.shape
        out = torch.empty_like(cur4)
        self._check(self.lib.pp_op_imgprop_step(self.h, _ptr(cur4), _ptr(prop4), _ptr(out), _ptr(flow_prop),
                                                _ptr(flow_check), H, W, self._stream()))
        return out

    def op_imgprop_step_f32(self, cur4, prop4, flow_prop, flow_check):
        H, W, _ = cur4.shape
        out = torch.empty_like(cur4)
        self._check(self.lib.pp_op_imgprop_step_f32(self.h, _ptr(cur4), _ptr(prop4), _ptr(out), _ptr(flow_prop),
                                                    _ptr(flow_check), H, W, self._stream()))
        return out

    def op_attention(self, qkv, pkv, win_flags, t, gh, gw, n_pool, parity):
        out = torch.zeros(t, gh, gw, 512, device=self.device, dtype=torch.float16)
        self._check(self.lib.pp_op_attention(self.h, _ptr(qkv), _ptr(pkv), _ptr(out), _ptr(win_flags), t, gh, gw, n_pool,
                                             parity, self._stream()))
        return out
```

include/propainter_b200.h:

```cpp
#ifndef PROPAINTER_B200_H
#define PROPAINTER_B200_H

#include <stddef.h>
#include <stdint.h>

#ifdef __cplusplus
extern "C" {
#endif

#if defined(__GNUC__)
#define PP_API __attribute__((visibility("default")))
#else
#define PP_API
#endif

typedef struct PPEngine* pp_handle;

PP_API const char* pp_last_error(void);
PP_API const char* pp_version(void);

PP_API int pp_create(int device, void* workspace, size_t workspace_bytes, pp_handle* out);
PP_API int pp_destroy(pp_handle h);
PP_API int pp_set_workspace(pp_handle h, void* workspace, size_t workspace_bytes);

PP_API int pp_register_conv(pp_handle h, const char* name, const void* w, const float* bias, int cout_g, int cout_g_pad,
                     int bn, int cin_g, int kh, int kw, int groups);
PP_API int pp_register_tensor(pp_handle h, const char* name, const void* ptr, size_t bytes);
PP_API int pp_set_conv_macs(pp_handle h, const char* name, double macs_per_pixel);

PP_API int pp_comm_unique_id(void* out128);
PP_API int pp_comm_init(pp_handle h, const void* unique_id128, int rank, int world);
PP_API int pp_comm_destroy(pp_handle h);
PP_API int pp_comm_all_gather_rows(pp_handle h, void* buf, const long long* rows_per_member, size_t row_bytes,
                                   int first_rank, int n_members, void* stream);

PP_API int pp_raft_bidir(pp_handle h, const float* frames, int T, int H, int W, int iters, float* flows_f, float* flows_b,
                  void* stream);
PP_API int pp_raft_bidir_fp32(pp_handle h, const float* frames, int T, int H, int W, int iters, float* flows_f,
                              float* flows_b, void* stream);
PP_API int pp_flow_complete(pp_handle h, const float* flows_f, const float* flows_b, const float* flow_masks, int T, int H,
                     int W, float* out_f, float* out_b, void* stream);
PP_API int pp_flow_complete_dist(pp_handle h, const float* flows_f, const float* flows_b, const float* flow_masks, int T,
                                 int H, int W, float* out_f, float* out_b, int team_first, int team_size, void* stream);
PP_API int pp_flow_complete_fp32(pp_handle h, const float* flows_f, const float* flows_b, const float* flow_masks, int T,
                                 int H, int W, float* out_f, float* out_b, void* stream);
PP_API int pp_flow_complete_dist_fp32(pp_handle h, const float* flows_f, const float* flows_b, const float* flow_masks,
                                      int T, int H, int W, float* out_f, float* out_b, int team_first, int team_size,
                                      void* stream);
PP_API int pp_image_propagate(pp_handle h, const float* frames, const float* masks, const float* flows_f,
                       const float* flows_b, int T, int H, int W, float* updated_frames, float* updated_masks,
                       void* stream);
PP_API int pp_image_propagate_fp32(pp_handle h, const float* frames, const float* masks, const float* flows_f,
                                   const float* flows_b, int T, int H, int W, float* updated_frames,
                                   float* updated_masks, void* stream);
PP_API int pp_gen_begin(pp_handle h, const float* updated_frames, const float* masks_dilated, const float* updated_masks,
                 const float* flows_f, const float* flows_b, int T, int H, int W, void* stream);
PP_API int pp_gen_begin_subset(pp_handle h, const float* updated_frames, const float* masks_dilated,
                               const float* updated_masks, const float* flows_f, const float* flows_b, int T, int H, int W,
                               const unsigned char* frames_needed, void* stream);
PP_API int pp_gen_window(pp_handle h, const int* frame_ids, int t, int l_t, void* pred_f16, void* stream);
PP_API int pp_gen_run(pp_handle h, const int* frame_ids, const int* win_t, const int* win_lt, int n_windows,
                      void* pred_f16, void* stream);
PP_API int pp_gen_end(pp_handle h);
PP_API int pp_composite(pp_handle h, const void* pred_f16, const float* masks_dilated, const uint8_t* orig, uint8_t* comp,
                 const int* frame_ids_dev, const int* first_visit_dev, int l_t, int H, int W, int half_math,
                 void* stream);

PP_API int pp_preprocess(pp_handle h, const float* image, const float* mask, int mask_frames, int T, int H, int W,
                         int flow_mask_dilates, int mask_dilates, uint8_t* orig_u8, float* frames, float* flow_masks,
                         float* masks_dilated, void* stream);
PP_API int pp_preprocess_resize(pp_handle h, const float* image, const float* mask, int mask_frames, int T, int H, int W,
                                int out_h, int out_w, int flow_mask_dilates, int mask_dilates, uint8_t* orig_u8,
                                float* frames, float* flow_masks, float* masks_dilated, void* stream);
PP_API int pp_preprocess_u8(pp_handle h, const uint8_t* image_u8, const uint8_t* mask_u8, int mask_frames, int T, int H,
                            int W, int out_h, int out_w, int flow_mask_dilates, int mask_dilates, uint8_t* orig_u8,
                            float* frames, float* flow_masks, float* masks_dilated, void* stream);
PP_API int pp_host_quantize_u8(const float* src, uint8_t* dst, long long n, int threads);
PP_API int pp_postprocess(pp_handle h, const uint8_t* comp_u8, float* image_out, long long n, void* stream);

PP_API long long pp_launch_count(pp_handle h);
PP_API size_t pp_workspace_peak(pp_handle h);

PP_API int pp_profile_enable(pp_handle h, int on);
PP_API int pp_profile_dump(pp_handle h, char* buf, size_t cap);

PP_API int pp_op_conv(pp_handle h, const char* name, const void* x_f16, int N, int H, int W, int stride, int pad, int dil,
               int replicate, int act, float slope, const void* residual_f16, void* out_f16, void* stream);
PP_API int pp_op_corr_lookup(pp_handle h, const void* l0, const void* l1, const void* l2, const void* l3,
                      const float* coords, void* out_f16, long long nq, int h8, int w8, void* stream);
PP_API int pp_op_conv_tf32(pp_handle h, const char* name, const float* x0, int x0_C, int x0_co, int x0_ch, const float* x1,
                           int x1_C, int x1_co, int x1_ch, int N, int H, int W, int sh, int sw, int ph, int pw, int dh,
                           int dw, int replicate, int epi, int act, float slope, float scale, int act2, const float* aux0, int aux0_C, int aux0_co,
                           float* aux1, int aux1_C, int aux1_co, float* out, int out_C, int out_co, int out_fp32,
                           void* stream);
PP_API int pp_op_dcn_sample_f32(pp_handle h, const float* x0, int C0, const float* x1, int C1, const float* offs, int N,
                                int H, int W, float max_mag, float* cols, void* stream);
PP_API int pp_op_upsample2x_f32(pp_handle h, const float* src, float* dst, int N, int H, int W, int C, void* stream);
PP_API int pp_op_instnorm(pp_handle h, const void* x, const void* residual, void* out, int N, int HW, int C, int relu,
                          int fp32, void* stream);
PP_API int pp_op_corr_pyramid(pp_handle h, const void* fmap1, const void* fmap2, int pairs, int h8, int w8, int fp32,
                              void* l0, void* l1, void* l2, void* l3, void* stream);
PP_API int pp_op_corr_lookup_f32(pp_handle h, const float* l0, const float* l1, const float* l2, const float* l3,
                                 const float* coords, float* out, long long nq, int h8, int w8, void* stream);
PP_API int pp_op_convex_upsample(pp_handle h, const float* coords1, const void* mask, float* out, int B, int h8, int w8,
                                 int fp32, void* stream);
PP_API int pp_op_imgprop_step(pp_handle h, const void* cur4_f16, const void* prop_in4_f16, void* prop_out4_f16,
                       const void* flow_prop_f16, const void* flow_check_f16, int H, int W, void* stream);
PP_API int pp_op_imgprop_step_f32(pp_handle h, const float* cur4, const float* prop_in4, float* prop_out4,
                                  const float* flow_prop, const float* flow_check, int H, int W, void* stream);
PP_API int pp_op_attention(pp_handle h, const void* qkv_f16, const void* pkv_f16, void* out_f16, const int* win_flags_dev,
                    int t, int gh, int gw, int n_pool, int parity, void* stream);

#ifdef __cplusplus
}
#endif
#endif
```

Measured before the change: 167.7.

## Use TMA loads and stores for the halo conv epilogue residual, GRU and output paths

Adds a TMA-based epilogue to the fp16 halo conv kernel. Residual and GRU aux tiles are prefetched with 4D tensor-map loads, issued just before the final wgmma wait so they overlap the math, and outputs are written with swizzled TMA bulk stores instead of per-thread global stores. The mainloop moves into a shared helper, the shared-memory layout changes for the output staging region, and a new pp_op_conv_ex API is exposed for testing. This costs extra tensor-map encoding per launch and more complex barrier and phase handling, with some risk of synchronisation bugs.

```diff
diff --git a/comfyui_propainter_nodes_b200/csrc/capi.cu b/comfyui_propainter_nodes_b200/csrc/capi.cu
--- a/comfyui_propainter_nodes_b200/csrc/capi.cu
+++ b/comfyui_propainter_nodes_b200/csrc/capi.cu
@@ -461,6 +461,31 @@
   return c.run(as_stream(stream));
 }
 
+int pp_op_conv_ex(pp_handle h, const char* name, const void* x_f16, int x_C, int x_co, int N, int H, int W, int ph,
+                  int pw, int epi, int act, float slope, float scale, int act2, const void* aux0_f16, int aux0_C,
+                  int aux0_co, void* aux1_f16, int aux1_C, int aux1_co, void* out_f16, int out_C, int out_co, void* stream) {
+  PP_HANDLE(h);
+  PP_REQUIRE(name && x_f16 && out_f16, "pp_op_conv_ex: null pointer");
+  PP_REQUIRE(epi == PP_EPI_STD || (aux0_f16 && aux1_f16), "pp_op_conv_ex: the GRU epilogues need aux0 and aux1");
+  const PPPackedConv* w = nullptr;
+  PP_TRY(pp_get_conv(e, name, &w));
+  PPConvCall c(e, name, N, H, W);
+  c.in(static_cast<const __half*>(x_f16), x_C, x_co, w->cin_g, w->groups > 1 ? w->cin_g : 0)
+      .geom(1, 1, ph, pw)
+      .out(static_cast<__half*>(out_f16), out_C, out_co, w->groups > 1 ? w->cout_g : 0);
+  const __half* a0 = static_cast<const __half*>(aux0_f16);
+  __half* a1 = static_cast<__half*>(aux1_f16);
+  if (epi == PP_EPI_GRU_ZR) {
+    c.gru_zr(a0, aux0_C, aux0_co, a1, aux1_C, aux1_co);
+  } else if (epi == PP_EPI_GRU_H) {
+    c.gru_h(a0, aux0_C, aux0_co, a1, aux1_C, aux1_co);
+  } else {
+    c.act(act, slope, scale, act2);
+    if (a0 != nullptr) c.residual(a0, aux0_C, aux0_co);
+  }
+  return c.run(as_stream(stream));
+}
+
 int pp_op_corr_lookup(pp_handle h, const void* l0, const void* l1, const void* l2, const void* l3,
                       const float* coords, void* out_f16, long long nq, int h8, int w8, void* stream) {
   PP_HANDLE(h);
diff --git a/comfyui_propainter_nodes_b200/csrc/conv_epilogue.cuh b/comfyui_propainter_nodes_b200/csrc/conv_epilogue.cuh
--- a/comfyui_propainter_nodes_b200/csrc/conv_epilogue.cuh
+++ b/comfyui_propainter_nodes_b200/csrc/conv_epilogue.cuh
@@ -126,6 +126,24 @@
       for (int i = 0; i < 16; ++i) v[i] = (1.f - z[i]) * h[i] + z[i] * v[i];
       store16(reinterpret_cast<__half*>(p.out) + mrow * p.out_cstride + p.out_coff + ng0, nvalid, vec, v);
     }
+}
+
+template <int ACT1>
+__device__ __forceinline__ void std_epi4(float (&v)[4], bool has_bias, const float2& bias, float scale, bool has_res,
+                                          const float (&res)[4], int act2, float slope) {
+  if (has_bias) {
+    v[0] += bias.x; v[1] += bias.y; v[2] += bias.x; v[3] += bias.y;
+  }
+  act16_t<ACT1>(v, slope);
+  if (scale != 1.f) {
+#pragma unroll
+    for (int i = 0; i < 4; ++i) v[i] *= scale;
+  }
+  if (has_res) {
+#pragma unroll
+    for (int i = 0; i < 4; ++i) v[i] += res[i];
+  }
+  if (act2 != PP_ACT_NONE) act16(v, act2, slope);
 }
 
 __device__ __forceinline__ void load16_split(const float* src, int lo, int nvalid, bool vec, float (&r)[16]) {
diff --git a/comfyui_propainter_nodes_b200/csrc/conv_gemm.cu b/comfyui_propainter_nodes_b200/csrc/conv_gemm.cu
--- a/comfyui_propainter_nodes_b200/csrc/conv_gemm.cu
+++ b/comfyui_propainter_nodes_b200/csrc/conv_gemm.cu
@@ -41,24 +41,6 @@
   return m;
 }
 
-template <int ACT1>
-__device__ __forceinline__ void gemm_epi4(float (&v)[4], bool has_bias, const float2& bias, float scale, bool has_res,
-                                          const float (&res)[4], int act2, float slope) {
-  if (has_bias) {
-    v[0] += bias.x; v[1] += bias.y; v[2] += bias.x; v[3] += bias.y;
-  }
-  ppconv::act16_t<ACT1>(v, slope);
-  if (scale != 1.f) {
-#pragma unroll
-    for (int i = 0; i < 4; ++i) v[i] *= scale;
-  }
-  if (has_res) {
-#pragma unroll
-    for (int i = 0; i < 4; ++i) v[i] += res[i];
-  }
-  if (act2 != PP_ACT_NONE) ppconv::act16(v, act2, slope);
-}
-
 template <int MB, int BN, int ACT1>
 __device__ __forceinline__ void gemm_epilogue(const PPConvParams& p, const float (&acc)[MB][BN / 2], uint8_t* so,
                                               const float* bs, bool has_res, int t128) {
@@ -83,7 +65,7 @@
         const float2 r0 = __half22float2(*lo), r1 = __half22float2(*hi);
         res[0] = r0.x; res[1] = r0.y; res[2] = r1.x; res[3] = r1.y;
       }
-      gemm_epi4<ACT1>(v, has_bias, bias, scale, has_res, res, act2, slope);
+      ppconv::std_epi4<ACT1>(v, has_bias, bias, scale, has_res, res, act2, slope);
       *lo = __floats2half2_rn(v[0], v[1]);
       *hi = __floats2half2_rn(v[2], v[3]);
     }
diff --git a/comfyui_propainter_nodes_b200/csrc/conv_halo.cu b/comfyui_propainter_nodes_b200/csrc/conv_halo.cu
--- a/comfyui_propainter_nodes_b200/csrc/conv_halo.cu
+++ b/comfyui_propainter_nodes_b200/csrc/conv_halo.cu
@@ -15,8 +15,9 @@
 constexpr int WARP_A = 8, WARP_B = 9;
 constexpr int MAX_SA = 4, MAX_SB = 8;
 constexpr int SMEM_BUDGET = 186 * 1024;
-
-struct HaloParams {
+constexpr int SMEM_MAX = 227 * 1024;
+
+struct HaloLayer {
   PPConvParams c;
   CUtensorMap tmap[PP_MAX_SEGS];
   int MT;
@@ -31,10 +32,18 @@
   int debug;
 };
 
+struct HaloParams : HaloLayer {
+  int tma_out;
+  CUtensorMap tm_out;
+  CUtensorMap tm_out2;
+  CUtensorMap tm_aux0;
+  CUtensorMap tm_aux1;
+};
+
 struct TileCoord {
   int n_idx, tx, ty, img, g;
 };
-__device__ __forceinline__ TileCoord decode_tile(const HaloParams& h, int tile) {
+__device__ __forceinline__ TileCoord decode_tile(const HaloLayer& h, int tile) {
   TileCoord t;
   t.n_idx = tile % h.n_tiles;
   int r = tile / h.n_tiles;
@@ -45,7 +54,7 @@
   return t;
 }
 
-__host__ __device__ inline int halo_total_tiles(const HaloParams& h) {
+__host__ __device__ inline int halo_total_tiles(const HaloLayer& h) {
   return h.n_tiles * h.tiles_x * h.tiles_y * h.n_img * h.c.groups;
 }
 
@@ -117,8 +126,51 @@
   wgmma_commit();
 }
 
+template <int BN, int MB, int NT, class BeforeWait>
+__device__ __forceinline__ void halo_mainloop(const HaloLayer& h, const HaloSmem& m, Ring& ra, Ring& rb, int wg,
+                                              float (&acc)[MB][BN / 2], BeforeWait&& before_wait) {
+  using namespace ppx;
+  const PPConvParams& p = h.c;
+  const int taps = p.kh * p.kw;
+  const uint32_t sbo = h.flat ? 1024u : (uint32_t)h.BW * 128;
+  const uint32_t step_x = (uint32_t)p.dw * 8;
+  const uint32_t step_row = (uint32_t)(p.dh * h.BW - (p.kw - 1) * p.dw) * 8;
+  const uint32_t tap16 = (uint32_t)p.BN * 8;
+  const int kw = p.kw;
+  uint32_t aoff[MB];
+#pragma unroll
+  for (int b = 0; b < MB; ++b) aoff[b] = MB == 2 ? wg * h.sub_bytes + b * 8 * sbo : wg * 8 * sbo;
+  uint32_t accum = 0;
+  int pend_a = -1, pend_b = -1;
+  for (int c = 0; c < h.chunks; ++c) {
+    mbar_wait(&m.a_full[ra.s], ra.ph);
+    uint64_t adesc[MB];
+#pragma unroll
+    for (int b = 0; b < MB; ++b) adesc[b] = gmma_desc_sw128_kmajor(smem_u32(m.a + ra.s * m.a_stage_bytes) + aoff[b], sbo);
+    int kx = 0;
+    for (int tap0 = 0; tap0 < taps; tap0 += h.tps) {
+      mbar_wait(&m.b_full[rb.s], rb.ph);
+      const uint64_t bdesc = gmma_desc_sw128_kmajor(smem_u32(m.b + rb.s * m.b_stage_bytes));
+      halo_tap_group<BN, MB, NT, false>(min(h.tps, taps - tap0), acc, adesc, bdesc, accum, kx, kw, step_x, step_row, tap16);
+      wgmma_wait<1>();
+      if (pend_b >= 0) mbar_arrive(&m.b_empty[pend_b]);
+      if (pend_a >= 0) mbar_arrive(&m.a_empty[pend_a]);
+      pend_b = rb.s;
+      pend_a = tap0 + h.tps >= taps ? ra.s : -1;
+      if (++rb.s == m.SB) { rb.s = 0; rb.ph ^= 1; }
+    }
+    if (++ra.s == m.SA) { ra.s = 0; ra.ph ^= 1; }
+  }
+  before_wait();
+  wgmma_wait<0>();
+#pragma unroll
+  for (int b = 0; b < MB; ++b) wgmma_fence_acc(acc[b]);
+  if (pend_b >= 0) mbar_arrive(&m.b_empty[pend_b]);
+  if (pend_a >= 0) mbar_arrive(&m.a_empty[pend_a]);
+}
+
 template <int BN, int MB, int NT, bool TF32 = false, bool PROG = false>
-__device__ __forceinline__ void halo_tile(const HaloParams& h, int tile, const HaloSmem& m, Ring& ra, Ring& rb, float* stg,
+__device__ __forceinline__ void halo_tile(const HaloLayer& h, int tile, const HaloSmem& m, Ring& ra, Ring& rb, float* stg,
                                           int wg, int t128) {
   using namespace ppx;
   const PPConvParams& p = h.c;
@@ -184,6 +236,165 @@
   }
 }
 
+__host__ __device__ constexpr int halo_panel_width(int bn) { return bn % 64 == 0 ? 64 : bn % 32 == 0 ? 32 : 16; }
+__host__ __device__ constexpr int halo_out_stage_bytes(int mt, int bn) { return 2 * 64 * mt * bn * 2; }
+__host__ __device__ constexpr int halo_out_bias_bytes(int bn) { return (2 * bn * 4 + 1023) / 1024 * 1024; }
+__host__ __device__ constexpr int halo_out_z_bytes(int mt, int bn) { return 2 * 64 * mt * halo_panel_width(bn) * 2; }
+__host__ __device__ constexpr int halo_tma_region_bytes(int mt, int bn, bool gru_h) {
+  return halo_out_stage_bytes(mt, bn) + halo_out_bias_bytes(bn) + (gru_h ? halo_out_z_bytes(mt, bn) : 0);
+}
+__device__ __forceinline__ uint64_t* halo_out_bar(const HaloSmem& m, int wg) { return m.spare + 1 + wg; }
+
+template <int PW>
+__device__ __forceinline__ uint32_t halo_stg_off(int r, int c) {
+  const uint32_t off = (uint32_t)(r * PW * 2 + (c % PW) * 2);
+  return off ^ ((off >> 3) & (uint32_t)((PW / 8 - 1) << 4));
+}
+
+template <int MB, int BN, int EPI, int ACT1>
+__device__ __forceinline__ void halo_frag_epilogue(const PPConvParams& p, const float (&acc)[MB][BN / 2], uint8_t* so,
+                                                   const uint8_t* zb, const float* bs, bool has_aux, bool r_tile, int P,
+                                                   int t128) {
+  constexpr int PW = halo_panel_width(BN);
+  constexpr int PANEL = 64 * MB * PW * 2;
+  const bool has_bias = p.bias != nullptr;
+  const float scale = p.scale, slope = p.slope;
+  const int act2 = p.act2;
+  const int fr = 16 * (t128 >> 5) + ((t128 & 31) >> 2), fc = 2 * (t128 & 3);
+#pragma unroll
+  for (int b = 0; b < MB; ++b) {
+    const int r = 64 * b + fr;
+#pragma unroll
+    for (int j = 0; j < BN / 8; ++j) {
+      const int col = 8 * j + fc;
+      if (EPI == PP_EPI_GRU_H && col / PW != P) continue;
+      const uint32_t off = (col / PW) * PANEL + halo_stg_off<PW>(r, col);
+      __half2* lo = reinterpret_cast<__half2*>(so + off);
+      __half2* hi = reinterpret_cast<__half2*>(so + off + 8 * PW * 2);
+      const float2 bias = *reinterpret_cast<const float2*>(bs + col);
+      float v[4] = {acc[b][4 * j], acc[b][4 * j + 1], acc[b][4 * j + 2], acc[b][4 * j + 3]};
+      float a[4] = {0.f, 0.f, 0.f, 0.f};
+      if (has_aux) {
+        const float2 a0 = __half22float2(*lo), a1 = __half22float2(*hi);
+        a[0] = a0.x; a[1] = a0.y; a[2] = a1.x; a[3] = a1.y;
+      }
+      if constexpr (EPI == PP_EPI_STD) {
+        ppconv::std_epi4<ACT1>(v, has_bias, bias, scale, has_aux, a, act2, slope);
+      } else {
+        if (has_bias) {
+          v[0] += bias.x; v[1] += bias.y; v[2] += bias.x; v[3] += bias.y;
+        }
+        if constexpr (EPI == PP_EPI_GRU_ZR) {
+          ppconv::act16_t<PP_ACT_SIGMOID>(v, 0.f);
+          if (r_tile) {
+#pragma unroll
+            for (int i = 0; i < 4; ++i) v[i] *= a[i];
+          }
+        } else {
+          const uint32_t zoff = halo_stg_off<PW>(r, col);
+          const float2 z0 = __half22float2(*reinterpret_cast<const __half2*>(zb + zoff));
+          const float2 z1 = __half22float2(*reinterpret_cast<const __half2*>(zb + zoff + 8 * PW * 2));
+          const float z[4] = {z0.x, z0.y, z1.x, z1.y};
+          ppconv::act16_t<PP_ACT_TANH>(v, 0.f);
+#pragma unroll
+          for (int i = 0; i < 4; ++i) v[i] = (1.f - z[i]) * a[i] + z[i] * v[i];
+        }
+      }
+      *lo = __floats2half2_rn(v[0], v[1]);
+      *hi = __floats2half2_rn(v[2], v[3]);
+    }
+  }
+}
+
+template <int BN, int MB, int NT>
+__device__ __forceinline__ void halo_tile_tma(const HaloParams& h, int tile, const HaloSmem& m, Ring& ra, Ring& rb,
+                                              uint32_t& xph, int wg, int t128) {
+  using namespace ppx;
+  const PPConvParams& p = h.c;
+  constexpr int PW = halo_panel_width(BN);
+  constexpr int PANEL = 64 * MB * PW * 2;
+  const TileCoord t = decode_tile(h, tile);
+  const int n0 = t.n_idx * BN;
+  const int epi = p.epi;
+  const int half_c = p.Cout_g >> 1;
+  const bool r_tile = epi == PP_EPI_GRU_ZR && n0 >= half_c;
+  const bool has_aux = epi == PP_EPI_STD ? p.aux0 != nullptr : (epi == PP_EPI_GRU_H || r_tile);
+  const int npanel = (min(BN, p.Cout_g - n0) + PW - 1) / PW;
+  uint8_t* so = reinterpret_cast<uint8_t*>(m.acc_stg) + wg * (64 * MB * BN * 2);
+  float* bs = reinterpret_cast<float*>(reinterpret_cast<uint8_t*>(m.acc_stg) + halo_out_stage_bytes(MB, BN)) + wg * BN;
+  uint8_t* zb = reinterpret_cast<uint8_t*>(bs - wg * BN) + halo_out_bias_bytes(BN) + wg * PANEL;
+  uint64_t* xbar = halo_out_bar(m, wg);
+  int x0, y0, img;
+  if (h.flat) {
+    x0 = MB == 2 ? (t.tx * 2 + wg) * 128 : t.tx * 128 + 64 * wg; y0 = 0; img = 0;
+  } else {
+    x0 = t.tx * (8 * MB) + (MB == 2 ? 8 * wg : 0); y0 = t.ty * 16 + (MB == 2 ? 0 : 8 * wg); img = t.img;
+  }
+  const int aux_c = r_tile ? n0 - half_c : n0;
+  const bool issuer = t128 == 0;
+  const bool skip = (h.debug & 1) != 0;
+  float acc[MB][BN / 2];
+  halo_mainloop<BN, MB, NT>(h, m, ra, rb, wg, acc, [&] {
+    if (issuer && has_aux && !skip) {
+      tma_store_wait_read<0>();
+      const int nz = epi == PP_EPI_GRU_H ? 1 : 0;
+      mbar_arrive_expect_tx(xbar, (uint32_t)((npanel + nz) * PANEL));
+      for (int pn = 0; pn < npanel; ++pn)
+        tma_load_4d(smem_u32(so + pn * PANEL), &h.tm_aux0, aux_c + pn * PW, x0, y0, img, xbar);
+      if (nz) tma_load_4d(smem_u32(zb), &h.tm_aux1, n0, x0, y0, img, xbar);
+    }
+  });
+  if (skip) return;
+
+  {
+    const int c0 = 2 * t128, n = t.g * p.Cout_g + n0 + c0;
+    float2 bv = make_float2(0.f, 0.f);
+    if (p.bias != nullptr && c0 < BN) {
+      if (n0 + c0 < p.Cout_g) bv.x = __ldg(p.bias + n);
+      if (n0 + c0 + 1 < p.Cout_g) bv.y = __ldg(p.bias + n + 1);
+    }
+    if (c0 < BN) *reinterpret_cast<float2*>(bs + c0) = bv;
+  }
+  const int bar_id = 4 + wg;
+  if (issuer && !has_aux) tma_store_wait_read<0>();
+  named_bar(bar_id, 128);
+  if (has_aux) {
+    mbar_wait(xbar, xph);
+    xph ^= 1;
+  }
+  if (epi == PP_EPI_STD) {
+    switch (p.act1) {
+      case PP_ACT_RELU: halo_frag_epilogue<MB, BN, PP_EPI_STD, PP_ACT_RELU>(p, acc, so, zb, bs, has_aux, false, 0, t128); break;
+      case PP_ACT_LRELU: halo_frag_epilogue<MB, BN, PP_EPI_STD, PP_ACT_LRELU>(p, acc, so, zb, bs, has_aux, false, 0, t128); break;
+      default: halo_frag_epilogue<MB, BN, PP_EPI_STD, PP_ACT_NONE>(p, acc, so, zb, bs, has_aux, false, 0, t128); break;
+    }
+  } else if (epi == PP_EPI_GRU_ZR) {
+    halo_frag_epilogue<MB, BN, PP_EPI_GRU_ZR, PP_ACT_NONE>(p, acc, so, zb, bs, r_tile, r_tile, 0, t128);
+  } else {
+#pragma unroll 1
+    for (int pn = 0; pn < npanel; ++pn) {
+      if (pn > 0) {
+        named_bar(bar_id, 128);
+        if (issuer) {
+          mbar_arrive_expect_tx(xbar, (uint32_t)PANEL);
+          tma_load_4d(smem_u32(zb), &h.tm_aux1, n0 + pn * PW, x0, y0, img, xbar);
+        }
+        mbar_wait(xbar, xph);
+        xph ^= 1;
+      }
+      halo_frag_epilogue<MB, BN, PP_EPI_GRU_H, PP_ACT_NONE>(p, acc, so, zb, bs, true, false, pn, t128);
+    }
+  }
+  fence_proxy_async();
+  named_bar(bar_id, 128);
+  if (issuer) {
+    const CUtensorMap* tm = r_tile ? &h.tm_out2 : &h.tm_out;
+    const int c0 = r_tile ? n0 - half_c : t.g * p.out_gstep + n0;
+    for (int pn = 0; pn < npanel; ++pn) tma_store_4d(tm, smem_u32(so + pn * PANEL), c0 + pn * PW, x0, y0, img);
+    tma_store_commit();
+  }
+}
+
 template <class F>
 __device__ __forceinline__ void with_tile_shape(int mt, int bn, F&& f) {
   if (mt == 2) ppconv::with_tile_width<128>(bn, [&](auto n) { f(n, ppconv::IntC<2>{}); });
@@ -197,7 +408,7 @@
   mbar_fence_init();
 }
 
-__device__ __forceinline__ void halo_produce_patches(const HaloParams& h, const HaloSmem& m, Ring& r) {
+__device__ __forceinline__ void halo_produce_patches(const HaloLayer& h, const HaloSmem& m, Ring& r) {
   using namespace ppx;
   const PPConvParams& p = h.c;
   const int total_tiles = halo_total_tiles(h);
@@ -217,7 +428,7 @@
   }
 }
 
-__device__ __forceinline__ void halo_produce_weights(const HaloParams& h, const HaloSmem& m, Ring& r) {
+__device__ __forceinline__ void halo_produce_weights(const HaloLayer& h, const HaloSmem& m, Ring& r) {
   using namespace ppx;
   const PPConvParams& p = h.c;
   const int total_tiles = halo_total_tiles(h);
@@ -248,7 +459,13 @@
   using namespace ppx;
   const HaloSmem m = halo_smem(dyn_smem_1024(), h.SA, h.a_stage_bytes, h.SB, h.b_stage_bytes);
   const int tid = threadIdx.x, warp = tid >> 5;
-  if (tid == 0) halo_smem_init_barriers(m);
+  if (tid == 0) {
+    if constexpr (!TF32) {
+      mbar_init(halo_out_bar(m, 0), 1);
+      mbar_init(halo_out_bar(m, 1), 1);
+    }
+    halo_smem_init_barriers(m);
+  }
   __syncthreads();
   asm volatile("griddepcontrol.wait;" ::: "memory");
   asm volatile("griddepcontrol.launch_dependents;" ::: "memory");
@@ -260,6 +477,18 @@
     float* stg = m.acc_stg + wg * (ppconv::STG_BYTES / 4);
     Ring ra = {0, 0}, rb = {0, 0};
     const int total_tiles = halo_total_tiles(h);
+    if constexpr (!TF32) {
+      if (h.tma_out) {
+        uint32_t xph = 0;
+        with_tile_shape(h.MT, h.c.BN, [&](auto bn, auto mb) {
+          constexpr int BN = decltype(bn)::value;
+          for (int tile = blockIdx.x; tile < total_tiles; tile += gridDim.x)
+            halo_tile_tma<BN, decltype(mb)::value, halo_max_tps(BN)>(h, tile, m, ra, rb, xph, wg, t128);
+        });
+        if (t128 == 0) tma_store_wait<0>();
+        return;
+      }
+    }
     with_tile_shape(h.MT, h.c.BN, [&](auto bn, auto mb) {
       constexpr int BN = decltype(bn)::value;
       for (int tile = blockIdx.x; tile < total_tiles; tile += gridDim.x)
@@ -310,7 +539,7 @@
   unsigned long long* ts;
   int kind[PROG_MAX_LAYERS];
   PPDcnArgs dcn[PROG_MAX_LAYERS];
-  HaloParams layer[PROG_MAX_LAYERS];
+  HaloLayer layer[PROG_MAX_LAYERS];
 };
 
 __device__ __forceinline__ void prog_wait(const unsigned int* counter, unsigned int target) {
@@ -374,7 +603,7 @@
           }
         }
       } else {
-        const HaloParams& h = P.layer[li];
+        const HaloLayer& h = P.layer[li];
         const int total_tiles = halo_total_tiles(h);
         with_prog_width(h.c.BN, [&](auto bn) {
           constexpr int BN = decltype(bn)::value;
@@ -436,7 +665,7 @@
 int halo_set_smem_limit() {
   static bool done = false;
   if (!done) {
-    PP_CUDA_CHECK(cudaFuncSetAttribute(conv_halo_kernel, cudaFuncAttributeMaxDynamicSharedMemorySize, 224 * 1024));
+    PP_CUDA_CHECK(cudaFuncSetAttribute(conv_halo_kernel, cudaFuncAttributeMaxDynamicSharedMemorySize, SMEM_MAX));
     PP_CUDA_CHECK(cudaFuncSetAttribute(conv_halo_tf32_kernel, cudaFuncAttributeMaxDynamicSharedMemorySize, 224 * 1024));
     PP_CUDA_CHECK(cudaFuncSetAttribute(conv_prog_kernel, cudaFuncAttributeMaxDynamicSharedMemorySize, 224 * 1024));
     done = true;
@@ -455,7 +684,56 @@
   return false;
 }
 
-int halo_configure(const PPConvParams& pin, HaloParams& h, bool one_wave) {
+bool halo_layer_stages(int budget, HaloLayer& h) {
+  int sa = 0, sb = 0;
+  if (!halo_stages(budget, h.a_stage_bytes, h.b_stage_bytes, sa, sb)) return false;
+  if (sa == 3 && sb == MAX_SB && (budget - 4 * h.a_stage_bytes) / h.b_stage_bytes >= MAX_SB) sa = 4;
+  h.SA = sa; h.SB = sb;
+  return true;
+}
+
+bool aligned16(const void* ptr, int cstride, int coff) {
+  return (reinterpret_cast<uintptr_t>(ptr) & 15) == 0 && cstride % 8 == 0 && coff % 8 == 0;
+}
+
+bool halo_tma_configure(HaloParams& h) {
+  const PPConvParams& p = h.c;
+  const int bn = p.BN, pw = halo_panel_width(bn), rows = 64 * h.MT;
+  if (p.split || p.out_fp32) return false;
+  if (p.epi == PP_EPI_STD && p.act1 != PP_ACT_NONE && p.act1 != PP_ACT_RELU && p.act1 != PP_ACT_LRELU) return false;
+  if (p.epi != PP_EPI_STD && p.groups != 1) return false;
+  if (p.epi == PP_EPI_STD && p.aux0 != nullptr && p.groups != 1) return false;
+  if (p.groups > 1 && (p.out_gstep != p.Cout_g || p.Cout_g % pw != 0)) return false;
+  if (p.epi == PP_EPI_GRU_ZR && (p.Cout_g % 2 != 0 || (p.Cout_g / 2) % bn != 0)) return false;
+  if (!aligned16(p.out, p.out_cstride, p.out_coff) || (p.groups > 1 && p.out_gstep % 8 != 0)) return false;
+  if (p.Cout_g % 8 != 0) return false;
+  if (p.aux0 != nullptr && !aligned16(p.aux0, p.aux0_cstride, p.aux0_coff)) return false;
+  if (p.epi == PP_EPI_GRU_H && !aligned16(p.aux1, p.aux1_cstride, p.aux1_coff)) return false;
+  if (p.epi == PP_EPI_GRU_ZR && !aligned16(p.out2, p.out2_cstride, p.out2_coff)) return false;
+  const int region = halo_tma_region_bytes(h.MT, bn, p.epi == PP_EPI_GRU_H);
+  HaloLayer staged = h;
+  if (!halo_layer_stages(SMEM_MAX - 2048 - region, staged)) return false;
+  h.SA = staged.SA; h.SB = staged.SB;
+  auto map = [&](CUtensorMap* m, const __half* base, int cols, int cstride) {
+    return h.flat ? pp_tmap_pixels_f16(m, base, cols, cstride, p.M_total, 1, 1, pw, rows, 1)
+                  : pp_tmap_pixels_f16(m, base, cols, cstride, p.OW, p.OH, p.N, pw, 8, rows / 8);
+  };
+  const __half* out = static_cast<const __half*>(p.out) + p.out_coff;
+  const int half_c = p.Cout_g / 2;
+  if (p.epi == PP_EPI_GRU_ZR) {
+    if (map(&h.tm_out, out, half_c, p.out_cstride) != PP_OK) return false;
+    if (map(&h.tm_out2, p.out2 + p.out2_coff, half_c, p.out2_cstride) != PP_OK) return false;
+    if (map(&h.tm_aux0, p.aux0 + p.aux0_coff, half_c, p.aux0_cstride) != PP_OK) return false;
+  } else {
+    if (map(&h.tm_out, out, (p.groups - 1) * p.out_gstep + p.Cout_g, p.out_cstride) != PP_OK) return false;
+    if (p.aux0 != nullptr && map(&h.tm_aux0, p.aux0 + p.aux0_coff, p.Cout_g, p.aux0_cstride) != PP_OK) return false;
+    if (p.epi == PP_EPI_GRU_H && map(&h.tm_aux1, p.aux1 + p.aux1_coff, p.Cout_g, p.aux1_cstride) != PP_OK) return false;
+  }
+  h.tma_out = 1;
+  return true;
+}
+
+int halo_configure(const PPConvParams& pin, HaloLayer& h, bool one_wave) {
   h.c = pin;
   PPConvParams& p = h.c;
   int num_sms = 0;
@@ -497,11 +775,7 @@
   h.a_stage_bytes = pp_ceil_div(h.BW * h.BH * 128, 1024) * 1024;
   h.tps = min(halo_max_tps(bn), p.kh * p.kw);
   h.b_stage_bytes = h.tps * bn * 128;
-  int sa = 0, sb = 0;
-  PP_REQUIRE(halo_stages(SMEM_BUDGET, h.a_stage_bytes, h.b_stage_bytes, sa, sb),
-             "conv_halo: patch %dx%d does not fit shared memory", h.BW, h.BH);
-  if (sa == 3 && sb == MAX_SB && (SMEM_BUDGET - 4 * h.a_stage_bytes) / h.b_stage_bytes >= MAX_SB) sa = 4;
-  h.SA = sa; h.SB = sb;
+  PP_REQUIRE(halo_layer_stages(SMEM_BUDGET, h), "conv_halo: patch %dx%d does not fit shared memory", h.BW, h.BH);
   h.debug = pp_conv_noepi();
   const long long total_tiles = count(mt, bn);
   PP_REQUIRE(total_tiles < (1LL << 31), "conv_halo: too many tiles");
@@ -512,11 +786,16 @@
 
 int pp_launch_conv_halo(const PPConvParams& pin, cudaStream_t stream) {
   HaloParams h;
+  memset(&h, 0, sizeof(h));
   PP_TRY(halo_configure(pin, h, false));
   PP_TRY(halo_set_smem_limit());
   int num_sms = 0;
   PP_TRY(pp_num_sms(&num_sms));
-  const int smem = halo_smem(nullptr, h.SA, h.a_stage_bytes, h.SB, h.b_stage_bytes).bytes;
+  int smem = halo_smem(nullptr, h.SA, h.a_stage_bytes, h.SB, h.b_stage_bytes).bytes;
+  if (halo_tma_configure(h)) {
+    smem = halo_smem(nullptr, h.SA, h.a_stage_bytes, h.SB, h.b_stage_bytes).bytes - 2 * ppconv::STG_BYTES +
+           halo_tma_region_bytes(h.MT, h.c.BN, h.c.epi == PP_EPI_GRU_H);
+  }
   return pp_conv_launch(h.c.split ? conv_halo_tf32_kernel : conv_halo_kernel, h, min(halo_total_tiles(h), num_sms),
                         NUM_THREADS, smem, stream);
 }
@@ -554,7 +833,7 @@
   PP_REQUIRE(p.epi == PP_EPI_STD, "conv program: only the plain epilogue (bias, activations, residual) is compiled in");
   const int li = r->prog.n_layers;
   PP_TRY(halo_configure(p, r->prog.layer[li], true));
-  const HaloParams& h = r->prog.layer[li];
+  const HaloLayer& h = r->prog.layer[li];
   PP_REQUIRE(h.MT == 1 && (h.c.BN == PROG_WIDTHS[0] || h.c.BN == PROG_WIDTHS[1] || h.c.BN == PROG_WIDTHS[2]),
              "conv program: layer tile %d x %d columns is not instantiated", h.MT, h.c.BN);
   r->prog.kind[li] = PROG_CONV;
@@ -614,7 +893,7 @@
     ++ts_printed;
     fprintf(stderr, "[prog %d] %d layers:", ts_printed, P.n_layers);
     for (int i = 0; i < P.n_layers; ++i) {
-      const HaloParams& L = P.layer[i];
+      const HaloLayer& L = P.layer[i];
       if (P.kind[i] == PROG_CONV)
         fprintf(stderr, " | conv K=%d N=%d bn=%d mt=%d tiles=%d: %.1f us (gap %.1f)", L.c.K_total, L.c.Cout_g, L.c.BN, L.MT,
                 halo_total_tiles(L), (h[2 * i + 1] - h[2 * i]) / 1e3, i ? (h[2 * i] - h[2 * i - 1]) / 1e3 : 0.0);
diff --git a/comfyui_propainter_nodes_b200/csrc/conv_igemm.cu b/comfyui_propainter_nodes_b200/csrc/conv_igemm.cu
--- a/comfyui_propainter_nodes_b200/csrc/conv_igemm.cu
+++ b/comfyui_propainter_nodes_b200/csrc/conv_igemm.cu
@@ -335,3 +335,23 @@
   PP_REQUIRE(r == CUDA_SUCCESS, "conv: cuTensorMapEncodeTiled (2-D, %d x %lld, ld %d) failed (%d)", cols, rows, ld, (int)r);
   return PP_OK;
 }
+
+int pp_tmap_pixels_f16(CUtensorMap* map, const __half* base, int cols, int cstride, long long w, int h, int n, int box_c,
+                       int box_w, int box_h) {
+  EncodeTiledFn enc = encode_fn();
+  PP_REQUIRE(enc != nullptr, "conv: cuTensorMapEncodeTiled is not available");
+  const cuuint64_t pix = (cuuint64_t)cstride * 2;
+  cuuint64_t dims[4] = {(cuuint64_t)cols, (cuuint64_t)w, (cuuint64_t)h, (cuuint64_t)n};
+  cuuint64_t strides[3] = {pix, (cuuint64_t)w * pix, (cuuint64_t)w * h * pix};
+  cuuint32_t box[4] = {(cuuint32_t)box_c, (cuuint32_t)box_w, (cuuint32_t)box_h, 1};
+  cuuint32_t es[4] = {1, 1, 1, 1};
+  const CUtensorMapSwizzle swz = box_c == 64 ? CU_TENSOR_MAP_SWIZZLE_128B : box_c == 32 ? CU_TENSOR_MAP_SWIZZLE_64B
+                                                                                        : CU_TENSOR_MAP_SWIZZLE_32B;
+  PP_REQUIRE(box_c == 64 || box_c == 32 || box_c == 16, "conv: pixel tensor map box of %d channels", box_c);
+  const CUresult r = enc(map, CU_TENSOR_MAP_DATA_TYPE_FLOAT16, 4, const_cast<__half*>(base), dims, strides, box, es,
+                         CU_TENSOR_MAP_INTERLEAVE_NONE, swz, CU_TENSOR_MAP_L2_PROMOTION_L2_128B,
+                         CU_TENSOR_MAP_FLOAT_OOB_FILL_NONE);
+  PP_REQUIRE(r == CUDA_SUCCESS, "conv: cuTensorMapEncodeTiled (%d ch x %lld x %d x %d, cstride %d) failed (%d)", cols, w, h, n,
+             cstride, (int)r);
+  return PP_OK;
+}
diff --git a/comfyui_propainter_nodes_b200/csrc/conv_igemm.cuh b/comfyui_propainter_nodes_b200/csrc/conv_igemm.cuh
--- a/comfyui_propainter_nodes_b200/csrc/conv_igemm.cuh
+++ b/comfyui_propainter_nodes_b200/csrc/conv_igemm.cuh
@@ -60,6 +60,8 @@
 bool pp_tmap_supported();
 int pp_conv_input_tmaps(const PPConvParams& p, int bw, int bh, bool flat, CUtensorMap* maps);
 int pp_tmap_2d_f16(CUtensorMap* map, const __half* base, int cols, long long rows, int ld, int box_rows);
+int pp_tmap_pixels_f16(CUtensorMap* map, const __half* base, int cols, int cstride, long long w, int h, int n, int box_c,
+                       int box_w, int box_h);
 int pp_conv_noepi();
 
 inline bool pp_conv_segs_chunked(const PPConvParams& p, bool flat) {
diff --git a/comfyui_propainter_nodes_b200/csrc/pp_common.cuh b/comfyui_propainter_nodes_b200/csrc/pp_common.cuh
--- a/comfyui_propainter_nodes_b200/csrc/pp_common.cuh
+++ b/comfyui_propainter_nodes_b200/csrc/pp_common.cuh
@@ -137,6 +137,11 @@
   asm volatile("cp.async.bulk.tensor.2d.global.shared::cta.bulk_group [%0, {%2, %3}], [%1];" ::"l"(tmap), "r"(src), "r"(c0), "r"(c1)
                : "memory");
 }
+__device__ __forceinline__ void tma_store_4d(const void* tmap, uint32_t src, int c0, int c1, int c2, int c3) {
+  asm volatile("cp.async.bulk.tensor.4d.global.shared::cta.bulk_group [%0, {%2, %3, %4, %5}], [%1];" ::"l"(tmap), "r"(src),
+               "r"(c0), "r"(c1), "r"(c2), "r"(c3)
+               : "memory");
+}
 __device__ __forceinline__ void tma_store_commit() { asm volatile("cp.async.bulk.commit_group;" ::: "memory"); }
 template <int N>
 __device__ __forceinline__ void tma_store_wait_read() {
diff --git a/comfyui_propainter_nodes_b200/engine.py b/comfyui_propainter_nodes_b200/engine.py
--- a/comfyui_propainter_nodes_b200/engine.py
+++ b/comfyui_propainter_nodes_b200/engine.py
@@ -55,6 +55,8 @@
     "pp_profile_enable": (_I, [_VP, _I]),
     "pp_profile_dump": (_I, [_VP, ctypes.c_char_p, _SZ]),
     "pp_op_conv": (_I, [_VP, _CP, _VP, _I, _I, _I, _I, _I, _I, _I, _I, _F, _VP, _VP, _VP]),
+    "pp_op_conv_ex": (_I, [_VP, _CP, _VP, _I, _I, _I, _I, _I, _I, _I, _I, _I, _F, _F, _I, _VP, _I, _I, _VP, _I, _I, _VP,
+                           _I, _I, _VP]),
     "pp_op_corr_lookup": (_I, [_VP, _VP, _VP, _VP, _VP, _VP, _VP, _LL, _I, _I, _VP]),
     "pp_op_conv_tf32": (_I, [_VP, _CP, _VP, _I, _I, _I, _VP, _I, _I, _I, _I, _I, _I, _I, _I, _I, _I, _I, _I, _I, _I, _I,
                              _F, _F, _I, _VP, _I, _I, _VP, _I, _I, _VP, _I, _I, _I, _VP]),
@@ -654,6 +656,22 @@
                                         act, float(slope), _ptr(residual), _ptr(out), self._stream()))
         return out
 
+    def op_conv_ex(self, name, x, out, x_co=0, out_co=0, pad=(0, 0), act=ACT_NONE, slope=0.0, scale=1.0, act2=ACT_NONE,
+                   residual=None, gru_zr=None, gru_h=None):
+        N, H, W, xC = x.shape
+        C = lambda t: 0 if t is None else t.shape[-1]
+        epi, a0, a0_co, a1, a1_co = self.EPI_STD, None, 0, None, 0
+        if residual is not None:
+            a0, a0_co = residual
+        if gru_zr is not None:
+            epi, (a0, a0_co, a1, a1_co) = self.EPI_GRU_ZR, gru_zr
+        if gru_h is not None:
+            epi, (a0, a0_co, a1, a1_co) = self.EPI_GRU_H, gru_h
+        self._check(self.lib.pp_op_conv_ex(
+            self.h, name.encode(), _ptr(x), xC, x_co, N, H, W, pad[0], pad[1], epi, act, float(slope), float(scale), act2,
+            _ptr(a0), C(a0), a0_co, _ptr(a1), C(a1), a1_co, _ptr(out), C(out), out_co, self._stream()))
+        return out
+
     def op_corr_lookup(self, levels, coords, h8, w8):
         nq = coords.shape[0]
         out = torch.empty(nq, 328, device=self.device, dtype=torch.float16)
diff --git a/include/propainter_b200.h b/include/propainter_b200.h
--- a/include/propainter_b200.h
+++ b/include/propainter_b200.h
@@ -86,6 +86,10 @@
 
 PP_API int pp_op_conv(pp_handle h, const char* name, const void* x_f16, int N, int H, int W, int stride, int pad, int dil,
                int replicate, int act, float slope, const void* residual_f16, void* out_f16, void* stream);
+PP_API int pp_op_conv_ex(pp_handle h, const char* name, const void* x_f16, int x_C, int x_co, int N, int H, int W, int ph,
+                         int pw, int epi, int act, float slope, float scale, int act2, const void* aux0_f16, int aux0_C,
+                         int aux0_co, void* aux1_f16, int aux1_C, int aux1_co, void* out_f16, int out_C, int out_co,
+                         void* stream);
 PP_API int pp_op_corr_lookup(pp_handle h, const void* l0, const void* l1, const void* l2, const void* l3,
                       const float* coords, void* out_f16, long long nq, int h8, int w8, void* stream);
 PP_API int pp_op_conv_tf32(pp_handle h, const char* name, const float* x0, int x0_C, int x0_co, int x0_ch, const float* x1,
```

After: 181.6 (median of 6 runs). 8.3% higher.
